# jhljx/CTGCN

Measured on AMD Instinct MI355X. Metric: aggregated edges/s over T-snapshot window (CTGCN-C embedding forward), higher is better.
Workload: dtype f32 (fp16x2-split MFMA operands); 1 GPU; BASELINE config 5: synthetic 1M nodes x 16 cumulative snapshots, avg-deg 16; CTGCN-C hid=128 embed=128, 1 transform + 2 diffusion layers, max_core=8, one-hot features; nodes=1000000, snapshots=16, max_core=8, parallelism=single GPU

## Files before the change

ctgcn_amd/_lib.py:

```python
import ctypes
import os

_HERE = os.path.dirname(os.path.abspath(__file__))
LIB_PATH = os.environ.get("CTGCN_HIP_LIB") or os.path.join(_HERE, "csrc", "libctgcn_hip.so")

F_SELF_LOOP, F_RELU, F_NESTED = 1, 2, 4
ACT_NONE, ACT_SELU = 0, 1
CLS_NODE, CLS_HADAMARD, CLS_DOT = 0, 1, 2
OP_KCORE = 1
OP_INGEST = 2
MAX_SLOTS = 255
ABI_VERSION = 31

_c = ctypes
_vp, _i64, _i32, _u32, _int, _sz = _c.c_void_p, _c.c_int64, _c.c_int32, _c.c_uint32, _c.c_int, _c.c_size_t

class AggSplitGroup(_c.Structure):
    _fields_ = [("row_ptr", _vp), ("col_idx", _vp), ("val", _vp), ("slot", _vp), ("X", _vp), ("ldx", _i64), ("K", _i32), ("flags", _u32),
                ("row_order", _vp), ("tile_mask", _vp), ("workspace", _vp), ("workspace_bytes", _sz),
                ("planes1", _vp), ("planes2", _vp), ("scales", _vp), ("tile_base", _vp)]


class GruLayerGroup(_c.Structure):
    _fields_ = [("planes", _vp), ("w_ih", _vp), ("w_hh", _vp), ("bias_gi", _vp), ("b_hn", _vp), ("ln_weight", _vp), ("ln_bias", _vp),
                ("ln_eps", _c.c_float), ("steps", _i32), ("out", _vp), ("ld_out", _i64), ("row_order", _vp), ("tile_mask", _vp), ("work", _i64)]


class GruSeqGroup(_c.Structure):
    _fields_ = [("gi", _vp), ("w_hh", _vp), ("b_hn", _vp), ("ln_weight", _vp), ("ln_bias", _vp), ("ln_eps", _c.c_float), ("steps", _i32),
                ("out", _vp), ("ld_out", _i64), ("row_order", _vp), ("tile_mask", _vp), ("tile_base", _vp), ("work", _i64)]


SIGNATURES = {
    "ctgcn_abi_version": (_int, []),
    "ctgcn_last_error": (_c.c_char_p, []),
    "ctgcn_device_info": (_int, [_c.c_char_p, _sz, _c.POINTER(_int)]),
    "ctgcn_transpose_bias_f32": (_int, [_i64, _i32, _vp, _i64, _vp, _vp, _i64, _vp]),
    "ctgcn_spmm_csr_f32": (_int, [_i64, _i32, _vp, _vp, _vp, _vp, _i64, _vp, _i64, _int, _vp]),
    "ctgcn_hub_workspace_bytes": (_sz, [_i32, _i32, _i32, _i32]),
    "ctgcn_hub_split_entries": (_i32, []),
    "ctgcn_core_aggregate_f32": (_int, [_i64, _i32, _i32, _vp, _vp, _vp, _vp, _vp, _i64, _vp, _u32, _vp, _i32, _i32, _i32, _vp, _sz, _vp]),
    "ctgcn_core_aggregate_bwd_prep_f32": (_int, [_i64, _i32, _i32, _vp, _vp, _vp, _vp, _u32, _vp]),
    "ctgcn_core_aggregate_bwd_f32": (_int, [_i64, _i32, _i32, _vp, _vp, _vp, _vp, _vp, _vp, _vp, _i64, _u32, _vp, _i32, _i32, _i32, _vp, _sz, _vp]),
    "ctgcn_edges_to_csr": (_int, [_i64, _i64, _vp, _vp, _vp, _vp, _vp, _vp, _c.POINTER(_i64), _vp, _sz, _vp]),
    "ctgcn_kcore_i32": (_int, [_i64, _vp, _vp, _vp, _vp, _sz, _i32, _c.POINTER(_i32), _vp]),
    "ctgcn_edge_levels_i32": (_int, [_i64, _vp, _vp, _vp, _vp, _vp, _vp, _vp, _i32, _vp]),
    "ctgcn_slot_reorder": (_int, [_i64, _i32, _vp, _vp, _vp, _vp, _vp, _i32, _vp, _vp, _vp, _vp]),
    "ctgcn_gru_seq_f32": (_int, [_i64, _i32, _i32, _vp, _vp, _vp, _vp, _vp, _c.c_float, _int, _vp, _i64, _vp, _int, _int, _vp, _vp, _vp, _vp]),
    "ctgcn_layernorm_bwd_f32": (_int, [_i64, _i32, _i32, _vp, _vp, _i64, _vp, _c.c_float, _vp, _vp, _i32, _vp, _vp]),
    "ctgcn_group_table_bytes": (_sz, [_i32]),
    "ctgcn_table_uploads": (ctypes.c_uint64, [_int]),
    "ctgcn_core_aggregate_split_group_f32": (_int, [_i32, _i64, _i32, _vp, _vp, _sz, _vp, _vp]),
    "ctgcn_gru_layer_presplit_group_f32": (_int, [_i32, _i64, _i32, _vp, _vp, _sz, _vp, _vp]),
    "ctgcn_transpose_bias_group_f32": (_int, [_i32, _i64, _i32, _vp, _i64, _vp, _vp, _i64, _vp, _sz, _vp, _vp]),
    "ctgcn_gru_seq_group_f32": (_int, [_i32, _i64, _i32, _vp, _vp, _sz, _vp, _vp]),
    "ctgcn_linear_packed_chain_f32": (_int, [_i64, _i32, _i32, _vp, _vp, _vp, _i32, _vp, _sz, _vp]),
    "ctgcn_linear_packed_group_f32": (_int, [_i32, _i64, _i32, _i32, _vp, _vp, _vp, _vp, _vp, _vp, _i32, _vp, _i64, _vp, _sz, _vp, _vp]),
    "ctgcn_gru_bwd_blocks": (_i32, [_i64]),
    "ctgcn_gru_layer_presplit_save_f32": (_int, [_i64, _i32, _i32, _vp, _i64, _i64, _vp, _vp, _vp, _vp, _vp, _vp, _vp, _vp, _vp]),
    "ctgcn_gru_bwd_rec_f32": (_int, [_i64, _i32, _i32, _vp, _i32, _vp, _vp, _vp, _vp, _vp, _vp, _vp, _vp, _i32, _i32, _vp]),
    "ctgcn_gru_bwd_in_f32": (_int, [_i64, _i32, _i32, _vp, _vp, _vp, _vp, _i64, _i64, _vp, _i64, _vp, _vp, _vp, _vp, _i32, _vp, _vp, _i32, _i32, _vp]),
    "ctgcn_lstm_seq_f32": (_int, [_i64, _i32, _i32, _vp, _vp, _vp, _vp, _c.c_float, _int, _vp, _vp, _vp]),
    "ctgcn_lstm_seq_bwd_f32": (_int, [_i64, _i32, _i32, _vp, _vp, _vp, _vp, _vp, _vp, _i32, _vp]),
    "ctgcn_gru_layer_f32": (_int, [_i64, _i32, _i32, _i32, _vp, _i64, _vp, _vp, _vp, _vp, _vp, _vp, _c.c_float, _int, _vp, _i64, _vp, _vp, _i64, _vp]),
    "ctgcn_linear_workspace_bytes": (_sz, [_i64, _i32, _i32]),
    "ctgcn_split_planes_bytes": (_sz, [_i64, _i32]),
    "ctgcn_split_rows_f32": (_int, [_i64, _i32, _vp, _i64, _vp, _sz, _vp]),
    "ctgcn_pack_weight_bytes": (_sz, [_i32, _i32]),
    "ctgcn_pack_weight_f32": (_int, [_i32, _i32, _vp, _i64, _vp, _sz, _vp]),
    "ctgcn_linear_packed_f32": (_int, [_i64, _i32, _i32, _vp, _vp, _vp, _i32, _vp, _i64, _vp]),
    "ctgcn_linear_f32": (_int, [_i64, _i32, _i32, _vp, _i64, _vp, _i64, _vp, _i32, _vp, _i64, _vp, _sz, _vp]),
    "ctgcn_core_aggregate_split_workspace_bytes": (_sz, [_i64, _i32, _i32, _i32, _i32]),
    "ctgcn_core_aggregate_split_f32": (_int, [_i64, _i32, _i32, _vp, _vp, _vp, _vp, _vp, _i64, _u32, _vp, _i32, _i32, _i32, _vp, _vp, _vp, _i64, _vp, _i32, _vp, _sz, _vp, _sz, _vp]),
    "ctgcn_gru_layer_presplit_f32": (_int, [_i64, _i32, _i32, _vp, _vp, _vp, _vp, _vp, _vp, _vp, _c.c_float, _vp, _i64, _vp, _vp, _vp]),
    "ctgcn_linear_presplit_f32": (_int, [_i64, _i32, _i32, _vp, _i64, _vp, _vp, _i64, _vp, _sz, _vp]),
    "ctgcn_gru_seq_bwd_f32": (_int, [_i64, _i32, _i32, _vp, _vp, _vp, _vp, _vp, _vp, _vp, _vp, _i32, _int, _vp]),
    "ctgcn_gru_input_proj_f32": (_int, [_i64, _i32, _i32, _vp, _i64, _vp, _vp, _vp, _int, _i32, _vp]),
    "ctgcn_gru_input_grad_f32": (_int, [_i64, _i32, _i32, _vp, _vp, _vp, _i64, _vp]),
    "ctgcn_gru_weight_grad_f32": (_int, [_i64, _i32, _i32, _vp, _i64, _vp, _i64, _vp, _i64, _int, _vp, _i32, _int, _vp]),
    "ctgcn_gru_row_granule": (_i64, []),
    "ctgcn_compute_units": (_i32, []),
    "ctgcn_row_cumsum_f32": (_int, [_i64, _vp, _vp, _vp, _vp]),
    "ctgcn_random_walk_pairs": (_int, [_i64, _vp, _vp, _vp, _i32, _i32, _i32, _c.c_uint64, _int, _vp, _vp, _vp, _vp]),
    "ctgcn_neg_sampling_indices": (_int, [_i64, _vp, _vp, _vp, _i32, _i64, _vp, _c.c_uint64, _vp, _vp, _vp, _vp, _vp, _vp]),
    "ctgcn_epoch_scan_workspace_bytes": (_sz, [_i64]),
    "ctgcn_neg_sampling_offsets_batched": (_int, [_i64, _vp, _vp, _i32, _i64, _vp, _vp, _vp, _sz, _vp]),
    "ctgcn_neg_sampling_indices_batched": (_int, [_i64, _vp, _i64, _vp, _vp, _vp, _i32, _i64, _vp, _vp, _vp, _vp, _vp, _vp, _vp]),
    "ctgcn_negsampling_loss_workspace_bytes": (_sz, [_i64, _i64, _i64, _i32]),
    "ctgcn_negsampling_loss_fwd_bwd_f32": (_int, [_i64, _i64, _i64, _i32, _i32, _c.c_float, _vp, _i64, _vp, _vp, _vp, _vp, _vp, _vp, _vp,
                                                  _vp, _vp, _vp, _i64, _vp, _sz, _vp]),
    "ctgcn_reconstruction_loss_workspace_bytes": (_sz, [_i64]),
    "ctgcn_reconstruction_loss_fwd_bwd_f32": (_int, [_i64, _i64, _i32, _vp, _vp, _i64, _vp, _i64, _vp, _vp, _i64, _vp, _i64, _vp, _sz, _vp]),
    "ctgcn_write_embedding_tsv": (_int, [_c.c_char_p, _i64, _i32, _vp, _i64, _c.c_char_p, _vp, _c.c_char, _i32]),
    "ctgcn_lp_neg_sample": (_int, [_i64, _i64, _vp, _i64, _c.c_uint64, _i64, _vp, _vp, _vp, _vp]),
    "ctgcn_lp_grad_workspace_bytes": (_sz, [_i64, _i32, _i32]),
    "ctgcn_lp_grad_f32": (_int, [_i64, _i32, _i32, _u32, _i64, _vp, _i64, _vp, _vp, _vp, _c.c_double, _c.c_double, _vp, _vp, _vp, _vp, _sz, _vp]),
    "ctgcn_lp_hess_workspace_bytes": (_sz, [_i64, _i32, _i32]),
    "ctgcn_lp_hess_f32": (_int, [_i64, _i32, _i32, _u32, _i64, _vp, _i64, _vp, _vp, _vp, _c.c_double, _c.c_double, _vp, _vp, _vp, _sz, _vp]),
    "ctgcn_lp_scores_f32": (_int, [_i64, _i32, _i32, _u32, _i64, _vp, _i64, _vp, _vp, _vp, _vp, _vp]),
    "ctgcn_cent_brandes_workspace_bytes": (_sz, [_i64, _i64, _i64]),
    "ctgcn_cent_brandes": (_int, [_i64, _vp, _vp, _i64, _i64, _vp, _vp, _vp, _vp, _sz, _vp]),
    "ctgcn_cent_eigenvector_workspace_bytes": (_sz, [_i64]),
    "ctgcn_cent_eigenvector": (_int, [_i64, _vp, _vp, _i32, _c.c_double, _vp, _c.POINTER(_i32), _vp, _sz, _vp]),
    "ctgcn_ridge_gram_workspace_bytes": (_sz, [_i32, _i32, _i32]),
    "ctgcn_ridge_gram_f32": (_int, [_i64, _i32, _i32, _i32, _vp, _i64, _vp, _vp, _vp, _sz, _vp]),
    "ctgcn_ridge_gram_f64": (_int, [_i64, _i32, _i32, _i32, _vp, _i64, _vp, _vp, _vp, _sz, _vp]),
    "ctgcn_ridge_sse_workspace_bytes": (_sz, [_i32, _i32]),
    "ctgcn_ridge_sse_f32": (_int, [_i64, _i32, _i32, _i32, _i32, _vp, _i64, _vp, _vp, _vp, _vp, _vp, _sz, _vp]),
    "ctgcn_ridge_sse_f64": (_int, [_i64, _i32, _i32, _i32, _i32, _vp, _i64, _vp, _vp, _vp, _vp, _vp, _sz, _vp]),
    "ctgcn_nc_chunks": (_i64, [_i64]),
    "ctgcn_nc_hess_parts": (_i64, [_i64, _i64]),
    "ctgcn_nc_grad_workspace_bytes": (_sz, [_i64, _i32, _i32]),
    "ctgcn_nc_grad_f32": (_int, [_i32, _i32, _i32, _vp, _vp, _i64, _vp, _vp, _vp, _vp, _vp, _vp, _i64, _vp, _i64, _vp, _i64, _vp, _vp, _vp,
                                 _sz, _vp]),
    "ctgcn_nc_hess_workspace_bytes": (_sz, [_i64, _i32, _i32]),
    "ctgcn_nc_hess_f32": (_int, [_i32, _i32, _i32, _vp, _vp, _i64, _i64, _vp, _vp, _vp, _vp, _vp, _vp, _i64, _vp, _i64, _vp, _i64, _vp, _vp,
                                 _sz, _vp]),
    "ctgcn_nc_predict_f32": (_int, [_i32, _i32, _i32, _i32, _vp, _vp, _i64, _vp, _vp, _vp, _vp, _vp, _i64, _vp, _i64, _vp, _i64, _vp, _vp,
                                    _vp]),
    "ctgcn_ec_grad_f32": (_int, [_i32, _i32, _i32, _vp, _vp, _i64, _vp, _vp, _vp, _vp, _vp, _vp, _vp, _i64, _vp, _i64, _vp, _i64, _vp, _vp,
                                 _vp, _sz, _vp]),
    "ctgcn_ec_hess_f32": (_int, [_i32, _i32, _i32, _vp, _vp, _i64, _i64, _vp, _vp, _vp, _vp, _vp, _vp, _vp, _i64, _vp, _i64, _vp, _i64, _vp,
                                 _vp, _sz, _vp]),
    "ctgcn_ec_predict_f32": (_int, [_i32, _i32, _i32, _i32, _vp, _vp, _i64, _vp, _vp, _vp, _vp, _vp, _vp, _i64, _vp, _i64, _vp, _i64, _vp,
                                    _vp, _vp]),
    "ctgcn_sim_panel_cols": (_i64, [_i64, _i64]),
    "ctgcn_sim_series_workspace_bytes": (_sz, [_i64, _i64]),
    "ctgcn_sim_series": (_int, [_i64, _vp, _vp, _vp, _c.c_double, _i32, _i64, _i64, _i64, _vp, _vp, _sz, _vp]),
    "ctgcn_sim_finish_workspace_bytes": (_sz, [_i64]),
    "ctgcn_sim_finish": (_int, [_i64, _i32, _c.c_double, _vp, _vp, _vp, _vp, _sz, _vp]),
    "ctgcn_sim_coo": (_int, [_i64, _vp, _vp, _vp, _vp, _vp, _vp, _vp]),
    "ctgcn_sim_gram_f32": (_int, [_i64, _i32, _vp, _i64, _vp, _vp, _vp]),
    "ctgcn_sim_gram_f64": (_int, [_i64, _i32, _vp, _i64, _vp, _vp, _vp]),
    "ctgcn_sim_normalize_workspace_bytes": (_sz, [_i64]),
    "ctgcn_sim_normalize": (_int, [_i64, _vp, _vp, _vp, _sz, _vp]),
    "ctgcn_sim_spearman_workspace_bytes": (_sz, [_i64]),
    "ctgcn_sim_spearman": (_int, [_i64, _vp, _vp, _vp, _vp, _vp, _vp, _sz, _vp]),
    "ctgcn_cls_pull_piece": (_i64, []),
    "ctgcn_cls_check_items": (_int, [_i32, _i64, _vp, _vp, _i64, _vp]),
    "ctgcn_cls_head_fwd_f32": (_int, [_i32, _i32, _i64, _i32, _i32, _vp, _vp, _i64, _vp, _i64, _vp, _vp, _vp, _vp]),
    "ctgcn_cls_loss_workspace_bytes": (_sz, [_i64]),
    "ctgcn_cls_loss_f32": (_int, [_i32, _i32, _i64, _i32, _vp, _vp, _vp, _vp, _vp, _vp, _vp, _sz, _vp]),
    "ctgcn_cls_head_bwd_workspace_bytes": (_sz, [_i64, _i32, _i32, _i64]),
    "ctgcn_cls_head_bwd_f32": (_int, [_i32, _i64, _i32, _i32, _vp, _vp, _i64, _vp, _i64, _vp, _vp, _i64, _vp, _vp, _vp, _vp, _vp, _i64, _vp,
                                      _vp, _i64, _vp, _i64, _vp, _vp, _vp, _sz, _vp]),
    "ctgcn_gcn_normalize_workspace_bytes": (_sz, [_i64]),
    "ctgcn_gcn_normalize_f32": (_int, [_i64, _vp, _vp, _vp, _i32, _vp, _vp, _vp, _sz, _vp]),
    "ctgcn_gcn_layer_fwd_f32": (_int, [_i64, _i32, _vp, _vp, _vp, _vp, _i64, _vp, _i64, _i32, _vp, _vp, _vp, _i32, _i32, _vp, _sz, _vp]),
    "ctgcn_gcn_layer_bwd_f32": (_int, [_i64, _i32, _vp, _vp, _vp, _vp, _i64, _vp, _i64, _i32, _vp, _i64, _vp, _i32, _i32, _vp, _sz, _vp]),
    "ctgcn_gcn_conv_fwd_f32": (_int, [_i64, _i32, _vp, _vp, _vp, _vp, _i64, _vp, _vp, _i64, _i32, _c.c_double, _c.c_uint64, _vp, _vp, _i32, _i32,
                                      _vp, _sz, _vp]),
    "ctgcn_gcn_conv_prep_rows": (_i32, []),
    "ctgcn_gcn_conv_prep_workspace_bytes": (_sz, [_i64, _i32]),
    "ctgcn_gcn_conv_prep_f32": (_int, [_i64, _i32, _vp, _i64, _vp, _i64, _vp, _i32, _c.c_double, _vp, _i64, _vp, _vp, _sz, _vp]),
    "ctgcn_gat_piece_floats": (_i32, [_i32, _i32]),
    "ctgcn_gat_da_workspace_bytes": (_sz, [_i64, _i32]),
# ... 110 lines not shown
```

ctgcn_amd/csrc/ctgcn_hip.hip:

```cpp
#include <hip/hip_runtime.h>

#include <atomic>
#include <cstdarg>
#include <cstdio>
#include <cstring>
#include <type_traits>
#include <vector>

#include "../../include/ctgcn_hip.h"
#include "ctgcn_jitter.h"
#include "ctgcn_table.h"
#include "ctgcn_try.h"

namespace {

thread_local char g_err[512] = "";

int fail(int code, const char *fmt, ...)
{
    va_list ap;
    va_start(ap, fmt);
    vsnprintf(g_err, sizeof(g_err), fmt, ap);
    va_end(ap);
    return code;
}

#define HIP_TRY(expr) CTGCN_TRY(expr)

typedef float f4 __attribute__((ext_vector_type(4)));


template <int VEC> struct vec_of;
template <> struct vec_of<4> { using type = f4; };
template <> struct vec_of<1> { using type = float; };

template <int VEC> __device__ __forceinline__ typename vec_of<VEC>::type vzero();
template <> __device__ __forceinline__ f4 vzero<4>() { return f4{0.f, 0.f, 0.f, 0.f}; }
template <> __device__ __forceinline__ float vzero<1>() { return 0.f; }

__device__ __forceinline__ f4 vmax0(f4 v) { return f4{fmaxf(v.x, 0.f), fmaxf(v.y, 0.f), fmaxf(v.z, 0.f), fmaxf(v.w, 0.f)}; }
__device__ __forceinline__ float vmax0(float v) { return fmaxf(v, 0.f); }
__device__ __forceinline__ f4 vfma(float a, f4 x, f4 acc)
{
    return f4{fmaf(a, x.x, acc.x), fmaf(a, x.y, acc.y), fmaf(a, x.z, acc.z), fmaf(a, x.w, acc.w)};
}
__device__ __forceinline__ float vfma(float a, float x, float acc) { return fmaf(a, x, acc); }

struct AggArgs {
    int64_t n;
    int32_t d, K;
    const int32_t *row_ptr;
    const int32_t *col;
    const float *val;
    const uint8_t *slot;
    const float *src;
    int64_t ldsrc;
    const float *self;
    float *out;
    int64_t out_ld;
    uint32_t flags;
    int32_t accumulate;
    int32_t chunks;
    int32_t passes;
    const int32_t *long_rows;
    int32_t n_long;
    int32_t long_thresh;
    int32_t hub_groups;
    int32_t hub_compact;
    int32_t hub_split;
    int32_t hub_ld;
    float *hub_part;
    const int32_t *order;
    const uint32_t *tmask;
    int32_t tile_shift;
    const int32_t *tbase;
};

template <int VEC, int LPR, int U>
__global__ __launch_bounds__(256) void agg_fwd_kernel(const AggArgs a)
{
    using V = typename vec_of<VEC>::type;
    const int lig = threadIdx.x & (LPR - 1);
    const int64_t row = (int64_t)blockIdx.x * (256 / LPR) + (threadIdx.x / LPR);
    if (row >= a.n) return;
    const int start = a.row_ptr[row], end = a.row_ptr[row + 1];
    if (end - start > a.long_thresh) return;
    const bool self = (a.flags & CTGCN_F_SELF_LOOP) != 0;
    const bool relu = (a.flags & CTGCN_F_RELU) != 0;
    const bool nested = (a.flags & CTGCN_F_NESTED) != 0;
    const uint8_t *__restrict__ slot = a.slot;
    const float *__restrict__ X = a.src;
    float *__restrict__ outrow = a.out + row * a.out_ld;

    for (int pass = 0; pass < a.passes; ++pass) {
        const int ch = pass * LPR + lig;
        const bool live = ch < a.chunks;
        const int64_t foff = live ? (int64_t)ch * VEC : 0;
        V R = vzero<VEC>(), P = vzero<VEC>();
        if (self) R = *(const V *)(X + row * a.ldsrc + foff);
        int cur = 0;

        auto close_slot = [&]() {
            R += P;
            if (!nested) P = vzero<VEC>();
            V v = relu ? vmax0(R) : R;
            if (live) {
                V *o = (V *)(outrow + (int64_t)cur * a.d + foff);
                if (a.accumulate) v += *o;
                __builtin_nontemporal_store(v, o);
            }
            ++cur;
        };

        for (int base = start; base < end; base += LPR) {
            const int my = base + lig;
            int c = 0, s = 0;
            float w = 0.f;
            if (my < end) {
                c = a.col[my];
                w = a.val[my];
                s = slot ? (int)slot[my] : 0;
            }
            const int cnt = min(LPR, end - base);
            int j = 0;
            for (; j + U <= cnt; j += U) {
                V xv[U];
                float wj[U];
                int sj[U];
#pragma unroll
                for (int u = 0; u < U; ++u) {
                    const int cj = __shfl(c, j + u, LPR);
                    wj[u] = __shfl(w, j + u, LPR);
                    sj[u] = __shfl(s, j + u, LPR);
                    xv[u] = *(const V *)(X + (int64_t)cj * a.ldsrc + foff);
                }
#pragma unroll
                for (int u = 0; u < U; ++u) {
                    while (cur < sj[u]) close_slot();
                    P = vfma(wj[u], xv[u], P);
                }
            }
            for (; j < cnt; ++j) {
                const int cj = __shfl(c, j, LPR);
                const float w1 = __shfl(w, j, LPR);
                const int s1 = __shfl(s, j, LPR);
                const V x1 = *(const V *)(X + (int64_t)cj * a.ldsrc + foff);
                while (cur < s1) close_slot();
                P = vfma(w1, x1, P);
            }
        }
        while (cur < a.K) close_slot();
    }
}

template <int VEC, int LPR, int U>
__global__ __launch_bounds__(256) void agg_bwd_kernel(const AggArgs a)
{
    using V = typename vec_of<VEC>::type;
    const int lig = threadIdx.x & (LPR - 1);
    const int64_t row = (int64_t)blockIdx.x * (256 / LPR) + (threadIdx.x / LPR);
    if (row >= a.n) return;
    const int start = a.row_ptr[row], end = a.row_ptr[row + 1];
    if (end - start > a.long_thresh) return;
    const uint8_t *__restrict__ slot = a.slot;
    const float *__restrict__ Z = a.src;
    const int64_t zrow = (int64_t)a.K * a.d;

    for (int pass = 0; pass < a.passes; ++pass) {
        const int ch = pass * LPR + lig;
        const bool live = ch < a.chunks;
        const int64_t foff = live ? (int64_t)ch * VEC : 0;
        V P = vzero<VEC>();
        if (a.self) P = *(const V *)(a.self + row * (int64_t)a.d + foff);
        for (int base = start; base < end; base += LPR) {
            const int my = base + lig;
            int64_t off = 0;
            float w = 0.f;
            if (my < end) {
                off = (int64_t)a.col[my] * zrow + (slot ? (int64_t)slot[my] * a.d : 0);
                w = a.val[my];
            }
            const int cnt = min(LPR, end - base);
            int j = 0;
            for (; j + U <= cnt; j += U) {
                V xv[U];
                float wj[U];
#pragma unroll
                for (int u = 0; u < U; ++u) {
                    const int64_t oj = __shfl(off, j + u, LPR);
                    wj[u] = __shfl(w, j + u, LPR);
                    xv[u] = *(const V *)(Z + oj + foff);
                }
#pragma unroll
                for (int u = 0; u < U; ++u) P = vfma(wj[u], xv[u], P);
            }
            for (; j < cnt; ++j) {
                const int64_t oj = __shfl(off, j, LPR);
                const float w1 = __shfl(w, j, LPR);
                P = vfma(w1, *(const V *)(Z + oj + foff), P);
            }
        }
        if (live) {
            V *o = (V *)(a.out + row * a.out_ld + foff);
            if (a.accumulate) P += *o;
            *o = P;
        }
    }
}


constexpr int HUB_THREADS = 1024;
constexpr int HUB_SPLIT_ENTRIES = 8192;
__host__ __device__ __forceinline__ int hub_pieces(int len, int max_pieces)
{
    const int np = (len + HUB_SPLIT_ENTRIES - 1) / HUB_SPLIT_ENTRIES;
    return np < 1 ? 1 : (np > max_pieces ? max_pieces : np);
}

template <int VEC, int LPR, int U>
__global__ __launch_bounds__(HUB_THREADS) void agg_fwd_hub_kernel(const AggArgs a)
{
    using V = typename vec_of<VEC>::type;
    extern __shared__ __align__(16) unsigned char hub_smem[];
    V *part = reinterpret_cast<V *>(hub_smem);
    const int lig = threadIdx.x & (LPR - 1), grp = threadIdx.x / LPR, G = a.hub_groups;
    const bool pieces = a.hub_part != nullptr;
    const int hub = pieces ? (int)(blockIdx.x / a.hub_split) : (int)blockIdx.x, piece = pieces ? (int)(blockIdx.x % a.hub_split) : 0;
    const int64_t row = a.long_rows[hub];
    int start = a.row_ptr[row], end = a.row_ptr[row + 1];
    if (pieces) {
        const int np = hub_pieces(end - start, a.hub_split);
        if (piece >= np) return;
        const int plen = ((end - start + np - 1) / np + LPR - 1) / LPR * LPR;
        start = min(end, start + piece * plen);
        end = min(end, start + plen);
    }
    const int seg = ((end - start + G - 1) / G + LPR - 1) / LPR * LPR;
    const int my_s = min(end, start + grp * seg), my_e = min(end, my_s + seg);
    const bool self = (a.flags & CTGCN_F_SELF_LOOP) != 0, relu = (a.flags & CTGCN_F_RELU) != 0;
    const bool nested = (a.flags & CTGCN_F_NESTED) != 0;
    const uint8_t *__restrict__ slot = a.slot;
    const float *__restrict__ X = a.src;
    float *__restrict__ outrow = a.out + (a.hub_compact ? (int64_t)hub : row) * a.out_ld;

    for (int pass = 0; pass < a.passes; ++pass) {
        const int ch = pass * LPR + lig;
        const bool live = ch < a.chunks;
        const int64_t foff = live ? (int64_t)ch * VEC : 0;
        if (grp < G) {
            for (int k = 0; k < a.K; ++k) part[((int64_t)grp * a.K + k) * LPR + lig] = vzero<VEC>();
            V P = vzero<VEC>();
            int cur = -1;
            for (int base = my_s; base < my_e; base += LPR) {
                const int my = base + lig;
                int c = 0, s = 0;
                float w = 0.f;
                if (my < my_e) { c = a.col[my]; w = a.val[my]; s = slot ? (int)slot[my] : 0; }
                const int cnt = min(LPR, my_e - base);
                int j = 0;
                for (; j + U <= cnt; j += U) {
                    V xv[U];
                    float wj[U];
                    int sj[U];
#pragma unroll
                    for (int u = 0; u < U; ++u) {
                        const int cj = __shfl(c, j + u, LPR);
                        wj[u] = __shfl(w, j + u, LPR);
                        sj[u] = __shfl(s, j + u, LPR);
                        xv[u] = *(const V *)(X + (int64_t)cj * a.ldsrc + foff);
                    }
#pragma unroll
                    for (int u = 0; u < U; ++u) {
                        if (sj[u] != cur) {
                            if (cur >= 0) part[((int64_t)grp * a.K + cur) * LPR + lig] = P;
                            P = vzero<VEC>();
                            cur = sj[u];
                        }
                        P = vfma(wj[u], xv[u], P);
                    }
                }
                for (; j < cnt; ++j) {
                    const int cj = __shfl(c, j, LPR);
                    const float w1 = __shfl(w, j, LPR);
                    const int s1 = __shfl(s, j, LPR);
                    const V x1 = *(const V *)(X + (int64_t)cj * a.ldsrc + foff);
                    if (s1 != cur) {
                        if (cur >= 0) part[((int64_t)grp * a.K + cur) * LPR + lig] = P;
                        P = vzero<VEC>();
                        cur = s1;
                    }
                    P = vfma(w1, x1, P);
                }
            }
            if (cur >= 0) part[((int64_t)grp * a.K + cur) * LPR + lig] = P;
        }
        __syncthreads();
        if (pieces) {
            if (grp == 0 && live) {
                for (int k = 0; k < a.K; ++k) {
                    V sk = vzero<VEC>();
                    for (int g = 0; g < G; ++g) sk += part[((int64_t)g * a.K + k) * LPR + lig];
                    *(V *)(a.hub_part + (((int64_t)hub * a.hub_split + piece) * a.K + k) * a.hub_ld + foff) = sk;
                }
            }
            __syncthreads();
            continue;
        }
        if (grp == 0) {
            V R = vzero<VEC>(), Pc = vzero<VEC>();
            if (self) R = *(const V *)(X + row * a.ldsrc + foff);
            for (int k = 0; k < a.K; ++k) {
                V sk = vzero<VEC>();
                for (int g = 0; g < G; ++g) sk += part[((int64_t)g * a.K + k) * LPR + lig];
                Pc = nested ? Pc + sk : sk;
                R += Pc;
                V v = relu ? vmax0(R) : R;
                if (live) {
                    V *o = (V *)(outrow + (int64_t)k * a.d + foff);
                    if (a.accumulate) v += *o;
                    *o = v;
                }
            }
        }
        __syncthreads();
    }
}

template <int VEC, int LPR, int U>
__global__ __launch_bounds__(HUB_THREADS) void agg_bwd_hub_kernel(const AggArgs a)
{
    using V = typename vec_of<VEC>::type;
    extern __shared__ __align__(16) unsigned char hub_smem[];
    V *part = reinterpret_cast<V *>(hub_smem);
    const int lig = threadIdx.x & (LPR - 1), grp = threadIdx.x / LPR, G = a.hub_groups;
    const bool pieces = a.hub_part != nullptr;
    const int hub = pieces ? (int)(blockIdx.x / a.hub_split) : (int)blockIdx.x, piece = pieces ? (int)(blockIdx.x % a.hub_split) : 0;
    const int64_t row = a.long_rows[hub];
    int start = a.row_ptr[row], end = a.row_ptr[row + 1];
    if (pieces) {
        const int np = hub_pieces(end - start, a.hub_split);
        if (piece >= np) return;
        const int plen = ((end - start + np - 1) / np + LPR - 1) / LPR * LPR;
        start = min(end, start + piece * plen);
        end = min(end, start + plen);
    }
    const int seg = ((end - start + G - 1) / G + LPR - 1) / LPR * LPR;
    const int my_s = min(end, start + grp * seg), my_e = min(end, my_s + seg);
    const uint8_t *__restrict__ slot = a.slot;
    const float *__restrict__ Z = a.src;
    const int64_t zrow = (int64_t)a.K * a.d;

    for (int pass = 0; pass < a.passes; ++pass) {
        const int ch = pass * LPR + lig;
        const bool live = ch < a.chunks;
        const int64_t foff = live ? (int64_t)ch * VEC : 0;
        if (grp < G) {
            V P = vzero<VEC>();
            for (int base = my_s; base < my_e; base += LPR) {
                const int my = base + lig;
                int64_t off = 0;
                float w = 0.f;
                if (my < my_e) {
                    off = (int64_t)a.col[my] * zrow + (slot ? (int64_t)slot[my] * a.d : 0);
                    w = a.val[my];
                }
                const int cnt = min(LPR, my_e - base);
                int j = 0;
                for (; j + U <= cnt; j += U) {
                    V xv[U];
                    float wj[U];
#pragma unroll
                    for (int u = 0; u < U; ++u) {
                        const int64_t oj = __shfl(off, j + u, LPR);
                        wj[u] = __shfl(w, j + u, LPR);
                        xv[u] = *(const V *)(Z + oj + foff);
                    }
#pragma unroll
                    for (int u = 0; u < U; ++u) P = vfma(wj[u], xv[u], P);
                }
                for (; j < cnt; ++j) {
                    const int64_t oj = __shfl(off, j, LPR);
                    const float w1 = __shfl(w, j, LPR);
                    P = vfma(w1, *(const V *)(Z + oj + foff), P);
                }
            }
            part[(int64_t)grp * LPR + lig] = P;
        }
        __syncthreads();
        if (pieces) {
            if (grp == 0 && live) {
                V P = vzero<VEC>();
                for (int g = 0; g < G; ++g) P += part[(int64_t)g * LPR + lig];
                *(V *)(a.hub_part + ((int64_t)hub * a.hub_split + piece) * a.hub_ld + foff) = P;
            }
            __syncthreads();
            continue;
        }
        if (grp == 0) {
            V P = vzero<VEC>();
            if (a.self) P = *(const V *)(a.self + row * (int64_t)a.d + foff);
            for (int g = 0; g < G; ++g) P += part[(int64_t)g * LPR + lig];
            if (live) {
                V *o = (V *)(a.out + row * a.out_ld + foff);
                if (a.accumulate) P += *o;
                *o = P;
            }
        }
        __syncthreads();
    }
}

template <int VEC, bool FWD>
__global__ __launch_bounds__(256) void agg_hub_final_kernel(const AggArgs a)
{
    using V = typename vec_of<VEC>::type;
    const int hub = blockIdx.x;
    const int64_t row = a.long_rows[hub];
    const int np = hub_pieces(a.row_ptr[row + 1] - a.row_ptr[row], a.hub_split);
    const bool self = (a.flags & CTGCN_F_SELF_LOOP) != 0, relu = (a.flags & CTGCN_F_RELU) != 0, nested = (a.flags & CTGCN_F_NESTED) != 0;
    const int KK = FWD ? a.K : 1;
    const float *__restrict__ mine = a.hub_part + (int64_t)hub * a.hub_split * KK * a.hub_ld;
    for (int ch = threadIdx.x; ch < a.chunks; ch += 256) {
        const int64_t foff = (int64_t)ch * VEC;
        if (FWD) {
            float *__restrict__ outrow = a.out + (a.hub_compact ? (int64_t)hub : row) * a.out_ld;
            V R = vzero<VEC>(), Pc = vzero<VEC>();
            if (self) R = *(const V *)(a.src + row * a.ldsrc + foff);
            for (int k = 0; k < a.K; ++k) {
                V sk = vzero<VEC>();
                for (int p = 0; p < np; ++p) sk += *(const V *)(mine + ((int64_t)p * a.K + k) * a.hub_ld + foff);
                Pc = nested ? Pc + sk : sk;
                R += Pc;
                V v = relu ? vmax0(R) : R;
                V *o = (V *)(outrow + (int64_t)k * a.d + foff);
                if (a.accumulate) v += *o;
                *o = v;
            }
        } else {
            V P = vzero<VEC>();
            if (a.self) P = *(const V *)(a.self + row * (int64_t)a.d + foff);
            for (int p = 0; p < np; ++p) P += *(const V *)(mine + (int64_t)p * a.hub_ld + foff);
            V *o = (V *)(a.out + row * a.out_ld + foff);
            if (a.accumulate) P += *o;
            *o = P;
        }
    }
}

template <int VEC>
__global__ __launch_bounds__(256) void agg_bwd_prep_kernel(int64_t n, int32_t d, int32_t K, int32_t chunks,
                                                           const float *__restrict__ dH, const float *__restrict__ H,
                                                           float *__restrict__ Z, float *__restrict__ S0, uint32_t flags)
{
    using V = typename vec_of<VEC>::type;
    const int64_t idx = (int64_t)blockIdx.x * 256 + threadIdx.x;
    if (idx >= n * chunks) return;
    const int64_t row = idx / chunks;
    const int64_t foff = (idx - row * chunks) * VEC;
    const bool relu = (flags & CTGCN_F_RELU) != 0, nested = (flags & CTGCN_F_NESTED) != 0;
    V s = vzero<VEC>(), t = vzero<VEC>();
    for (int j = K - 1; j >= 0; --j) {
        const int64_t o = (row * K + j) * d + foff;
        V g = *(const V *)(dH + o);
        if (relu) {
            const V h = *(const V *)(H + o);
            if constexpr (VEC == 4) {
                g.x = h.x > 0.f ? g.x : 0.f; g.y = h.y > 0.f ? g.y : 0.f;
                g.z = h.z > 0.f ? g.z : 0.f; g.w = h.w > 0.f ? g.w : 0.f;
            } else {
                g = h > 0.f ? g : 0.f;
            }
        }
        s += g;
        t += s;
        *(V *)(Z + o) = nested ? t : s;
    }
    if (S0) *(V *)(S0 + row * d + foff) = s;
}

struct AggPlan { int vec, lpr, chunks, passes; };

AggPlan plan_for(int d, bool vec4_ok)
{
    AggPlan p;
    p.vec = vec4_ok ? 4 : 1;
    p.chunks = (d + p.vec - 1) / p.vec;
    int lpr = 8;
    while (lpr < 64 && lpr < p.chunks) lpr <<= 1;
    p.lpr = lpr;
    p.passes = (p.chunks + lpr - 1) / lpr;
    return p;
}

#ifdef CTGCN_LAYER_TIMELINE
struct LayerArgs;
const char *timeline_begin(LayerArgs &a, unsigned nb8, void *stream);
void timeline_end(LayerArgs &a, unsigned nb8, const char *tl_file, void *stream);
#endif
int g_persistent_cus = 0;
int persistent_cus(int device_cus) { return g_persistent_cus > 0 && g_persistent_cus < device_cus ? g_persistent_cus : device_cus; }


constexpr size_t HUB_LDS_BUDGET = 144 * 1024;

template <bool FWD, int VEC, int LPR>
void launch_agg_t(AggArgs a, hipStream_t st)
{
    constexpr int U = 4;
    const int rows_per_block = 256 / LPR;
    const int64_t blocks = (a.n + rows_per_block - 1) / rows_per_block;
    if (FWD)
        hipLaunchKernelGGL((agg_fwd_kernel<VEC, LPR, U>), dim3((unsigned)blocks), dim3(256), 0, st, a);
    else
        hipLaunchKernelGGL((agg_bwd_kernel<VEC, LPR, U>), dim3((unsigned)blocks), dim3(256), 0, st, a);
    if (a.n_long > 0) {
        const size_t per_group = (size_t)(FWD ? a.K : 1) * LPR * sizeof(typename vec_of<VEC>::type);
        int G = HUB_THREADS / LPR;
        while (G > 1 && per_group * G > HUB_LDS_BUDGET) --G;
        a.hub_groups = G;
        const size_t lds = per_group * G;
        const unsigned hub_grid = (unsigned)a.n_long * (unsigned)(a.hub_part ? a.hub_split : 1);
        if (FWD) {
            auto k = agg_fwd_hub_kernel<VEC, LPR, U>;
            if (lds > 64 * 1024) (void)hipFuncSetAttribute(reinterpret_cast<const void *>(k), hipFuncAttributeMaxDynamicSharedMemorySize, (int)lds);
            hipLaunchKernelGGL(k, dim3(hub_grid), dim3(HUB_THREADS), lds, st, a);
        } else {
            auto k = agg_bwd_hub_kernel<VEC, LPR, U>;
            hipLaunchKernelGGL(k, dim3(hub_grid), dim3(HUB_THREADS), lds, st, a);
        }
        if (a.hub_part) hipLaunchKernelGGL((agg_hub_final_kernel<VEC, FWD>), dim3((unsigned)a.n_long), dim3(256), 0, st, a);
    }
}

size_t hub_workspace_bytes_(int64_t n_long, int32_t hub_split, int32_t slots, int32_t d)
{
    if (n_long <= 0 || hub_split <= 1) return 0;
    return (size_t)n_long * hub_split * slots * ((d + 3) / 4 * 4) * sizeof(float);
}
int set_hub_pieces(AggArgs &a, int32_t slots, int32_t hub_split, void *ws, size_t ws_bytes, const char *who)
{
    a.hub_split = 1; a.hub_part = nullptr; a.hub_ld = (a.d + 3) / 4 * 4;
    if (a.n_long <= 0 || hub_split <= 1 || !ws) return CTGCN_OK;
    if (hub_split > 64) return fail(CTGCN_E_INVALID, "%s: hub_split=%d outside [1,64]", who, hub_split);
    if ((reinterpret_cast<uintptr_t>(ws) & 15u) || ws_bytes < hub_workspace_bytes_(a.n_long, hub_split, slots, a.d))
        return fail(CTGCN_E_WORKSPACE, "%s: hub workspace must be 16-byte aligned and hold ctgcn_hub_workspace_bytes() bytes", who);
    a.hub_split = hub_split; a.hub_part = (float *)ws;
    return CTGCN_OK;
}

template <bool FWD>
int launch_agg(AggArgs a, bool vec4_ok, hipStream_t st)
{
    const AggPlan p = plan_for(a.d, vec4_ok);
    a.chunks = p.chunks;
    a.passes = p.passes;
    if (a.n == 0) return CTGCN_OK;
    if (a.n_long <= 0 || !a.long_rows) { a.n_long = 0; a.long_thresh = 0x7fffffff; }
    if (a.n_long > 0 && (size_t)a.K * p.lpr * (p.vec * 4) > HUB_LDS_BUDGET) { a.n_long = 0; a.long_thresh = 0x7fffffff; }
    const int64_t rows_per_block = 256 / p.lpr;
    if ((a.n + rows_per_block - 1) / rows_per_block > 0x7fffffffLL) return fail(CTGCN_E_UNSUPPORTED, "grid too large");
#define CASE(V, L) if (p.vec == V && p.lpr == L) { launch_agg_t<FWD, V, L>(a, st); }
    CASE(4, 8) else CASE(4, 16) else CASE(4, 32) else CASE(4, 64)
    else CASE(1, 8) else CASE(1, 16) else CASE(1, 32) else CASE(1, 64)
#undef CASE
    HIP_TRY(hipGetLastError());
    return CTGCN_OK;
}

struct KcoreCtl {
    int visited;
    int pool_tail;
    int max_core;
    int pad[13];
};

constexpr int KC_QCAP = 8192;
constexpr int KC_GROUP = 16;
constexpr int KC_LONG = 48;

__global__ __launch_bounds__(256) void kcore_init_kernel(int n, const int32_t *__restrict__ row_ptr,
                                                         const int32_t *__restrict__ col, int32_t *__restrict__ deg)
{
    const int lig = threadIdx.x & 7;
    const int64_t v = ((int64_t)blockIdx.x * 256 + threadIdx.x) >> 3;
    if (v >= n) return;
    int cnt = 0;
    for (int e = row_ptr[v] + lig, end = row_ptr[v + 1]; e < end; e += 8) cnt += (col[e] != (int)v);
    cnt += __shfl_xor(cnt, 1, 8);
    cnt += __shfl_xor(cnt, 2, 8);
    cnt += __shfl_xor(cnt, 4, 8);
    if (lig == 0) deg[v] = cnt;
}

__device__ __forceinline__ bool kc_claim(unsigned *claimed, int v)
{
    const unsigned bit = 1u << (v & 31);
    return (atomicOr(&claimed[v >> 5], bit) & bit) == 0;
}

__global__ __launch_bounds__(256) void kcore_level_kernel(int n, int k, int chunk, const int32_t *__restrict__ row_ptr,
                                                          const int32_t *__restrict__ col, int32_t *deg,
                                                          unsigned *claimed, int32_t *pool_v, int32_t *pool_prev,
                                                          KcoreCtl *ctl)
{
    __shared__ int q[KC_QCAP];
    __shared__ int s_tail, s_top;
    const int tid = threadIdx.x;
    if (tid == 0) { s_tail = 0; s_top = -1; }
    __syncthreads();

    auto push = [&](int u) {
        const int pos = atomicAdd(&s_tail, 1);
        if (pos < KC_QCAP) {
            q[pos] = u;
        } else {
            const int p = atomicAdd(&ctl->pool_tail, 1);
            pool_v[p] = u;
            pool_prev[p] = atomicExch(&s_top, p);
        }
    };

    const int lo = blockIdx.x * chunk, hi = min(n, lo + chunk);
    for (int v = lo + tid; v < hi; v += 256)
        if (__hip_atomic_load(&deg[v], __ATOMIC_RELAXED, __HIP_MEMORY_SCOPE_AGENT) == k && kc_claim(claimed, v)) push(v);

    const int grp = tid / KC_GROUP, lig = tid % KC_GROUP, ngrp = 256 / KC_GROUP;
    const int wv = tid >> 6, wl = tid & 63;
    auto relax = [&](int v, int u) {
        if (u == v) return;
        if (__hip_atomic_load(&deg[u], __ATOMIC_RELAXED, __HIP_MEMORY_SCOPE_AGENT) > k) {
            const int old = atomicSub(&deg[u], 1);
            if (old == k + 1) {
                if (kc_claim(claimed, u)) push(u);
            } else if (old <= k) {
                atomicAdd(&deg[u], 1);
            }
        }
    };
    int begin = 0, processed = 0;
    for (;;) {
        __syncthreads();
        int tail = min(s_tail, KC_QCAP);
        __syncthreads();
        if (begin == tail) {
// ... 808 lines not shown
        __syncthreads();
        auto emit_step = [&](int t) {
            for (int r = wave; r <= last; r += 8)
                gru_layernorm_row(sbuf[r], a.out + ((row0 + r) * steps + t) * GRU_H, lane, a.gamma, a.beta, a.eps);
            __syncthreads();
        };
        if (!REDUCE) emit_step(0);

        for (int t = 1; t < steps; ++t) {
            const int pb = (t - 1) & 1, cb = t & 1;
            const float *gi_t = gi_tile + t * 3 * GRU_H;
            f4v acc[2][3], gq[2][3];
#pragma unroll
            for (int rt = 0; rt <= GRU_RT; ++rt) {
                const int cur = rt & 1, prv = cur ^ 1;
                if (rt < GRU_RT) {
                    const float *p = gi_t + goff(rt);
                    gq[cur][0] = *(const f4v *)p; gq[cur][1] = *(const f4v *)(p + GRU_H); gq[cur][2] = *(const f4v *)(p + 2 * GRU_H);
#pragma unroll
                    for (int g = 0; g < 3; ++g) acc[cur][g] = zero4;
#pragma unroll
                    for (int c = 0; c < 4; ++c) {
                        bf8v af[3];
#pragma unroll
                        for (int sp = 0; sp < 3; ++sp) af[sp] = *(const bf8v *)(&Hs[pb][sp][rt * 16 + col][c * 32 + 8 * grp]);
#define CTGCN_X3_MFMA(I, J)                                                                                              \
                        _Pragma("unroll") for (int g = 0; g < 3; ++g)                                                    \
                            acc[cur][g] = __builtin_amdgcn_mfma_f32_16x16x32_bf16(Wf[J][c][g], af[I], acc[cur][g], 0, 0, 0);
                        CTGCN_X3_PAIRS(CTGCN_X3_MFMA)
#undef CTGCN_X3_MFMA
                    }
                }
                if (rt > 0) {
                    const int rp = rt - 1;
                    const f4v h = gates(gq[prv][0], gq[prv][1], gq[prv][2], acc[prv][0], acc[prv][1], acc[prv][2], hreg[rp], t, rp * 16 + col);
                    hreg[rp] = h;
                    publish(cb, rp * 16 + col, h);
                    if (REDUCE) {
                        f4v *sp_ = (f4v *)(&sbuf[rp * 16 + col][oc]);
                        *sp_ = *sp_ + h;
                    }
                }
            }
            __syncthreads();
            if (!REDUCE) emit_step(t);
        }
        if (REDUCE)
            for (int r = wave; r <= last; r += 8)
                gru_layernorm_row(sbuf[r], a.out + (row0 + r) * a.ldo, lane, a.gamma, a.beta, a.eps);
        __syncthreads();
    }
}

typedef _Float16 h8v __attribute__((ext_vector_type(8)));
typedef _Float16 h4v __attribute__((ext_vector_type(4)));

__device__ __forceinline__ void h2_scale(float m, float &s, float &inv_s)
{
    int e = (int)(__float_as_uint(m) >> 23);
    e = e < 15 ? 15 : (e > 253 ? 253 : e);
    s = __uint_as_float((uint32_t)(e - 14) << 23);
    inv_s = __uint_as_float((uint32_t)(268 - e) << 23);
}
template <int RS>
__device__ __forceinline__ void h2_split(float xs, _Float16 &a, _Float16 &b)
{
    a = (_Float16)xs;
    b = (_Float16)((xs - (float)a) * (float)RS);
}
template <int LPR>
__device__ __forceinline__ float group_max(float m)
{
    uint32_t u = __float_as_uint(m);
    auto dpp = [](uint32_t v, auto ctrl) { return (uint32_t)__builtin_amdgcn_update_dpp(0, (int)v, decltype(ctrl)::value, 0xf, 0xf, true); };
    u = max(u, dpp(u, std::integral_constant<int, 0xB1>{}));
    u = max(u, dpp(u, std::integral_constant<int, 0x4E>{}));
    u = max(u, dpp(u, std::integral_constant<int, 0x141>{}));
    u = max(u, dpp(u, std::integral_constant<int, 0x140>{}));
    u = max(u, (uint32_t)__shfl_xor((int)u, 16, 64));
    if (LPR == 64) u = max(u, (uint32_t)__shfl_xor((int)u, 32, 64));
    return __uint_as_float(u);
}

template <int LPR, int CH, int U, bool WIDE = false>
__device__ __forceinline__ void agg_fwd_split_body(const AggArgs &a, _Float16 *__restrict__ p1, _Float16 *__restrict__ p2,
                                                   float *__restrict__ scale, int32_t kp, float residual_scale, const int64_t bid)
{
    const int lig = threadIdx.x & (LPR - 1);
    const int64_t pos = bid * (256 / LPR) + (threadIdx.x / LPR);
    if (pos >= a.n) return;
    const int64_t row = a.order ? (int64_t)a.order[pos] : pos;
    const int64_t tile = (bid * (256 / LPR)) >> a.tile_shift;
    typedef typename std::conditional<WIDE, uint64_t, uint32_t>::type mask_t;
    constexpr int MB = WIDE ? 63 : 31;
    mask_t need;
    int nneed;
    if constexpr (WIDE) {
        need = a.tmask ? ((mask_t)a.tmask[2 * tile] | ((mask_t)a.tmask[2 * tile + 1] << (WIDE ? 32 : 0))) : ~(mask_t)0;
        nneed = __popcll(need);
    } else {
        need = a.tmask ? a.tmask[tile] : 0xffffffffu;
        nneed = __popc(need);
    }
    const int64_t obase = a.tbase ? (int64_t)a.tbase[tile] + (pos & ((1 << a.tile_shift) - 1)) * nneed : pos * a.K;
    const int start = a.row_ptr[row], end = a.row_ptr[row + 1];
    if (end - start > a.long_thresh) return;
    const bool self = (a.flags & CTGCN_F_SELF_LOOP) != 0;
    const bool relu = (a.flags & CTGCN_F_RELU) != 0;
    const bool nested = (a.flags & CTGCN_F_NESTED) != 0;
    const uint8_t *__restrict__ slot = a.slot;
    const float *__restrict__ X = a.src;
    bool live[CH];
    int64_t foff[CH];
    f4 R[CH], P[CH];
#pragma unroll
    for (int c = 0; c < CH; ++c) {
        const int ch = c * LPR + lig;
        live[c] = ch < a.chunks;
        foff[c] = live[c] ? (int64_t)ch * 4 : 0;
        R[c] = P[c] = vzero<4>();
        if (self && live[c]) R[c] = *(const f4 *)(X + row * a.ldsrc + foff[c]);
    }
    int cur = 0;

    auto close_slot = [&]() {
        f4 v[CH];
        float m = 0.f;
#pragma unroll
        for (int c = 0; c < CH; ++c) {
            R[c] += P[c];
            if (!nested) P[c] = vzero<4>();
        }
        if (!((need >> (cur & MB)) & 1)) { ++cur; return; }
#pragma unroll
        for (int c = 0; c < CH; ++c) {
            v[c] = relu ? vmax0(R[c]) : R[c];
            if (!live[c]) v[c] = vzero<4>();
            m = fmaxf(m, fmaxf(fmaxf(fabsf(v[c].x), fabsf(v[c].y)), fmaxf(fabsf(v[c].z), fabsf(v[c].w))));
        }
        m = group_max<LPR>(m);
        float s, inv;
        h2_scale(m, s, inv);
        int64_t orow;
        if constexpr (WIDE) orow = obase + (a.tbase ? __popcll(need & (((mask_t)1 << (cur & 63)) - (mask_t)1)) : cur);
        else orow = obase + (a.tbase ? __popc(need & ((1u << cur) - 1u)) : cur);
        if (lig == 0) scale[orow] = s;
#pragma unroll
        for (int c = 0; c < CH; ++c) {
            const int k = (c * LPR + lig) * 4;
            if (k < kp) {
                const float xs[4] = {v[c].x * inv, v[c].y * inv, v[c].z * inv, v[c].w * inv};
                h4v h1, h2;
#pragma unroll
                for (int j = 0; j < 4; ++j) {
                    h1[j] = (_Float16)xs[j];
                    h2[j] = (_Float16)((xs[j] - (float)h1[j]) * residual_scale);
                }
                __builtin_nontemporal_store(h1, (h4v *)(p1 + orow * kp + k));
                __builtin_nontemporal_store(h2, (h4v *)(p2 + orow * kp + k));
            }
        }
        ++cur;
    };

    for (int base = start; base < end; base += LPR) {
        const int my = base + lig;
        int c = 0, s = 0;
        float w = 0.f;
        if (my < end) {
            c = a.col[my];
            w = a.val[my];
            s = slot ? (int)slot[my] : 0;
        }
        const int cnt = min(LPR, end - base);
        int j = 0;
        for (; j + U <= cnt; j += U) {
            f4 xv[U][CH];
            float wj[U];
            int sj[U];
#pragma unroll
            for (int u = 0; u < U; ++u) {
                const int cj = __shfl(c, j + u, LPR);
                wj[u] = __shfl(w, j + u, LPR);
                sj[u] = __shfl(s, j + u, LPR);
#pragma unroll
                for (int q = 0; q < CH; ++q) xv[u][q] = *(const f4 *)(X + (int64_t)cj * a.ldsrc + foff[q]);
            }
#pragma unroll
            for (int u = 0; u < U; ++u) {
                while (cur < sj[u]) close_slot();
#pragma unroll
                for (int q = 0; q < CH; ++q) P[q] = vfma(wj[u], xv[u][q], P[q]);
            }
        }
        for (; j < cnt; ++j) {
            const int cj = __shfl(c, j, LPR);
            const float w1 = __shfl(w, j, LPR);
            const int s1 = __shfl(s, j, LPR);
            f4 x1[CH];
#pragma unroll
            for (int q = 0; q < CH; ++q) x1[q] = *(const f4 *)(X + (int64_t)cj * a.ldsrc + foff[q]);
            while (cur < s1) close_slot();
#pragma unroll
            for (int q = 0; q < CH; ++q) P[q] = vfma(w1, x1[q], P[q]);
        }
    }
    while (cur < a.K) close_slot();
}

template <int LPR, int CH, int U, bool WIDE = false>
__global__ __launch_bounds__(256) void agg_fwd_split_kernel(const AggArgs a, _Float16 *__restrict__ p1, _Float16 *__restrict__ p2,
                                                            float *__restrict__ scale, int32_t kp, float residual_scale)
{
    agg_fwd_split_body<LPR, CH, U, WIDE>(a, p1, p2, scale, kp, residual_scale, blockIdx.x);
}
__global__ __launch_bounds__(256) __attribute__((amdgpu_waves_per_eu(7, 8))) void agg_fwd_split32_kernel(
    const AggArgs a, _Float16 *__restrict__ p1, _Float16 *__restrict__ p2, float *__restrict__ scale, int32_t kp, float residual_scale)
{
    agg_fwd_split_body<32, 1, 4>(a, p1, p2, scale, kp, residual_scale, blockIdx.x);
}
__global__ __launch_bounds__(256) void agg_fwd_split32_u8_kernel(
    const AggArgs a, _Float16 *__restrict__ p1, _Float16 *__restrict__ p2, float *__restrict__ scale, int32_t kp, float residual_scale)
{
    agg_fwd_split_body<32, 1, 8>(a, p1, p2, scale, kp, residual_scale, blockIdx.x);
}
struct AggSplitGroup {
    AggArgs a;
    _Float16 *p1, *p2;
    float *scale;
};
__global__ __launch_bounds__(256) void agg_fwd_split32_group_kernel(const AggSplitGroup *__restrict__ table, int32_t blocks_per_group, int32_t kp,
                                                                    float residual_scale)
{
    const int g = __builtin_amdgcn_readfirstlane((int)(blockIdx.x / (unsigned)blocks_per_group));
    const AggSplitGroup G = table[g];
    agg_fwd_split_body<32, 1, 8>(G.a, G.p1, G.p2, G.scale, kp, residual_scale, (int64_t)(blockIdx.x % (unsigned)blocks_per_group));
}
template <int CH>
__global__ __launch_bounds__(256) void agg_fwd_split_group_kernel(const AggSplitGroup *__restrict__ table, int32_t blocks_per_group, int32_t kp,
                                                                  float residual_scale)
{
    const int g = __builtin_amdgcn_readfirstlane((int)(blockIdx.x / (unsigned)blocks_per_group));
    const AggSplitGroup G = table[g];
    agg_fwd_split_body<64, CH, 8>(G.a, G.p1, G.p2, G.scale, kp, residual_scale, (int64_t)(blockIdx.x % (unsigned)blocks_per_group));
}

template <int RS>
__device__ __forceinline__ void h2_split_x8(const float *src, float inv_s, h8v &s0, h8v &s1)
{
    const f4v lo = *(const f4v *)src, hi = *(const f4v *)(src + 4);
#pragma unroll
    for (int j = 0; j < 4; ++j) {
        _Float16 a, b;
        h2_split<RS>(lo[j] * inv_s, a, b); s0[j] = a; s1[j] = b;
        h2_split<RS>(hi[j] * inv_s, a, b); s0[4 + j] = a; s1[4 + j] = b;
    }
}
template <int RS>
__device__ __forceinline__ void h2_load_weights(const float *w, int wave, int col, int grp, h8v (&Wf)[2][4][3], float (*wscale)[GRU_H])
{
#pragma unroll
    for (int g = 0; g < 3; ++g) {
        const float *row = w + (int64_t)(g * GRU_H + wave * 16 + col) * GRU_H;
        float m = 0.f;
#pragma unroll
        for (int c = 0; c < 4; ++c) {
            const f4v lo = *(const f4v *)(row + c * 32 + 8 * grp), hi = *(const f4v *)(row + c * 32 + 8 * grp + 4);
#pragma unroll
            for (int j = 0; j < 4; ++j) m = fmaxf(m, fmaxf(fabsf(lo[j]), fabsf(hi[j])));
        }
        m = fmaxf(m, __shfl_xor(m, 16));
        m = fmaxf(m, __shfl_xor(m, 32));
        float sc, inv;
        h2_scale(m, sc, inv);
        if (grp == 0) wscale[g][wave * 16 + col] = sc;
#pragma unroll
        for (int c = 0; c < 4; ++c) h2_split_x8<RS>(row + c * 32 + 8 * grp, inv, Wf[0][c][g], Wf[1][c][g]);
    }
}
#define CTGCN_H2_MFMA1(WF, C, X1, X2, A)                                                                                 \
    _Pragma("unroll") for (int g = 0; g < 3; ++g) A[g] = __builtin_amdgcn_mfma_f32_16x16x32_f16(WF[0][C][g], X2, A[g], 0, 0, 0); \
    _Pragma("unroll") for (int g = 0; g < 3; ++g) A[g] = __builtin_amdgcn_mfma_f32_16x16x32_f16(WF[1][C][g], X1, A[g], 0, 0, 0); \
    _Pragma("unroll") for (int g = 0; g < 3; ++g) A[g] = __builtin_amdgcn_mfma_f32_16x16x32_f16(WF[0][C][g], X1, A[g], 0, 0, 0);

__global__ __launch_bounds__(512, 2) void gru_proj_h2_kernel(const ProjArgs a)
{
    __shared__ _Float16 As[2][2][PJ_BM][PJ_PITCH];
    __shared__ float rscale[2][PJ_BM];
    __shared__ float wscale[3][GRU_H];
    const int tid = threadIdx.x, wave = tid >> 6, lane = tid & 63;
    const int col = lane & 15, grp = lane >> 4;

    h8v Wf[2][4][3];
    h2_load_weights<1>(a.w, wave, col, grp, Wf, wscale);
    __syncthreads();
    const int oc = wave * 16 + 4 * grp;
    f4v bias[3], wsc[3];
#pragma unroll
    for (int g = 0; g < 3; ++g) {
        bias[g] = a.bias ? *(const f4v *)(a.bias + g * GRU_H + oc) : f4v{0.f, 0.f, 0.f, 0.f};
        wsc[g] = *(const f4v *)(&wscale[g][oc]);
    }
// ... 1964 lines not shown
template <bool VEC>
__global__ __launch_bounds__(256) void transpose_bias_kernel(int64_t n, int d, const float *__restrict__ w, int64_t ldw,
                                                             const float *__restrict__ bias, float *__restrict__ out, int64_t ldo)
{
    transpose_bias_body<VEC>(n, d, w, ldw, bias, out, ldo);
}
template <bool VEC>
__global__ __launch_bounds__(256) void transpose_bias_group_kernel(int64_t n, int d, const TransposeGroup *__restrict__ table, int64_t ldw, int64_t ldo)
{
    const TransposeGroup G = table[blockIdx.z];
    transpose_bias_body<VEC>(n, d, G.w, ldw, G.bias, G.out, ldo);
}

__global__ void kcore_copy_kernel(int n, int cap, const int32_t *__restrict__ deg, int32_t *__restrict__ core)
{
    const int64_t v = (int64_t)blockIdx.x * 256 + threadIdx.x;
    if (v < n) core[v] = min(deg[v], cap);
}

size_t align_up(size_t x, size_t a) { return (x + a - 1) / a * a; }

}

extern "C" size_t ctgcn_ingest_workspace_bytes_(int64_t n, int64_t m);

extern "C" int ctgcn_set_error_(int code, const char *msg) { return fail(code, "%s", msg); }
extern "C" void ctgcn_set_persistent_cus(int cus) { g_persistent_cus = cus; }
extern "C" int ctgcn_persistent_cus_(int device_cus) { return persistent_cus(device_cus); }
extern "C" int ctgcn_split_rows_mapped_(int64_t rows, int32_t k, int32_t kp, const float *x, int64_t ldx, void *p1, void *p2, float *scale,
                                        const int32_t *group_map, int32_t group, float residual_scale, void *stream);

extern "C" {

int ctgcn_abi_version(void) { return CTGCN_ABI_VERSION; }

static std::atomic<uint64_t> g_table_written{0}, g_table_current{0};
void ctgcn_table_count_(int written) { (written ? g_table_written : g_table_current).fetch_add(1, std::memory_order_relaxed); }
uint64_t ctgcn_table_uploads(int current) { return (current ? g_table_current : g_table_written).load(std::memory_order_relaxed); }

const char *ctgcn_last_error(void) { return g_err; }

int ctgcn_device_info(char *name_host, size_t name_len, int *cu_count_host)
{
    int dev = 0;
    HIP_TRY(hipGetDevice(&dev));
    hipDeviceProp_t prop;
    HIP_TRY(hipGetDeviceProperties(&prop, dev));
    if (name_host && name_len) snprintf(name_host, name_len, "%s (%s)", prop.name, prop.gcnArchName);
    if (cu_count_host) *cu_count_host = prop.multiProcessorCount;
    return CTGCN_OK;
}

int ctgcn_transpose_bias_f32(int64_t n, int32_t d, const float *w, int64_t ldw, const float *bias, float *out, int64_t ldo,
                             void *stream)
{
    if (n < 0 || d < 1 || ldw < n || ldo < d) return fail(CTGCN_E_INVALID, "transpose_bias: bad sizes n=%lld d=%d", (long long)n, d);
    if (n == 0) return CTGCN_OK;
    if (!w || !out) return fail(CTGCN_E_INVALID, "transpose_bias: null pointer");
    const dim3 grid((unsigned)((n + 63) / 64), (unsigned)((d + 63) / 64));
    if (!(ldw & 3) && !(ldo & 3) && ctgcn_aligned16(w) && ctgcn_aligned16(out))
        hipLaunchKernelGGL(transpose_bias_kernel<true>, grid, dim3(256), 0, (hipStream_t)stream, n, d, w, ldw, bias, out, ldo);
    else
        hipLaunchKernelGGL(transpose_bias_kernel<false>, grid, dim3(256), 0, (hipStream_t)stream, n, d, w, ldw, bias, out, ldo);
    HIP_TRY(hipGetLastError());
    return CTGCN_OK;
}

int ctgcn_spmm_csr_f32(int64_t n_rows, int32_t d, const int32_t *row_ptr, const int32_t *col_idx,
                       const float *val, const float *X, int64_t ldx, float *Y, int64_t ldy,
                       int accumulate, void *stream)
{
    if (n_rows < 0 || d <= 0 || ldx < d || ldy < d) return fail(CTGCN_E_INVALID, "spmm_csr: bad sizes n=%lld d=%d ldx=%lld ldy=%lld", (long long)n_rows, d, (long long)ldx, (long long)ldy);
    if (n_rows == 0) return CTGCN_OK;
    if (!row_ptr || !X || !Y) return fail(CTGCN_E_INVALID, "spmm_csr: null pointer");
    AggArgs a{};
    a.n = n_rows; a.d = d; a.K = 1;
    a.row_ptr = row_ptr; a.col = col_idx; a.val = val; a.slot = nullptr;
    a.src = X; a.ldsrc = ldx; a.self = nullptr; a.out = Y; a.out_ld = ldy;
    a.flags = CTGCN_F_NESTED; a.accumulate = accumulate ? 1 : 0;
    const bool v4 = (d % 4 == 0) && (ldx % 4 == 0) && (ldy % 4 == 0) && ctgcn_aligned16(X) && ctgcn_aligned16(Y);
    return launch_agg<true>(a, v4, (hipStream_t)stream);
}

int ctgcn_core_aggregate_f32(int64_t n_rows, int32_t d, int32_t K, const int32_t *row_ptr,
                             const int32_t *col_idx, const float *val, const uint8_t *slot,
                             const float *X, int64_t ldx, float *H, uint32_t flags,
                             const int32_t *long_rows, int32_t n_long, int32_t long_threshold,
                             int32_t hub_split, void *hub_workspace, size_t hub_workspace_bytes, void *stream)
{
    if (n_rows < 0 || d <= 0 || ldx < d) return fail(CTGCN_E_INVALID, "core_aggregate: bad sizes n=%lld d=%d ldx=%lld", (long long)n_rows, d, (long long)ldx);
    if (K < 1 || K > CTGCN_MAX_SLOTS) return fail(CTGCN_E_INVALID, "core_aggregate: K=%d outside [1,%d]", K, CTGCN_MAX_SLOTS);
    if (n_rows == 0) return CTGCN_OK;
    if (!row_ptr || !X || !H) return fail(CTGCN_E_INVALID, "core_aggregate: null pointer");
    if (!slot && K != 1) return fail(CTGCN_E_INVALID, "core_aggregate: slot tags required when K > 1");
    AggArgs a{};
    a.n = n_rows; a.d = d; a.K = K;
    a.row_ptr = row_ptr; a.col = col_idx; a.val = val; a.slot = slot;
    a.src = X; a.ldsrc = ldx; a.self = nullptr; a.out = H; a.out_ld = (int64_t)K * d;
    a.flags = flags; a.accumulate = 0;
    a.long_rows = long_rows; a.n_long = n_long; a.long_thresh = long_threshold;
    if (n_long > 0 && long_threshold < 1) return fail(CTGCN_E_INVALID, "core_aggregate: long_threshold must be >= 1");
    if (int rc = set_hub_pieces(a, K, hub_split, hub_workspace, hub_workspace_bytes, "core_aggregate")) return rc;
    const bool v4 = (d % 4 == 0) && (ldx % 4 == 0) && ctgcn_aligned16(X) && ctgcn_aligned16(H);
    return launch_agg<true>(a, v4, (hipStream_t)stream);
}

size_t ctgcn_core_aggregate_split_workspace_bytes(int64_t n_rows, int32_t d, int32_t K, int32_t n_out, int32_t n_long)
{
    if (n_rows < 0 || d < 1 || K < 1 || n_out < 1 || n_long < 0) return 0;
    return ctgcn_linear_workspace_bytes((n_rows + 63) / 64 * 64 * K, n_out, d) + ((size_t)n_long * K * d * 4 + 255) / 256 * 256;
}

int ctgcn_core_aggregate_split_f32(int64_t n_rows, int32_t d, int32_t K, const int32_t *row_ptr, const int32_t *col_idx,
                                   const float *val, const uint8_t *slot, const float *X, int64_t ldx, uint32_t flags,
                                   const int32_t *long_rows, int32_t n_long, int32_t long_threshold, int32_t n_out,
                                   const int32_t *row_order, const uint32_t *tile_mask, const int32_t *tile_base, int64_t operand_rows,
                                   const int32_t *hub_row_dest,
                                   int32_t hub_split, void *hub_workspace, size_t hub_workspace_bytes,
                                   void *workspace, size_t workspace_bytes, void *stream)
{
    if (n_rows < 0 || d <= 0 || ldx < d || n_out < 1) return fail(CTGCN_E_INVALID, "core_aggregate_split: bad sizes n=%lld d=%d ldx=%lld", (long long)n_rows, d, (long long)ldx);
    if (K < 1 || K > CTGCN_MAX_SLOTS) return fail(CTGCN_E_INVALID, "core_aggregate_split: K=%d outside [1,%d]", K, CTGCN_MAX_SLOTS);
    if (n_rows == 0) return CTGCN_OK;
    if (!row_ptr || !X || !workspace) return fail(CTGCN_E_INVALID, "core_aggregate_split: null pointer");
    if (!slot && K != 1) return fail(CTGCN_E_INVALID, "core_aggregate_split: slot tags required when K > 1");
    if ((d & 3) || d > 512 || (ldx & 3) || !ctgcn_aligned16(X) || (reinterpret_cast<uintptr_t>(workspace) & 255u))
        return fail(CTGCN_E_UNSUPPORTED, "core_aggregate_split: needs d %% 4 == 0, d <= 512, 16-byte aligned rows, 256-byte aligned workspace");
    if (n_long < 0 || (n_long > 0 && (!long_rows || long_threshold < 1))) return fail(CTGCN_E_INVALID, "core_aggregate_split: bad hub row list");
    if ((row_order == nullptr) != (tile_mask == nullptr)) return fail(CTGCN_E_INVALID, "core_aggregate_split: row_order and tile_mask come together");
    if (row_order && K > 64) return fail(CTGCN_E_UNSUPPORTED, "core_aggregate_split: a row plan needs K <= 64");
    if (row_order && ((d == 128 && n_out == 1) != (tile_base == nullptr)))
        return fail(CTGCN_E_INVALID, "core_aggregate_split: tile_base (compact operand rows, tiles of 64) goes with the GEMM consumer, tiles of 16 without it with the GRU layer kernel");
    if (!row_order && tile_base) return fail(CTGCN_E_INVALID, "core_aggregate_split: tile_base without a row plan");
    if (tile_base && (operand_rows < 1 || operand_rows > (n_rows + 63) / 64 * 64 * K))
        return fail(CTGCN_E_INVALID, "core_aggregate_split: operand_rows=%lld outside [1, ceil64(n_rows) K]", (long long)operand_rows);
    if (row_order && n_long > 0 && !hub_row_dest) return fail(CTGCN_E_INVALID, "core_aggregate_split: hub rows under a row plan need their destination rows");
    if (workspace_bytes < ctgcn_core_aggregate_split_workspace_bytes(n_rows, d, K, n_out, n_long))
        return fail(CTGCN_E_WORKSPACE, "core_aggregate_split: workspace too small (ctgcn_core_aggregate_split_workspace_bytes)");
    hipStream_t st = (hipStream_t)stream;
    const int64_t rows = tile_base ? operand_rows : n_rows * K;
    const int32_t kp = (d + 63) / 64 * 64;
    _Float16 *p1 = (_Float16 *)workspace, *p2 = p1 + (size_t)rows * kp;
    float *scale = (float *)(p2 + (size_t)rows * kp);
    float *hub = (float *)((char *)workspace + ctgcn_linear_workspace_bytes((n_rows + 63) / 64 * 64 * K, n_out, d));
    AggArgs a{};
    a.n = n_rows; a.d = d; a.K = K;
    a.row_ptr = row_ptr; a.col = col_idx; a.val = val; a.slot = slot;
    a.src = X; a.ldsrc = ldx; a.self = nullptr; a.out = hub; a.out_ld = (int64_t)K * d;
    a.flags = flags; a.accumulate = 0;
    a.long_rows = long_rows; a.n_long = n_long; a.long_thresh = long_threshold;
    a.order = row_order; a.tmask = tile_mask; a.tbase = tile_base; a.tile_shift = tile_base ? 6 : 4;
    const AggPlan p = plan_for(d, true);
    a.chunks = p.chunks;
    a.passes = p.passes;
    if (a.n_long > 0 && (size_t)K * p.lpr * 16 > HUB_LDS_BUDGET) a.n_long = 0;
    if (a.n_long <= 0) { a.n_long = 0; a.long_thresh = 0x7fffffff; }
    if (int rc = set_hub_pieces(a, K, hub_split, hub_workspace, hub_workspace_bytes, "core_aggregate_split")) return rc;
    const int rows_per_block = p.chunks <= 32 ? 8 : 4;
    const int64_t blocks = (n_rows + rows_per_block - 1) / rows_per_block;
    if (blocks > 0x7fffffffLL) return fail(CTGCN_E_UNSUPPORTED, "core_aggregate_split: grid too large");
    const float rsc = 1.f;
    static const int force_u8 = [] { const char *e = getenv("CTGCN_AGG_U8"); return e ? atoi(e) : -1; }();
    const bool u8 = force_u8 >= 0 ? force_u8 != 0 : n_rows <= 200000;
    if (row_order && K > 32) {
        if (p.chunks <= 32) hipLaunchKernelGGL((agg_fwd_split_kernel<32, 1, 8, true>), dim3((unsigned)blocks), dim3(256), 0, st, a, p1, p2, scale, kp, rsc);
        else if (p.chunks <= 64) hipLaunchKernelGGL((agg_fwd_split_kernel<64, 1, 8, true>), dim3((unsigned)blocks), dim3(256), 0, st, a, p1, p2, scale, kp, rsc);
        else hipLaunchKernelGGL((agg_fwd_split_kernel<64, 2, 8, true>), dim3((unsigned)blocks), dim3(256), 0, st, a, p1, p2, scale, kp, rsc);
    } else
    if (p.chunks <= 32 && u8) hipLaunchKernelGGL(agg_fwd_split32_u8_kernel, dim3((unsigned)blocks), dim3(256), 0, st, a, p1, p2, scale, kp, rsc);
    else if (p.chunks <= 32) hipLaunchKernelGGL(agg_fwd_split32_kernel, dim3((unsigned)blocks), dim3(256), 0, st, a, p1, p2, scale, kp, rsc);
    else if (p.chunks <= 64) hipLaunchKernelGGL((agg_fwd_split_kernel<64, 1, 4>), dim3((unsigned)blocks), dim3(256), 0, st, a, p1, p2, scale, kp, rsc);
    else if (n_rows <= 200000) hipLaunchKernelGGL((agg_fwd_split_kernel<64, 2, 8>), dim3((unsigned)blocks), dim3(256), 0, st, a, p1, p2, scale, kp, rsc);
    else hipLaunchKernelGGL((agg_fwd_split_kernel<64, 2, 4>), dim3((unsigned)blocks), dim3(256), 0, st, a, p1, p2, scale, kp, rsc);
    HIP_TRY(hipGetLastError());
    if (a.n_long > 0) {
        a.hub_compact = 1;
        const size_t per_group = (size_t)K * p.lpr * 16;
        int G = HUB_THREADS / p.lpr;
        while (G > 1 && per_group * G > HUB_LDS_BUDGET) --G;
        a.hub_groups = G;
        const size_t lds = per_group * G;
#define HUBCASE(L)                                                                                                                        \
        if (p.lpr == L) {                                                                                                                 \
            auto k = agg_fwd_hub_kernel<4, L, 4>;                                                                                        \
            if (lds > 64 * 1024) (void)hipFuncSetAttribute(reinterpret_cast<const void *>(k), hipFuncAttributeMaxDynamicSharedMemorySize, (int)lds); \
            hipLaunchKernelGGL(k, dim3((unsigned)a.n_long * (unsigned)(a.hub_part ? a.hub_split : 1)), dim3(HUB_THREADS), lds, st, a);    \
        }
        HUBCASE(8) else HUBCASE(16) else HUBCASE(32) else HUBCASE(64)
#undef HUBCASE
        if (a.hub_part) hipLaunchKernelGGL((agg_hub_final_kernel<4, true>), dim3((unsigned)a.n_long), dim3(256), 0, st, a);
        HIP_TRY(hipGetLastError());
        const int rc = row_order ? ctgcn_split_rows_mapped_((int64_t)a.n_long * K, d, kp, hub, d, p1, p2, scale, hub_row_dest, -1, rsc, stream)
                                 : ctgcn_split_rows_mapped_((int64_t)a.n_long * K, d, kp, hub, d, p1, p2, scale, long_rows, K, rsc, stream);
        if (rc != CTGCN_OK) return rc;
    }
    return CTGCN_OK;
}

int ctgcn_core_aggregate_bwd_prep_f32(int64_t n_rows, int32_t d, int32_t K, const float *dH,
                                      const float *H, float *Z, float *S0, uint32_t flags, void *stream)
{
    if (n_rows < 0 || d <= 0 || K < 1 || K > CTGCN_MAX_SLOTS) return fail(CTGCN_E_INVALID, "bwd_prep: bad sizes");
    if (n_rows == 0) return CTGCN_OK;
    if (!dH || !Z || ((flags & CTGCN_F_RELU) && !H)) return fail(CTGCN_E_INVALID, "bwd_prep: null pointer");
    const bool v4 = (d % 4 == 0) && ctgcn_aligned16(dH) && ctgcn_aligned16(Z) && (!H || ctgcn_aligned16(H)) && (!S0 || ctgcn_aligned16(S0));
    const int vec = v4 ? 4 : 1;
    const int chunks = (d + vec - 1) / vec;
    const int64_t total = n_rows * chunks;
    const int64_t blocks = (total + 255) / 256;
    if (blocks > 0x7fffffffLL) return fail(CTGCN_E_UNSUPPORTED, "bwd_prep: grid too large");
    if (v4)
        hipLaunchKernelGGL(agg_bwd_prep_kernel<4>, dim3((unsigned)blocks), dim3(256), 0, (hipStream_t)stream, n_rows, d, K, chunks, dH, H, Z, S0, flags);
    else
        hipLaunchKernelGGL(agg_bwd_prep_kernel<1>, dim3((unsigned)blocks), dim3(256), 0, (hipStream_t)stream, n_rows, d, K, chunks, dH, H, Z, S0, flags);
    HIP_TRY(hipGetLastError());
    return CTGCN_OK;
}

int ctgcn_core_aggregate_bwd_f32(int64_t n_rows, int32_t d, int32_t K, const int32_t *row_ptr,
                                 const int32_t *col_idx, const float *val, const uint8_t *slot,
                                 const float *Z, const float *S0, float *dX, int64_t lddx,
                                 uint32_t flags, const int32_t *long_rows, int32_t n_long,
                                 int32_t long_threshold, int32_t hub_split, void *hub_workspace, size_t hub_workspace_bytes, void *stream)
{
    if (n_rows < 0 || d <= 0 || lddx < d || K < 1 || K > CTGCN_MAX_SLOTS) return fail(CTGCN_E_INVALID, "core_aggregate_bwd: bad sizes");
    if (n_rows == 0) return CTGCN_OK;
    if (!row_ptr || !Z || !dX) return fail(CTGCN_E_INVALID, "core_aggregate_bwd: null pointer");
    if (!slot && K != 1) return fail(CTGCN_E_INVALID, "core_aggregate_bwd: slot tags required when K > 1");
    if ((flags & CTGCN_F_SELF_LOOP) && !S0) return fail(CTGCN_E_INVALID, "core_aggregate_bwd: S0 required with SELF_LOOP");
    AggArgs a{};
    a.n = n_rows; a.d = d; a.K = K;
    a.row_ptr = row_ptr; a.col = col_idx; a.val = val; a.slot = slot;
    a.src = Z; a.ldsrc = 0; a.self = (flags & CTGCN_F_SELF_LOOP) ? S0 : nullptr;
    a.out = dX; a.out_ld = lddx; a.flags = flags; a.accumulate = 0;
    a.long_rows = long_rows; a.n_long = n_long; a.long_thresh = long_threshold;
    if (n_long > 0 && long_threshold < 1) return fail(CTGCN_E_INVALID, "core_aggregate_bwd: long_threshold must be >= 1");
    if (int rc = set_hub_pieces(a, 1, hub_split, hub_workspace, hub_workspace_bytes, "core_aggregate_bwd")) return rc;
    const bool v4 = (d % 4 == 0) && (lddx % 4 == 0) && ctgcn_aligned16(Z) && ctgcn_aligned16(dX) && (!a.self || ctgcn_aligned16(a.self));
    return launch_agg<false>(a, v4, (hipStream_t)stream);
}

size_t ctgcn_hub_workspace_bytes(int32_t n_long, int32_t hub_split, int32_t slots, int32_t d)
{
    return hub_workspace_bytes_(n_long, hub_split, slots, d);
}

int32_t ctgcn_hub_split_entries(void) { return HUB_SPLIT_ENTRIES; }

size_t ctgcn_workspace_bytes(int op, int64_t n, int64_t nnz, int32_t d, int32_t K)
{
    (void)nnz; (void)d; (void)K;
    if (op == CTGCN_OP_KCORE) {
        const size_t nn = (size_t)(n > 0 ? n : 0);
        return align_up(sizeof(KcoreCtl), 256) + align_up(nn * 4, 256)  + align_up((nn + 31) / 32 * 4, 256)
               + 2 * align_up(nn * 4, 256) ;
    }
    if (op == CTGCN_OP_INGEST) return ctgcn_ingest_workspace_bytes_(n, nnz);
    return 0;
}

int ctgcn_kcore_i32(int64_t n, const int32_t *row_ptr, const int32_t *col_idx, int32_t *core,
                    void *workspace, size_t workspace_bytes, int32_t level_cap, int32_t *max_core_host, void *stream)
{
    if (n < 0 || n > 0x7fffffffLL) return fail(CTGCN_E_INVALID, "kcore: n=%lld out of range", (long long)n);
    if (max_core_host) *max_core_host = 0;
    if (n == 0) return CTGCN_OK;
    if (!row_ptr || !core || !workspace) return fail(CTGCN_E_INVALID, "kcore: null pointer");
    const size_t need = ctgcn_workspace_bytes(CTGCN_OP_KCORE, n, 0, 0, 0);
    if (workspace_bytes < need) return fail(CTGCN_E_WORKSPACE, "kcore: workspace %zu < %zu bytes", workspace_bytes, need);
    hipStream_t st = (hipStream_t)stream;
    char *ws = (char *)workspace;
    KcoreCtl *ctl = (KcoreCtl *)ws; ws += align_up(sizeof(KcoreCtl), 256);
    int32_t *deg = (int32_t *)ws; ws += align_up((size_t)n * 4, 256);
    unsigned *claimed = (unsigned *)ws; const size_t claimed_bytes = align_up(((size_t)n + 31) / 32 * 4, 256); ws += claimed_bytes;
    int32_t *pool_v = (int32_t *)ws; ws += align_up((size_t)n * 4, 256);
    int32_t *pool_prev = (int32_t *)ws;

    const int nn = (int)n;
    static const int forced = [] { const char *e = getenv("CTGCN_KCORE"); return !e ? 0 : (!strcmp(e, "peel") ? 1 : (!strcmp(e, "hindex") ? 2 : 0)); }();
// ... 697 lines not shown
```

ctgcn_amd/layers.py:

```python
import torch
from torch import nn
from torch.nn import functional as F

from . import ops
from .core_adj import CoreAdj

_RNN = {"GRU": nn.GRU, "LSTM": nn.LSTM}
_RNN_MAX_ELEMS = 1 << 29


def rnn_reduce_norm(rnn, norm, seq, reduce_sum, out=None, resident_backward=True):
    if out is not None and torch.is_grad_enabled() and (seq.requires_grad or any(p.requires_grad for p in rnn.parameters())):
        out = None
    if ops.gru_fused_ok(rnn, seq):
        if out is not None and reduce_sum:
            return ops.gru_sequence(rnn, seq, norm, reduce_sum, out=out)
        res = ops.gru_sequence(rnn, seq, norm, reduce_sum, resident_backward=resident_backward)
    elif ops.lstm_fused_ok(rnn, seq):
        res = ops.lstm_sequence(rnn, seq, norm, reduce_sum)
    elif ops.rnn_cell_ok(rnn, seq):
        res = norm(rnn_cells_over_rows(rnn, seq, reduce_sum))
    else:
        res = norm(rnn_over_rows(rnn, seq, reduce_sum))
    if out is not None:
# ... 47 lines not shown


def as_gcn_adj(adj, device, symmetric=True):
    if isinstance(adj, ops.GcnAdj):
        if adj.device != torch.device(device):
            raise ValueError("GcnAdj on %s but features on %s" % (adj.device, device))
        return adj
    if not (isinstance(adj, torch.Tensor) and adj.is_sparse):
        raise TypeError("a GcnAdj or a torch sparse matrix expected, got %s" % type(adj).__name__)
    key = (id(adj), adj._values().data_ptr(), str(device), bool(symmetric))
    hit = _gcn_adj_cache.get(key)
    if hit is None:
        if len(_gcn_adj_cache) > 256:
            _gcn_adj_cache.clear()
        hit = _gcn_adj_cache[key] = (ops.GcnAdj.from_sparse_tensor(adj, device, check_symmetric=bool(symmetric)), adj)
    return hit[0]


def as_pool_adj(adj, kind, self_loop=False):
    cache = adj.__dict__.setdefault("_pool", {})
    hit = cache.get((kind, bool(self_loop)))
    if hit is not None:
        return hit
    n, dev = adj.n, adj.device
    rows, cols = adj._rows(), adj.col.to(torch.int64)
    eye = torch.arange(n, device=dev)
    if kind in ("sum", "average"):
        vals = adj.val
        if self_loop:
            rows, cols, vals = torch.cat((rows, eye)), torch.cat((cols, eye)), torch.cat((vals, torch.ones(n, device=dev)))
        t = torch.sparse_coo_tensor(torch.stack((rows, cols)), vals, torch.Size((n, n)))
        out = ops.GcnAdj.from_sparse_tensor(t, dev, long_threshold=adj.long_threshold, check_symmetric=False)
        if kind == "average":
            out.val = ops.gcn_normalize(out.row_ptr, out.col, out.val, row_norm=True)
    elif kind in ("pattern-sum", "pattern-average"):
        keys = rows * n + cols
        if self_loop:
            keys = torch.unique(torch.cat((keys, eye * (n + 1))))
        else:
            keys = torch.unique(keys)
        rows, cols = torch.div(keys, n, rounding_mode="floor"), keys % n
        counts = torch.bincount(rows, minlength=n)
        row_ptr = torch.zeros(n + 1, dtype=torch.int64, device=dev)
        row_ptr[1:] = counts.cumsum(0)
        vals = torch.ones(keys.numel(), dtype=torch.float32, device=dev)
        if kind == "pattern-average":
            vals = (1.0 / counts.to(torch.float64))[rows].to(torch.float32)
        out = ops.GcnAdj(row_ptr.to(torch.int32), cols.to(torch.int32), vals, adj.long_threshold)
    else:
        raise ValueError("unknown pooling matrix %r" % (kind,))
    cache[kind, bool(self_loop)] = out
    return out


_identity_cache = {}


def _is_identity(sp_tensor):
    key = (id(sp_tensor), sp_tensor._values().data_ptr())
    entry = _identity_cache.get(key)
    if entry is None:
        n, m = sp_tensor.shape
        idx, val = sp_tensor._indices(), sp_tensor._values()
        flag = bool(n == m and val.numel() == n and idx.shape[0] == 2
                    and bool(((idx[0] == idx[1]) & (val == 1)).all())
                    and bool((idx[0].sort().values == torch.arange(n, device=idx.device)).all()))
        if len(_identity_cache) > 256:
            _identity_cache.clear()
        entry = _identity_cache[key] = (flag, sp_tensor)
    return entry[0]


class CoreDiffusion(nn.Module):

    def __init__(self, input_dim, output_dim, core_num=1, bias=True, rnn_type='GRU'):
        super().__init__()
        assert rnn_type in _RNN
        self.input_dim, self.output_dim = input_dim, output_dim
        self.core_num, self.bias, self.rnn_type = core_num, bias, rnn_type
        self.linear = nn.Linear(input_dim, output_dim)
        self.rnn = _RNN[rnn_type](input_size=input_dim, hidden_size=output_dim, num_layers=1, bias=bias, batch_first=True)
        self.norm = nn.LayerNorm(output_dim)

    def aggregate(self, x, adj_list):
        return ops.core_aggregate(x, as_core_adj(adj_list, x.device), relu=True)

    def forward(self, x, adj_list, out=None):
        if torch.is_tensor(x) and not x.is_sparse and x.is_cuda:
            adj = as_core_adj(adj_list, x.device)
            if ops.aggregate_split_ok(self.rnn, x, adj):
                return ops.core_diffusion_split(x, adj, self.rnn, self.norm, out=out)
            if torch.is_grad_enabled() and ops.core_diffusion_fused_ok(self.rnn, self.norm, x, adj):
                return ops.core_diffusion_fused(x, adj, self.rnn, self.norm)
        seq = self.aggregate(x, adj_list)
        return rnn_reduce_norm(self.rnn, self.norm, seq, reduce_sum=True, out=out)


class MLP(nn.Module):

    def __init__(self, input_dim, hidden_dim, output_dim, layer_num, bias=True, activate_type='N'):
        super().__init__()
        assert activate_type in ['L', 'N']
        assert layer_num > 0
        self.input_dim, self.hidden_dim, self.output_dim = input_dim, hidden_dim, output_dim
        self.layer_num, self.bias, self.activate_type = layer_num, bias, activate_type
        if layer_num == 1:
            self.linear = nn.Linear(input_dim, output_dim, bias=bias)
        else:
            widths = [input_dim] + [hidden_dim] * (layer_num - 1) + [output_dim]
            self.linears = nn.ModuleList(nn.Linear(a, b, bias=bias) for a, b in zip(widths[:-1], widths[1:]))

    @staticmethod
    def _apply_linear(layer, h, selu=False, static_x=False):
        out, fused = MLP._linear(layer, h, selu, static_x)
        return F.selu(out) if (selu and not fused) else out

    @staticmethod
    def _linear(layer, h, selu, static_x=False):
        if h.is_sparse:
            if _is_identity(h):
                if h.is_cuda and layer.weight.dtype == torch.float32:
                    return ops.linear_of_identity(layer.weight, layer.bias), False
                return (layer.weight.t() + layer.bias if layer.bias is not None else layer.weight.t().contiguous()), False
            out = torch.sparse.mm(h, layer.weight.t())
            return (out if layer.bias is None else out + layer.bias), False
        needs_grad = torch.is_grad_enabled() and (h.requires_grad or any(p.requires_grad for p in layer.parameters()))
        if not needs_grad and h.dim() == 2 and ops.linear_split_ok(h, layer.weight):
            return ops.linear_split(h, layer.weight, layer.bias, selu=selu, static_x=static_x), bool(selu)
        if needs_grad and h.dim() == 2 and ops.linear_train_enabled() and ops.linear_split_ok(h, layer.weight) and ops.plane_cache_enabled() \
                and h.shape[0] >= 4096:
            return ops.linear_split_train(h, layer.weight, layer.bias, static_x=static_x), False
        return layer(h), False

    def forward(self, x):
        stack = [self.linear] if self.layer_num == 1 else list(self.linears)
        selu = self.activate_type == 'N'
        if len(stack) > 1 and not (torch.is_grad_enabled() and (any(p.requires_grad for p in self.parameters()) or
                                                              (torch.is_tensor(x) and x.requires_grad))):
            i = 0
            while i + 1 < len(stack) and ops.linear_chain_ok(x, stack[i].weight, stack[i + 1].weight):
                x = ops.linear_split(x, stack[i].weight, stack[i].bias, selu=selu, static_x=(i == 0 and ops.is_static(x)), planes_out=True)
                i += 1
            if i:
                x = ops.linear_split(x, stack[i].weight, stack[i].bias, selu=selu)
                stack = stack[i + 1:]
        for i, layer in enumerate(stack):
            x = self._apply_linear(layer, x, selu=self.activate_type == 'N', static_x=(i == 0 and ops.is_static(x)))
        return x
```

ctgcn_amd/models.py:

```python
import os

import torch
from torch import nn
from torch.nn import functional as F

from . import ops
from ._lib import ACT_NONE, ACT_SELU, CtgcnHipError
from .layers import CoreDiffusion, MLP, rnn_reduce_norm
from . import snapshot_parallel as sp_par


class CDN(nn.Module):

    def __init__(self, input_dim, hidden_dim, output_dim, diffusion_num, bias=True, rnn_type='GRU'):
        super().__init__()
        if diffusion_num < 1:
            raise ValueError("number of layers should be positive!")
        self.input_dim, self.hidden_dim, self.output_dim = input_dim, hidden_dim, output_dim
        self.diffusion_num, self.bias, self.rnn_type = diffusion_num, bias, rnn_type
        dims = [input_dim] + [hidden_dim] * (diffusion_num - 1) + [output_dim]
        self.diffusion_list = nn.ModuleList(
            CoreDiffusion(a, b, bias=bias, rnn_type=rnn_type) for a, b in zip(dims[:-1], dims[1:]))

    def forward(self, x, adj_list, out=None):
        last = len(self.diffusion_list) - 1
        for i, layer in enumerate(self.diffusion_list):
            x = layer(x, adj_list, out=out if i == last else None)
        return x


def _check_types(model_type, trans_activate_type):
    assert model_type in ['C', 'S']
    assert trans_activate_type in ['L', 'N']


def _branch_dims(model_type, hidden_dim, output_dim):
    return (hidden_dim, hidden_dim) if model_type == 'C' else (output_dim, output_dim)


class CGCN(nn.Module):

    def __init__(self, input_dim, hidden_dim, output_dim, trans_num, diffusion_num, bias=True, rnn_type='GRU',
                 model_type='C', trans_activate_type='L'):
        super().__init__()
        _check_types(model_type, trans_activate_type)
        self.input_dim, self.hidden_dim, self.output_dim = input_dim, hidden_dim, output_dim
        self.trans_num, self.diffusion_num, self.bias = trans_num, diffusion_num, bias
        self.rnn_type, self.model_type, self.trans_activate_type = rnn_type, model_type, trans_activate_type
        self.method_name = 'CGCN-' + model_type
        mlp_out, cdn_in = _branch_dims(model_type, hidden_dim, output_dim)
        self.mlp = MLP(input_dim, hidden_dim, mlp_out, trans_num, bias=bias, activate_type=trans_activate_type)
        self.duffision = CDN(cdn_in, output_dim, output_dim, diffusion_num, rnn_type=rnn_type)
        self.process_group = None

    def cgcn(self, x, adj):
        trans = self.mlp(x)
        emb = self.duffision(trans, adj)
        return (emb, trans) if self.model_type == 'S' else emb

    def forward(self, x, adj):
        if not isinstance(x, list):
            return self.cgcn(x, adj)
        if self.process_group is not None:
            return sp_par.cgcn_forward_sharded(self, x, adj)
        results = [self.cgcn(x_t, adj_t) for x_t, adj_t in zip(x, adj)]
        if self.model_type == 'C':
            return results
        return [r[0] for r in results], [r[1] for r in results]


class _StackSteps(torch.autograd.Function):

    @staticmethod
    def forward(ctx, *hx):
        n, d = hx[0].shape
        out = torch.empty(n, len(hx), d, dtype=hx[0].dtype, device=hx[0].device)
        for t, h in enumerate(hx):
            out[:, t].copy_(h)
        return out

    @staticmethod
    def backward(ctx, grad):
        return tuple(grad[:, t] for t in range(grad.shape[1]))


def _stack_steps(hx):
    same = all(h.shape == hx[0].shape and h.dtype == hx[0].dtype and h.device == hx[0].device for h in hx)
    return _StackSteps.apply(*hx) if same and hx[0].dim() == 2 else torch.stack(hx).transpose(0, 1)


class CTGCN(nn.Module):

    def __init__(self, input_dim, hidden_dim, output_dim, trans_num, diffusion_num, duration, bias=True, rnn_type='GRU',
                 model_type='C', trans_activate_type='L'):
        super().__init__()
        _check_types(model_type, trans_activate_type)
        assert rnn_type in ['LSTM', 'GRU']
        self.input_dim, self.hidden_dim, self.output_dim = input_dim, hidden_dim, output_dim
        self.rnn_type, self.model_type, self.trans_activate_type = rnn_type, model_type, trans_activate_type
        self.method_name = 'CTGCN-' + model_type
        self.duration, self.trans_num, self.diffusion_num, self.bias = duration, trans_num, diffusion_num, bias
        mlp_out, cdn_in = _branch_dims(model_type, hidden_dim, output_dim)
        self.mlp_list = nn.ModuleList(
            MLP(input_dim, hidden_dim, mlp_out, trans_num, bias=bias, activate_type=trans_activate_type)
            for _ in range(duration))
        self.duffision_list = nn.ModuleList(
            CDN(cdn_in, output_dim, output_dim, diffusion_num, rnn_type=rnn_type) for _ in range(duration))
        rnn_cls = nn.LSTM if rnn_type == 'LSTM' else nn.GRU
        self.rnn = rnn_cls(output_dim, output_dim, num_layers=1, bias=bias, batch_first=True)
        self.norm = nn.LayerNorm(output_dim)
        self.process_group = None

    def snapshot_branch(self, t, x, adj, out=None):
        trans = self.mlp_list[t](x)
        return self.duffision_list[t](trans, adj, out=out), trans

    def temporal_head(self, hx):
        return rnn_reduce_norm(self.rnn, self.norm, hx, reduce_sum=False).transpose(0, 1)

    def _needs_autograd(self, x_list):
        if not torch.is_grad_enabled():
            return False
        return any(p.requires_grad for p in self.parameters()) or any(
            isinstance(x, torch.Tensor) and x.requires_grad for x in x_list)

    def _snapshot_streams(self, seq, n, T, x_list):
        if seq is None or not seq.is_cuda or T < 2:
            return None
        env = os.environ.get("CTGCN_STREAMS")
        k = int(env) if env else (2 if n <= 200_000 else 1)
        k = min(k, T)
        if k <= 1 or not self._branches_use_own_kernels(x_list):
            return None
        cache = getattr(self, "_stream_cache", None)
        if cache is None or cache[0] != (seq.device, k):
            cache = self._stream_cache = ((seq.device, k), [torch.cuda.Stream(device=seq.device) for _ in range(k)])
        return cache[1]

    def _training_streams(self, x_list, adj_list, T):
        from . import ops
        from .layers import _is_identity
        k = min(int(os.environ.get("CTGCN_TRAIN_STREAMS", "3")), T)
        if k <= 1 or self.rnn_type != 'GRU' or self.output_dim != 128 or not ops.split_mfma_enabled() or not ops.linear_split_enabled() \
                or not ops.wide_weight_grad_enabled() or torch.cuda.is_current_stream_capturing():
            return None
        p0 = next(self.parameters())
        if not p0.is_cuda or not all(torch.is_tensor(x) and x.is_sparse and x.is_cuda and _is_identity(x) for x in x_list):
            return None
        n = adj_list[0].n if hasattr(adj_list[0], "n") else adj_list[0][0].shape[0]
        if n > 200_000 or any(m.layer_num != 1 for m in self.mlp_list):
            return None
        cache = getattr(self, "_train_stream_cache", None)
        if cache is None or cache[0] != (p0.device, k):
            cache = self._train_stream_cache = ((p0.device, k), [torch.cuda.Stream(device=p0.device) for _ in range(k)])
        return cache[1]

    def _branches_use_own_kernels(self, x_list):
        from . import ops
        from .layers import _is_identity

        def kind(x):
            if not torch.is_tensor(x):
                return None
            if x.is_sparse:
                return ("sparse", _is_identity(x), tuple(x.shape))
            return ("dense", tuple(x.shape), tuple(x.stride()), x.data_ptr() % 16, x.dtype, x.device)
        key = (ops.forward_split_mode(), ops.linear_split_enabled()) + tuple(kind(x) for x in x_list)
        cache = getattr(self, "_own_kernel_cache", None)
        if cache is None or cache[0] != key:
            cache = self._own_kernel_cache = (key, self._branches_use_own_kernels_uncached(x_list))
        return cache[1]

    def _branches_use_own_kernels_uncached(self, x_list):
        from . import ops
        from .layers import _is_identity
        if self.rnn_type != 'GRU' or self.output_dim != 128 or ops.forward_split_mode() != 2 or not ops.linear_split_enabled():
            return False
        for t, x in enumerate(x_list):
            if not torch.is_tensor(x) or not x.is_cuda:
                return False
            mlp = self.mlp_list[t]
            layers = [mlp.linear] if mlp.layer_num == 1 else list(mlp.linears)
            if x.is_sparse:
                if not _is_identity(x) or layers[0].weight.dtype != torch.float32:
                    return False
                layers = layers[1:]
                h = None
                width = mlp.output_dim if mlp.layer_num == 1 else mlp.hidden_dim
            else:
                h, width = x, x.shape[1]
            for lin in layers:
                probe = h if h is not None else torch.empty(1, width, dtype=torch.float32, device=x.device)
                if probe.dim() != 2 or not ops.linear_split_ok(probe, lin.weight):
                    return False
                h, width = None, lin.weight.shape[0]
            for cd in self.duffision_list[t].diffusion_list:
# ... 6 lines not shown
        if not ops.group_launch_enabled() or T < 2 or self.rnn_type != 'GRU' or self.output_dim != 128 or not hasattr(adj_list[0], "n"):
            return None
        if adj_list[0].n > ops._GROUP_MAX_NODES:
            return None
        L = self.diffusion_num
        g0 = L
        for l in reversed(range(L)):
            if all(cdn.diffusion_list[l].input_dim == 128 and cdn.diffusion_list[l].output_dim == 128 for cdn in self.duffision_list):
                g0 = l
            else:
                break
        return g0 if g0 < L else None

    _HEAD_GROUP_MAX = 120_000

    def _grouped_head(self, x_list, adj_list, seq):
        from . import ops
        from .layers import as_core_adj, _is_identity
        T = len(x_list)
        dev = seq.device
        mods = [self.duffision_list[t].diffusion_list[0] for t in range(T)]
        if any(m.input_dim == 128 or m.output_dim != 128 for m in mods) or not ops.group_launch_enabled():
            return None
        adjs = [as_core_adj(adj_list[t], dev) for t in range(T)]
        env = os.environ.get("CTGCN_GROUP_HEAD")
        if env == "0" or (env != "1" and adjs[0].n * T > self._HEAD_GROUP_MAX):
            return None
        mlps = [self.mlp_list[t] for t in range(T)]
        one_hot = all(m.layer_num == 1 and m.activate_type == 'L' and torch.is_tensor(x) and x.is_sparse and x.is_cuda and _is_identity(x)
                      for m, x in zip(mlps, x_list))
        ws, bs = [m.linear.weight for m in mlps] if one_hot else None, [m.linear.bias for m in mlps] if one_hot else None
        if one_hot and ops.linear_of_identity_group_ok(ws, bs):
            trans = ops.linear_of_identity_group(ws, bs)
        else:
            trans = [mlps[t](x_list[t]) for t in range(T)]
        rnns, norms = [m.rnn for m in mods], [m.norm for m in mods]
        if ops.core_diffusion_wide_group_ok(trans, adjs, rnns, norms):
            outs = [torch.empty(trans[t].shape[0], self.output_dim, dtype=trans[t].dtype, device=dev) for t in range(T)]
            ops.core_diffusion_wide_group(trans, adjs, rnns, norms, outs)
        else:
            outs = [mods[t](trans[t], adjs[t]) for t in range(T)]
        return outs, trans

    def _grouped_layers(self, g0, hs, adj_list, seq):
        from . import ops
        from .layers import as_core_adj
        T, L = len(hs), self.diffusion_num
        adjs = [as_core_adj(adj_list[t], hs[t].device) for t in range(T)]
        for l in range(g0, L):
            mods = [self.duffision_list[t].diffusion_list[l] for t in range(T)]
            last = l == L - 1
            outs = [seq[:, t] if last else torch.empty(hs[t].shape[0], self.output_dim, dtype=hs[t].dtype, device=hs[t].device) for t in range(T)]
            rnns, norms = [m.rnn for m in mods], [m.norm for m in mods]
            if ops.core_diffusion_group_ok(hs, adjs, rnns, norms):
                ops.core_diffusion_split_group(hs, adjs, rnns, norms, outs)
            else:
                for t in range(T):
                    r = mods[t](hs[t], adjs[t], out=outs[t] if last else None)
                    if last and r.data_ptr() != outs[t].data_ptr():
                        outs[t].copy_(r)
                    elif not last:
                        outs[t] = r
            hs = outs
        return hs

    def forward(self, x_list, adj_list):
        if self.process_group is not None:
            return sp_par.ctgcn_forward_sharded(self, x_list, adj_list)
        hx, trans = [], []
        T = len(x_list)
        seq = None
        if T > 0 and not self._needs_autograd(x_list):
            n = adj_list[0].n if hasattr(adj_list[0], "n") else adj_list[0][0].shape[0]
            p0 = next(self.parameters())
            seq = torch.empty(n, T, self.output_dim, dtype=p0.dtype, device=p0.device)
        lanes = self._snapshot_streams(seq, n if seq is not None else 0, T, x_list)
        g0 = self._group_start(adj_list, T) if (seq is not None and seq.is_cuda) else None
        grouped_head = self._grouped_head(x_list, adj_list, seq) if g0 == 1 else None
        if grouped_head is not None:
            hx, trans = grouped_head
            self._grouped_layers(g0, hx, adj_list, seq)
        elif g0 is not None:
            def head(t):
                tr = self.mlp_list[t](x_list[t])
                h = tr
                for l in range(g0):
                    h = self.duffision_list[t].diffusion_list[l](h, adj_list[t])
                return h, tr
            if lanes:
                main = torch.cuda.current_stream(seq.device)
                for s_ in lanes:
                    s_.wait_stream(main)
                for t in range(T):
                    with torch.cuda.stream(lanes[t % len(lanes)]):
                        h, tr = head(t)
                        h.record_stream(main)
                        tr.record_stream(main)
                    hx.append(h)
                    trans.append(tr)
                for s_ in lanes:
                    main.wait_stream(s_)
            else:
                for t in range(T):
                    h, tr = head(t)
                    hx.append(h)
                    trans.append(tr)
            self._grouped_layers(g0, hx, adj_list, seq)
        elif lanes:
            main = torch.cuda.current_stream(seq.device)
            for s_ in lanes:
                s_.wait_stream(main)
            for t in range(T):
                with torch.cuda.stream(lanes[t % len(lanes)]):
                    h, tr = self.snapshot_branch(t, x_list[t], adj_list[t], out=seq[:, t])
                    if h.data_ptr() != seq[:, t].data_ptr():
                        seq[:, t].copy_(h)
                    tr.record_stream(main)
                hx.append(h)
                trans.append(tr)
            for s_ in lanes:
                main.wait_stream(s_)
        elif seq is None and self._training_streams(x_list, adj_list, T):
            tl = self._training_streams(x_list, adj_list, T)
            main = torch.cuda.current_stream(tl[0].device)
            for s_ in tl:
                s_.wait_stream(main)
            for t in range(T):
                with torch.cuda.stream(tl[t % len(tl)]):
                    h, tr = self.snapshot_branch(t, x_list[t], adj_list[t])
                    h.record_stream(main)
                    tr.record_stream(main)
                hx.append(h)
                trans.append(tr)
            for s_ in tl:
                main.wait_stream(s_)
        else:
            for t in range(T):
                h, tr = self.snapshot_branch(t, x_list[t], adj_list[t], out=None if seq is None else seq[:, t])
                if seq is not None and h.data_ptr() != seq[:, t].data_ptr():
                    seq[:, t].copy_(h)
                hx.append(h)
                trans.append(tr)
        out = self.temporal_head(seq if seq is not None else _stack_steps(hx))
        return out if self.model_type == 'C' else (out, trans)


def _snapshots(x):
    return isinstance(x, (list, tuple)) or x.dim() == 3


def _check_head_input(x, what):
    if not x.is_cuda:
        raise CtgcnHipError("%s runs on MI355X only: got a %s tensor; there is no CPU fallback" % (what, x.device))
    if x.dtype != torch.float32 or x.dim() != 2:
        raise ValueError("%s reads float32 [N, d] embeddings, got %s %s" % (what, x.dtype, tuple(x.shape)))


def _single_linear(layer_num, what):
    if layer_num != 1:
        raise NotImplementedError("%s: the fused head covers a single Linear (layer_num == 1, every shipped config); got layer_num = %d"
                                  % (what, layer_num))


class MLPClassifier(nn.Module):

    def __init__(self, input_dim, hidden_dim, output_dim, layer_num, duration, bias=True, activate_type='N'):
        super().__init__()
        _single_linear(layer_num, "MLPClassifier")
        self.input_dim, self.hidden_dim, self.output_dim = input_dim, hidden_dim, output_dim
        self.layer_num, self.duration, self.bias, self.activate_type = layer_num, duration, bias, activate_type
        self.fused = True
        self.mlp_list = nn.ModuleList(MLP(input_dim, hidden_dim, output_dim, layer_num, bias=bias, activate_type=activate_type)
                                      for _ in range(duration))

    def forward(self, x, batch_indices=None):
        if _snapshots(x):
            return [self.mlp_classifier(x[i], None if batch_indices is None else batch_indices[i]) for i in range(len(x))]
        return self.mlp_classifier(x, batch_indices)

    def _head(self, x, idx, mode):
        _check_head_input(x, type(self).__name__)
        lin = self.mlp_list[0].linear
        selu = self.activate_type == 'N'
        if self.fused:
            return ops.cls_head(x, idx, lin.weight, lin.bias, mode, ACT_SELU if selu else ACT_NONE)
        feat = x[idx] if mode == ops.CLS_NODE else x[idx[0]] * x[idx[1]]
        out = F.linear(feat, lin.weight, lin.bias)
        return F.selu(out) if selu else out

    def mlp_classifier(self, x, batch_indices=None):
        if batch_indices is None:
            _check_head_input(x, "MLPClassifier")
            return self.mlp_list[0](x)
        return self._head(x, batch_indices, ops.CLS_NODE)


class InnerProduct(nn.Module):

    def __init__(self, reduce=True):
        super().__init__()
        self.reduce = reduce
        self.fused = True

    def forward(self, x, edge_index):
        if _snapshots(x):
            return [self.inner_product(x[i], edge_index[i]) for i in range(len(x))]
        return self.inner_product(x, edge_index)

    def inner_product(self, x, edge_index):
        assert edge_index.shape[0] == 2
        _check_head_input(x, "InnerProduct")
        if self.reduce and self.fused:
            return ops.cls_head(x, edge_index, None, None, ops.CLS_DOT)
        prod = x[edge_index[0]] * x[edge_index[1]]
# ... 28 lines not shown
```

ctgcn_amd/ops.py:

```python
import ctypes

import torch

from . import _lib
from ._lib import check, ptr


def _need_cuda(*tensors):
    for t in tensors:
        if t is not None and not t.is_cuda:
            raise _lib.CtgcnHipError(
                "ctgcn_amd runs on MI355X only: got a %s tensor. Move inputs (features and CoreAdj) to the GPU; "
                "there is no CPU fallback." % t.device)


def _stream():
    return ctypes.c_void_p(torch.cuda.current_stream().cuda_stream)


_launch_timer = None


def set_launch_timer(callback):
    global _launch_timer
# ... 23 lines not shown


def edges_to_csr(src, dst, w, n):
    _need_cuda(src, dst, w)
    lib = _lib.load()
    src, dst = _i32(src), _i32(dst)
    if w is not None:
        w = w if (w.dtype == torch.float32 and w.is_contiguous()) else w.to(torch.float32).contiguous()
    m = src.numel()
    dev = src.device
    row_ptr = torch.empty(n + 1, dtype=torch.int32, device=dev)
    col = torch.empty(2 * m, dtype=torch.int32, device=dev)
    val = torch.empty(2 * m, dtype=torch.float32, device=dev)
    nnz = ctypes.c_int64(0)
    with torch.cuda.device(dev):
        nbytes = lib.ctgcn_workspace_bytes(_lib.OP_INGEST, n, m, 0, 0)
        ws = torch.empty(max(nbytes, 1), dtype=torch.uint8, device=dev)
        check(lib.ctgcn_edges_to_csr(n, m, ptr(src), ptr(dst), ptr(w), ptr(row_ptr), ptr(col), ptr(val), ctypes.byref(nnz),
                                     ptr(ws), nbytes, _stream()), "ctgcn_edges_to_csr")
    k = int(nnz.value)
    return row_ptr, col[:k], val[:k]


def kcore(row_ptr, col, level_cap=-1):
    _need_cuda(row_ptr, col)
    lib = _lib.load()
    row_ptr, col = _i32(row_ptr), _i32(col)
    n = row_ptr.numel() - 1
    core = torch.empty(n, dtype=torch.int32, device=row_ptr.device)
    if n == 0:
        return core, 0
    with torch.cuda.device(row_ptr.device):
        nbytes = lib.ctgcn_workspace_bytes(_lib.OP_KCORE, n, col.numel(), 0, 0)
        ws = torch.empty(nbytes, dtype=torch.uint8, device=row_ptr.device)
        mx = ctypes.c_int32(0)
        check(lib.ctgcn_kcore_i32(n, ptr(row_ptr), ptr(col), ptr(core), ptr(ws), nbytes, int(level_cap), ctypes.byref(mx),
                                  _stream()), "ctgcn_kcore_i32")
    return core, int(mx.value)


def edge_levels(row_ptr, col, val, core, hist_len):
    _need_cuda(row_ptr, col, val, core)
    lib = _lib.load()
    n = row_ptr.numel() - 1
    dev = row_ptr.device
    level = torch.empty(col.numel(), dtype=torch.int32, device=dev)
    count = torch.zeros(hist_len, dtype=torch.int64, device=dev)
    wsum = torch.zeros(hist_len, dtype=torch.float64, device=dev)
    with torch.cuda.device(dev):
        check(lib.ctgcn_edge_levels_i32(n, ptr(row_ptr), ptr(col), ptr(val), ptr(core), ptr(level), ptr(count), ptr(wsum),
                                        hist_len, _stream()), "ctgcn_edge_levels_i32")
    return level, count, wsum


def slot_reorder(row_ptr, col, val, level, table, K):
    _need_cuda(row_ptr, col, val, level, table)
    lib = _lib.load()
    n = row_ptr.numel() - 1
    col2, val2 = torch.empty_like(col), torch.empty_like(val)
    slot2 = torch.empty(col.numel(), dtype=torch.uint8, device=col.device)
    with torch.cuda.device(col.device):
        check(lib.ctgcn_slot_reorder(n, K, ptr(row_ptr), ptr(col), ptr(val), ptr(level), ptr(table), table.numel(),
                                     ptr(col2), ptr(val2), ptr(slot2), _stream()), "ctgcn_slot_reorder")
    return col2, val2, slot2


def spmm_csr(row_ptr, col, val, x, out=None, accumulate=False):
    _need_cuda(row_ptr, col, val, x)
    lib = _lib.load()
    if x.dtype != torch.float32:
        raise TypeError("fp32 features expected")
    x = x if x.stride(-1) == 1 else x.contiguous()
    n = row_ptr.numel() - 1
    d = x.shape[1]
    if out is None:
        out = torch.empty(n, d, dtype=torch.float32, device=x.device)
        accumulate = False
    with torch.cuda.device(x.device):
        check(lib.ctgcn_spmm_csr_f32(n, d, ptr(row_ptr), ptr(col), ptr(val), ptr(x), x.stride(0), ptr(out), out.stride(0),
                                     1 if accumulate else 0, _stream()), "ctgcn_spmm_csr_f32")
    return out


def _transpose_bias(src, bias):
    lib = _lib.load()
    d, n = src.shape
    w = src if src.stride(1) == 1 else src.contiguous()
    out = torch.empty(n, d, dtype=torch.float32, device=src.device)
    with torch.cuda.device(src.device):
        check(lib.ctgcn_transpose_bias_f32(n, d, ptr(w), w.stride(0), ptr(bias.contiguous() if bias is not None else None),
                                           ptr(out), out.stride(0), _stream()), "ctgcn_transpose_bias_f32")
    return out


class _LinearOfIdentity(torch.autograd.Function):

    @staticmethod
    def forward(ctx, weight, bias):
        ctx.has_bias = bias is not None
        return _transpose_bias(weight.detach(), None if bias is None else bias.detach())

    @staticmethod
    def backward(ctx, dout):
        if dout.shape[0] > 64 * 65535:
            dw = dout.t().contiguous()
        else:
            dw = _transpose_bias(dout if dout.stride(1) == 1 else dout.contiguous(), None)
        return dw, (dout.sum(0) if ctx.has_bias else None)


def linear_of_identity(weight, bias):
    _need_cuda(weight)
    if torch.is_grad_enabled() and (weight.requires_grad or (bias is not None and bias.requires_grad)):
        return _LinearOfIdentity.apply(weight, bias)
    return _transpose_bias(weight.detach(), None if bias is None else bias.detach())


def _hub_pieces(lib, adj, long_rows, slots, d, device, transposed=False):
    split = adj.hub_split(transposed) if long_rows is not None else 1
    if split <= 1:
        return 1, None, 0
    nbytes = int(lib.ctgcn_hub_workspace_bytes(long_rows.numel(), split, slots, d))
    return split, torch.empty(nbytes, dtype=torch.uint8, device=device), nbytes


def _aggregate_fwd(adj, x, relu):
    lib = _lib.load()
    n, d = x.shape
    H = torch.empty(n, adj.K, d, dtype=torch.float32, device=x.device)
    flags = adj.flags | (_lib.F_RELU if relu else 0)
    with torch.cuda.device(x.device), _timed("agg_fwd", n=n, d=d, K=adj.K, nnz=adj.nnz):
        long_rows = adj.long_rows()
        split, hub_ws, hub_bytes = _hub_pieces(lib, adj, long_rows, adj.K, d, x.device)
        check(lib.ctgcn_core_aggregate_f32(n, d, adj.K, ptr(adj.row_ptr), ptr(adj.col), ptr(adj.val), ptr(adj.slot), ptr(x),
                                           x.stride(0), ptr(H), flags, ptr(long_rows), 0 if long_rows is None else long_rows.numel(),
                                           adj.LONG_ROW, split, ptr(hub_ws), hub_bytes, _stream()), "ctgcn_core_aggregate_f32")
    return H


def _aggregate_gather(adj, Z, S0, relu):
    lib = _lib.load()
    n, K, d = Z.shape
    flags = adj.flags | (_lib.F_RELU if relu else 0)
    dX = torch.empty(n, d, dtype=torch.float32, device=Z.device)
    t_ptr, t_col, t_val, t_slot = adj.transposed()
    long_rows = adj.long_rows(transposed=True)
    split, hub_ws, hub_bytes = _hub_pieces(lib, adj, long_rows, 1, d, Z.device, transposed=True)
    with torch.cuda.device(Z.device), _timed("agg_bwd", n=n, d=d, K=K, nnz=adj.nnz):
        check(lib.ctgcn_core_aggregate_bwd_f32(n, d, K, ptr(t_ptr), ptr(t_col), ptr(t_val), ptr(t_slot), ptr(Z), ptr(S0),
                                               ptr(dX), d, flags, ptr(long_rows), 0 if long_rows is None else long_rows.numel(),
                                               adj.LONG_ROW, split, ptr(hub_ws), hub_bytes, _stream()), "ctgcn_core_aggregate_bwd_f32")
    return dX


def _aggregate_bwd(adj, H, dH, relu):
    lib = _lib.load()
    n, K, d = dH.shape
    flags = adj.flags | (_lib.F_RELU if relu else 0)
    Z = torch.empty_like(dH)
    S0 = torch.empty(n, d, dtype=torch.float32, device=dH.device) if adj.self_loop else None
    with torch.cuda.device(dH.device), _timed("agg_bwd_prep", n=n, d=d, K=K, self_loop=adj.self_loop):
        check(lib.ctgcn_core_aggregate_bwd_prep_f32(n, d, K, ptr(dH), ptr(H), ptr(Z), ptr(S0), flags, _stream()),
              "ctgcn_core_aggregate_bwd_prep_f32")
    return _aggregate_gather(adj, Z, S0, relu)


class _CoreAggregate(torch.autograd.Function):
    @staticmethod
    def forward(ctx, x, adj, relu):
        H = _aggregate_fwd(adj, x, relu)
        ctx.adj, ctx.relu = adj, relu
        ctx.save_for_backward(H)
        return H

    @staticmethod
    def backward(ctx, dH):
        (H,) = ctx.saved_tensors
        dH = dH.contiguous()
        return _aggregate_bwd(ctx.adj, H, dH, ctx.relu), None, None


def core_aggregate(x, adj, relu=True):
    _need_cuda(x, adj.col)
    if adj.K < 1:
        raise ValueError("empty k-core adjacency list")
    if x.dim() != 2 or x.shape[0] != adj.n:
        raise ValueError("features must be [%d, d], got %s" % (adj.n, tuple(x.shape)))
    if x.dtype != torch.float32:
        raise TypeError("fp32 features expected")
    if x.device != adj.device:
        raise ValueError("features on %s but adjacency on %s" % (x.device, adj.device))
    x = x if x.stride(1) == 1 else x.contiguous()
    return _CoreAggregate.apply(x, adj, relu)


import os as _os
_GI_MAX_ELEMS = int(_os.environ.get("CTGCN_GI_MAX_ELEMS", 1 << 30))


def gru_fused_ok(rnn, seq):
    return (isinstance(rnn, torch.nn.GRU) and rnn.hidden_size == 128 and rnn.num_layers == 1 and not rnn.bidirectional
            and rnn.batch_first and seq.is_cuda and seq.dtype == torch.float32)


def _gru_bias(rnn, hid):
    if not rnn.bias:
        return None, None
    b_ih, b_hh = rnn.bias_ih_l0, rnn.bias_hh_l0

    def fold():
        both = torch.empty(4 * hid, dtype=b_ih.dtype, device=b_ih.device)
        both[: 3 * hid] = b_ih.detach()
        both[: 2 * hid] += b_hh.detach()[: 2 * hid]
        both[3 * hid:] = b_hh.detach()[2 * hid:]
        return both
    if plane_cache_enabled() and not b_ih.is_inference() and not b_hh.is_inference():
        tag = (b_hh.data_ptr(), b_hh._version)

        def make():
            both = fold()
            both._ctgcn_tag = tag
            return both, 16 * hid
        both = _plane_cache.get(b_ih, "gru_bias", make)
        if getattr(both, "_ctgcn_tag", None) != tag:
            _plane_cache.forget(b_ih, "gru_bias")
            both = _plane_cache.get(b_ih, "gru_bias", make)
    else:
        both = fold()
    return both[: 3 * hid], both[3 * hid:]


def _row_chunks(lib, rows, steps, hid):
    if rows <= 0:
        return [(0, 0)]
    granule = int(lib.ctgcn_gru_row_granule())
    max_rows = max(granule, (_GI_MAX_ELEMS // (steps * 4 * hid)) // granule * granule)
    n_chunks = -(-rows // max_rows)
    chunk = -(-(-(-rows // n_chunks)) // granule) * granule
    return [(lo, min(chunk, rows - lo)) for lo in range(0, rows, chunk)]


def split_mfma_enabled():
    import os
    return os.environ.get("CTGCN_FP32_MFMA_ONLY", "0") != "1"


def layer_kernel_enabled(reduce_sum=True):
    import os
    mode = os.environ.get("CTGCN_GRU_LAYER", "1")
    if mode == "0":
        return False
    return bool(reduce_sum) or mode != "sum"


def forward_split_mode():
    import os
    if not split_mfma_enabled():
        return 0
    return 1 if os.environ.get("CTGCN_GRU_SPLIT", "f16x2") == "bf16x3" else 2


_LINEAR_WS_MAX = 2 << 30


def linear_split_enabled():
    import os
    return forward_split_mode() == 2 and os.environ.get("CTGCN_LINEAR_SPLIT", "1") != "0"


def linear_split_ok(x2d, weight):
    return (linear_split_enabled() and x2d.is_cuda and x2d.dtype == torch.float32 and weight.dtype == torch.float32 and x2d.dim() == 2
            and x2d.stride(1) == 1 and weight.stride(1) == 1 and x2d.data_ptr() % 4 == 0 and weight.data_ptr() % 4 == 0
            and x2d.shape[0] > 0 and x2d.shape[1] >= 32 and x2d.stride(0) >= x2d.shape[1] and weight.stride(0) >= weight.shape[1])


class _PlaneCache(object):
# ... 297 lines not shown
    rows, steps, d_in = seq.shape
    hid = w_hh.shape[1]
    if out is None:
        out = torch.empty((rows, hid) if reduce_sum else (rows, steps, hid), dtype=torch.float32, device=seq.device)
    elif not (reduce_sum and out.shape == (rows, hid) and out.dtype == torch.float32 and out.stride(1) == 1
              and out.stride(0) % 2 == 0 and out.stride(0) >= hid and out.device == seq.device):
        raise ValueError("gru: out must be a [rows, %d] fp32 view with unit column stride (reduce_sum only)" % hid)
    ldo = out.stride(0) if reduce_sum else 0
    if rows == 0:
        return out
    split = forward_split_mode()
    if split == 2 and d_in == hid and layer_kernel_enabled(reduce_sum) and seq.stride(2) == 1 and seq.stride(1) % 4 == 0 \
            and seq.stride(0) == steps * seq.stride(1) and seq.data_ptr() % 16 == 0 and w_ih.is_contiguous():
        with torch.cuda.device(seq.device), _timed("gru_layer", rows=rows, steps=steps, reduce_sum=bool(reduce_sum)):
            check(lib.ctgcn_gru_layer_f32(rows, steps, d_in, hid, ptr(seq), seq.stride(1), ptr(w_ih), ptr(w_hh), ptr(bias), ptr(b_hn),
                                          ptr(ln_w), ptr(ln_b), eps, 1 if reduce_sum else 0, ptr(out), ldo, None, None, 0, _stream()), "ctgcn_gru_layer_f32")
        return out
    chunks = _row_chunks(lib, rows, steps, hid)
    gi_buf = _gi_buffer(chunks[0][1], steps, hid, seq.device)
    with torch.cuda.device(seq.device):
        for lo, n in chunks:
            blocked = _project(seq[lo:lo + n].reshape(n * steps, d_in), w_ih, bias, gi_buf, steps_blocked=steps)
            with _timed("gru_seq", rows=n, steps=steps):
                check(lib.ctgcn_gru_seq_f32(n, steps, hid, ptr(gi_buf), ptr(w_hh), ptr(b_hn), ptr(ln_w), ptr(ln_b), eps,
                                            1 if reduce_sum else 0, ptr(out[lo:lo + n]), ldo, None, split, 1 if blocked else 0,
                                            None, None, None, _stream()), "ctgcn_gru_seq_f32")
        if keep_gi is not None and len(chunks) == 1:
            keep_gi.append((gi_buf, blocked))
    return out


def gru_steps_scattered_ok(rnn, base, steps=None):
    import os
    return ((steps is None or 1 <= steps <= 32) and gru_fused_ok(rnn, base) and rnn.input_size == rnn.hidden_size and forward_split_mode() == 2 and layer_kernel_enabled(False)
            and os.environ.get("CTGCN_GRU_LAYER_WAVES", "8") != "4" and rnn.weight_ih_l0.is_contiguous()
            and not (torch.is_grad_enabled() and any(p.requires_grad for p in rnn.parameters())))


def gru_sequence_scattered(rnn, norm, base, step_offsets, ld_row, rows):
    lib = _lib.load()
    steps, hid = int(step_offsets.numel()), rnn.hidden_size
    bias, b_hn = _gru_bias(rnn, hid)
    ln_w = None if norm is None else norm.weight
    ln_b = None if norm is None else norm.bias
    eps = 0.0 if norm is None else float(norm.eps)
    out = torch.empty(rows, steps, hid, dtype=torch.float32, device=base.device)
    if rows == 0:
        return out
    with torch.cuda.device(base.device), _timed("gru_layer", rows=rows, steps=steps, reduce_sum=False):
        check(lib.ctgcn_gru_layer_f32(rows, steps, hid, hid, ptr(base), hid, ptr(rnn.weight_ih_l0.detach()), ptr(rnn.weight_hh_l0.detach().contiguous()),
                                      ptr(bias), ptr(b_hn), ptr(ln_w), ptr(ln_b), eps, 0, ptr(out), 0, None, ptr(step_offsets), int(ld_row), _stream()),
              "ctgcn_gru_layer_f32")
    return out


def aggregate_split_enabled():
    import os
    return linear_split_enabled() and os.environ.get("CTGCN_AGG_SPLIT", "1") != "0"


_AGG_SPLIT_MAX = 16 << 30


def aggregate_split_ok(rnn, x, adj):
    if not aggregate_split_enabled() or x.dim() != 2 or not gru_fused_ok(rnn, x) or x.shape[0] != adj.n or x.device != adj.device:
        return False
    if torch.is_grad_enabled() and (x.requires_grad or any(p.requires_grad for p in rnn.parameters())):
        return False
    d, hid = x.shape[1], rnn.hidden_size
    if d % 4 or d < 32 or d > 512 or x.stride(1) != 1 or x.stride(0) % 4 or x.data_ptr() % 16 or adj.K < 1 or adj.n < 1:
        return False
    if d == hid:
        return layer_kernel_enabled(True) and adj.n * adj.K * (d * 4 + 4) <= _AGG_SPLIT_MAX and rnn.weight_ih_l0.is_contiguous()
    if adj.n * adj.K * (-(-d // 64) * 64 * 4 + 4) > _LINEAR_WS_MAX:
        return False
    return len(_row_chunks(_lib.load(), adj.n, adj.K, hid)) == 1


def row_plan_enabled():
    import os
    return os.environ.get("CTGCN_DEDUP", "1") != "0"


def aggregate_split_planes(x, adj, n_out, plan=None, ws=None):
    lib = _lib.load()
    n, d = x.shape
    flags = adj.flags | _lib.F_RELU
    long_rows = adj.long_rows()
    n_long = 0 if long_rows is None else long_rows.numel()
    ws_bytes = int(lib.ctgcn_core_aggregate_split_workspace_bytes(n, d, adj.K, n_out, n_long))
    if ws is None:
        ws = torch.empty(ws_bytes, dtype=torch.uint8, device=x.device)
    compact = plan is not None and not (d == 128 and n_out == 1)
    if plan is not None and plan["tile"] != (adj.PLAN_TILE_GEMM if compact else adj.PLAN_TILE):
        raise ValueError("aggregate_split_planes: plan tile %d does not belong to this consumer" % plan["tile"])
    hub_dest = adj.plan_row_dest(plan, long_rows, compact) if (plan is not None and n_long) else None
    split, hub_ws, hub_bytes = _hub_pieces(lib, adj, long_rows, adj.K, d, x.device)
    with _timed("agg_fwd", n=n, d=d, K=adj.K, nnz=adj.nnz, split=True, rows_written=(plan["new_rows"] if plan is not None else n * adj.K)):
        check(lib.ctgcn_core_aggregate_split_f32(n, d, adj.K, ptr(adj.row_ptr), ptr(adj.col), ptr(adj.val), ptr(adj.slot), ptr(x), x.stride(0),
                                                 flags, ptr(long_rows), n_long, adj.LONG_ROW, n_out,
                                                 ptr(plan["order"]) if plan is not None else None, ptr(plan["tile_mask"]) if plan is not None else None,
                                                 ptr(plan["tile_base"]) if compact else None, plan["operand_rows"] if compact else 0,
                                                 ptr(hub_dest), split, ptr(hub_ws), hub_bytes, ptr(ws), ws_bytes, _stream()), "ctgcn_core_aggregate_split_f32")
    return ws, ws_bytes


def gru_layer_presplit(ws, n, K, rnn, norm, out, plan=None):
    lib = _lib.load()
    hid = rnn.hidden_size
    bias, b_hn = _gru_bias(rnn, hid)
    w_ih, w_hh = rnn.weight_ih_l0.detach(), rnn.weight_hh_l0.detach().contiguous()
    ln_w = None if norm is None else norm.weight
    ln_b = None if norm is None else norm.bias
    eps = 0.0 if norm is None else float(norm.eps)
    with _timed("gru_layer", rows=n, steps=K, reduce_sum=True, presplit=True, new_rows=(plan["new_rows"] if plan is not None else n * K)):
        check(lib.ctgcn_gru_layer_presplit_f32(n, K, hid, ptr(ws), ptr(w_ih), ptr(w_hh), ptr(bias), ptr(b_hn), ptr(ln_w), ptr(ln_b), eps,
                                               ptr(out), out.stride(0), ptr(plan["order"]) if plan is not None else None,
                                               ptr(plan["tile_mask"]) if plan is not None else None, _stream()), "ctgcn_gru_layer_presplit_f32")
    return out


def core_diffusion_split(x, adj, rnn, norm, out=None):
    lib = _lib.load()
    n, d = x.shape
    K, hid = adj.K, rnn.hidden_size
    n_out = 3 * hid
    if out is None:
        out = torch.empty(n, hid, dtype=torch.float32, device=x.device)
    elif not (out.shape == (n, hid) and out.dtype == torch.float32 and out.stride(1) == 1 and out.stride(0) % 2 == 0
              and out.stride(0) >= hid and out.device == x.device):
        raise ValueError("core_diffusion_split: out must be a [rows, %d] fp32 view with unit column stride" % hid)
    with torch.cuda.device(x.device):
        if d == hid:
            plan = adj.row_plan() if row_plan_enabled() else None
            ws, _ = aggregate_split_planes(x, adj, 1, plan)
            return gru_layer_presplit(ws, n, K, rnn, norm, out, plan)
        bias, b_hn = _gru_bias(rnn, hid)
        w_ih, w_hh = rnn.weight_ih_l0.detach(), rnn.weight_hh_l0.detach().contiguous()
        ln_w = None if norm is None else norm.weight
        ln_b = None if norm is None else norm.bias
        eps = 0.0 if norm is None else float(norm.eps)
        plan = adj.row_plan(adj.PLAN_TILE_GEMM) if (row_plan_enabled() and forward_split_mode() == 2) else None
        rows = plan["operand_rows"] if plan is not None else n * K
        ws, ws_bytes = aggregate_split_planes(x, adj, n_out, plan)
        gi_buf = torch.empty(rows * n_out, dtype=torch.float32, device=x.device) if plan is not None else _gi_buffer(n, K, hid, x.device)
        with _timed("linear_split", rows=rows, k=d, n_out=n_out, presplit=True):
            if plane_cache_enabled():
                wp = _plane_cache.packed(rnn.weight_ih_l0, lib)
                check(lib.ctgcn_linear_packed_f32(rows, n_out, d, ptr(ws), ptr(wp), ptr(bias), _lib.ACT_NONE, ptr(gi_buf), n_out, _stream()),
                      "ctgcn_linear_packed_f32")
            else:
                check(lib.ctgcn_linear_presplit_f32(rows, n_out, d, ptr(w_ih), w_ih.stride(0), ptr(bias), ptr(gi_buf), n_out, ptr(ws), ws_bytes,
                                                    _stream()), "ctgcn_linear_presplit_f32")
        with _timed("gru_seq", rows=n, steps=K):
            check(lib.ctgcn_gru_seq_f32(n, K, hid, ptr(gi_buf), ptr(w_hh), ptr(b_hn), ptr(ln_w), ptr(ln_b), eps, 1, ptr(out), out.stride(0),
                                        None, forward_split_mode(), 0, ptr(plan["order"]) if plan is not None else None,
                                        ptr(plan["tile_mask"]) if plan is not None else None, ptr(plan["tile_base"]) if plan is not None else None,
                                        _stream()), "ctgcn_gru_seq_f32")
    return out


def train_fused_enabled():
    import os
    return os.environ.get("CTGCN_TRAIN_FUSED", "1") != "0"


def core_diffusion_fused_ok(rnn, norm, x, adj):
    if not train_fused_enabled() or not aggregate_split_enabled() or not layer_kernel_enabled(True) or forward_split_mode() != 2:
        return False
    if x.dim() != 2 or not gru_fused_ok(rnn, x) or x.shape[0] != adj.n or x.device != adj.device or not isinstance(norm, torch.nn.LayerNorm):
        return False
    if not norm.elementwise_affine or norm.bias is None:
        return False
    d, hid = x.shape[1], rnn.hidden_size
    if d != hid or rnn.input_size != hid or x.stride(1) != 1 or x.stride(0) % 4 or x.data_ptr() % 16 or adj.K < 1 or adj.K > 64 or adj.n < 1:
        return False
    return bool(adj.symmetric) and adj.n * adj.K * (d * 4 + 4) <= _AGG_SPLIT_MAX and rnn.weight_ih_l0.is_contiguous()


def _u32ptr(t, offset=0):
    return None if t is None else t.data_ptr() + 4 * int(offset)


_kept_planes = {"bytes": 0, "budget": int(float(_os.environ.get("CTGCN_TRAIN_PLANES_GB", "32")) * (1 << 30))}


def _release_planes(nbytes):
    _kept_planes["bytes"] -= nbytes


class _CoreDiffusionFused(torch.autograd.Function):

    @staticmethod
    def forward(ctx, x, adj, w_ih, w_hh, b_ih, b_hh, ln_w, ln_b, eps):
        lib = _lib.load()
        n, K, hid = adj.n, adj.K, w_hh.shape[1]
        plan = adj.row_plan() if row_plan_enabled() else None
        x_d = x.detach()
        with torch.cuda.device(x.device):
            ws, _ = aggregate_split_planes(x_d, adj, 1, plan)
            bias, b_hn = _fold_gru_bias(b_ih, b_hh, hid)
            out = torch.empty(n, hid, dtype=torch.float32, device=x.device)
            with _timed("gru_layer", rows=n, steps=K, reduce_sum=True, presplit=True, new_rows=(plan["new_rows"] if plan is not None else n * K)):
                check(lib.ctgcn_gru_layer_presplit_f32(n, K, hid, ptr(ws), ptr(w_ih.detach()), ptr(w_hh.detach().contiguous()), ptr(bias), ptr(b_hn),
                                                       ptr(ln_w.detach()), ptr(ln_b.detach()), eps, ptr(out), out.stride(0),
                                                       ptr(plan["order"]) if plan is not None else None,
                                                       ptr(plan["tile_mask"]) if plan is not None else None, _stream()), "ctgcn_gru_layer_presplit_f32")
        ctx.adj, ctx.plan, ctx.eps = adj, plan, eps
        nbytes = ws.numel()
        keep = _kept_planes["bytes"] + nbytes <= _kept_planes["budget"]
        ctx.kept = keep
        if keep:
            import weakref
            _kept_planes["bytes"] += nbytes
            weakref.finalize(ws, _release_planes, nbytes)
        ctx.save_for_backward(ws if keep else x_d, w_ih, w_hh, b_ih, b_hh, ln_w, ln_b)
        return out

    @staticmethod
    def backward(ctx, dout):
        lib = _lib.load()
        ws, w_ih, w_hh, b_ih, b_hh, ln_w, ln_b = ctx.saved_tensors
        if not ctx.kept:
            with torch.cuda.device(ws.device):
                ws, _ = aggregate_split_planes(ws, ctx.adj, 1, ctx.plan)
        adj, plan, eps = ctx.adj, ctx.plan, ctx.eps
        n, K, hid = adj.n, adj.K, w_hh.shape[1]
        dev = ws.device
        w_ih_d, w_hh_d = w_ih.detach(), w_hh.detach().contiguous()
        bias, b_hn = _fold_gru_bias(b_ih, b_hh, hid)
        if not (dout.dim() == 2 and dout.stride(1) == 1 and dout.stride(0) >= hid and dout.stride(0) % 2 == 0 and dout.data_ptr() % 8 == 0):
            dout = dout.contiguous()
        order = plan["order"] if plan is not None else None
        tmask = plan["tile_mask"] if plan is not None else None
        chunks = _row_chunks(lib, n, K, hid)
        cmax = chunks[0][1]
        nb = int(lib.ctgcn_gru_bwd_blocks(cmax))
        with torch.cuda.device(dev):
            gates = torch.empty(cmax * K, 3 * hid, dtype=torch.float32, device=dev)
            hseq = torch.empty(cmax * K, hid, dtype=torch.float32, device=dev)
            presum = torch.empty(cmax, hid, dtype=torch.float32, device=dev)
            dpre = torch.empty(cmax, hid, dtype=torch.float32, device=dev)
            dgi = torch.empty(cmax * K, 3 * hid, dtype=torch.float32, device=dev)
            dw_hh_part = torch.zeros(nb, 3 * hid, hid, dtype=torch.float32, device=dev)
            dw_ih_part = torch.zeros(nb, 3 * hid, hid, dtype=torch.float32, device=dev)
            dbn_part = torch.zeros(nb, hid, dtype=torch.float32, device=dev)
            dbi_part = torch.zeros(nb, 3 * hid, dtype=torch.float32, device=dev)
            ln_part = torch.empty(2048, 2 * hid, dtype=torch.float32, device=dev)
            ln_sum = torch.zeros(2 * hid, dtype=torch.float32, device=dev)
            Z = torch.empty(n, K, hid, dtype=torch.float32, device=dev)
            S0 = torch.empty(n, hid, dtype=torch.float32, device=dev) if adj.self_loop else None
            for lo, cnt in chunks:
                tm = _u32ptr(tmask, (lo // 16) * (2 if K > 32 else 1))
                od = _u32ptr(order, lo)
                fresh = (plan["new_rows"] / float(n * K)) if plan is not None else 1.0
                with _timed("gru_layer", rows=cnt, steps=K, reduce_sum=True, presplit=True, save=True, new_rows=int(cnt * K * fresh)):
                    check(lib.ctgcn_gru_layer_presplit_save_f32(cnt, K, hid, ptr(ws), n * K, lo, ptr(w_ih_d), ptr(w_hh_d), ptr(bias), ptr(b_hn), tm,
                                                                ptr(gates), ptr(hseq), ptr(presum), _stream()), "ctgcn_gru_layer_presplit_save_f32")
                dy = dout if order is not None else dout[lo:lo + cnt]
                check(lib.ctgcn_layernorm_bwd_f32(cnt, 1, hid, ptr(presum), ptr(dy), dy.stride(0), ptr(ln_w.detach()), eps, ptr(dpre), ptr(ln_part),
                                                  ln_part.shape[0], od, _stream()), "ctgcn_layernorm_bwd_f32")
                ln_sum += ln_part.sum(0)
                with _timed("gru_bwd_rec", rows=cnt, steps=K, fresh=fresh, per_step=False):
                    check(lib.ctgcn_gru_bwd_rec_f32(cnt, K, hid, ptr(gates), 3, ptr(hseq), ptr(dpre), None, ptr(w_hh_d), tm, ptr(dgi), ptr(dw_hh_part),
                                                    ptr(dbn_part), nb, 1, _stream()), "ctgcn_gru_bwd_rec_f32")
                with _timed("gru_bwd_in", rows=cnt, steps=K, fresh=fresh, z_out=True):
                    check(lib.ctgcn_gru_bwd_in_f32(cnt, K, hid, ptr(dgi), ptr(w_ih_d), tm, ptr(ws), n * K, lo, None, 0, None,
                                                   ptr(Z) if order is not None else ptr(Z[lo:]),
                                                   ptr(S0) if (S0 is None or order is not None) else ptr(S0[lo:]), od, 1 if adj.nested else 0,
                                                   ptr(dw_ih_part), ptr(dbi_part), nb, 1, _stream()), "ctgcn_gru_bwd_in_f32")
            dX = _aggregate_gather(adj, Z, S0, True) if ctx.needs_input_grad[0] else None
        dw_ih = dw_ih_part.sum(0)
        dw_hh = dw_hh_part.sum(0)
        db_ih = db_hh = None
        if b_ih is not None:
            db_ih = dbi_part.sum(0)
            db_hh = torch.cat([db_ih[: 2 * hid], dbn_part.sum(0)])
        return dX, None, dw_ih, dw_hh, db_ih, db_hh, ln_sum[:hid].clone(), ln_sum[hid:].clone(), None


def _fold_gru_bias(b_ih, b_hh, hid):
    if b_ih is None:
        return None, None
    bias = b_ih.detach().clone()
    bias[: 2 * hid] += b_hh.detach()[: 2 * hid]
    return bias, b_hh.detach()[2 * hid:].contiguous()


def core_diffusion_fused(x, adj, rnn, norm):
    b_ih = rnn.bias_ih_l0 if rnn.bias else None
    b_hh = rnn.bias_hh_l0 if rnn.bias else None
    return _CoreDiffusionFused.apply(x, adj, rnn.weight_ih_l0, rnn.weight_hh_l0, b_ih, b_hh, norm.weight, norm.bias, float(norm.eps))


_GROUP_MAX_NODES = 200_000


def _compute_units(dev):
    with torch.cuda.device(dev):
        return int(_lib.load().ctgcn_compute_units())


class _GroupTables(object):

    SLAB_BYTES = 8 << 20

    def __init__(self, limit=1024):
        import collections
        self.limit, self.entries = limit, collections.OrderedDict()
        self.slabs = {}
        self.misses = {}

    def _carve(self, dev, nbytes):
        key = str(dev)
        need = -(-nbytes // 256) * 256
        slab = self.slabs.get(key)
        if slab is None or slab[1] + need > slab[0].numel():
            if slab is not None:
                for k in [k for k in self.entries if k[2] == key]:
                    del self.entries[k]
                self._retire(slab[0])
            slab = self.slabs[key] = [torch.empty(max(self.SLAB_BYTES, need), dtype=torch.uint8, device=dev), 0]
        view = slab[0][slab[1]: slab[1] + need]
        slab[1] += need
        return view

    def get(self, lib, site, groups, dev, desc=b""):
        nbytes = int(lib.ctgcn_group_table_bytes(groups))
        if torch.cuda.is_current_stream_capturing():
            return torch.empty(nbytes, dtype=torch.uint8, device=dev), None, nbytes
        key = (site, groups, str(dev), torch.cuda.current_stream(dev).cuda_stream, hash(desc))
        e = self.entries.get(key)
        if e is None:
            self.misses[site] = self.misses.get(site, 0) + 1
            if len(self.entries) >= self.limit:
                self.entries.clear()
                for old in self.slabs.values():
                    self._retire(old[0])
                self.slabs.clear()
            e = self.entries[key] = (self._carve(dev, nbytes), ctypes.create_string_buffer(nbytes))
        else:
            self.entries.move_to_end(key)
        return e[0], e[1], nbytes

    def _retire(self, slab):
        torch.cuda.synchronize(slab.device)

    def clear(self):
        for old in self.slabs.values():
            self._retire(old[0])
        self.entries.clear()
        self.slabs.clear()


_group_tables = _GroupTables()


def group_launch_enabled():
    import os
    return os.environ.get("CTGCN_GROUP", "1") != "0"


def core_diffusion_group_ok(xs, adjs, rnns, norms):
    if not group_launch_enabled() or len(xs) < 2 or not xs[0].is_cuda or len(xs) > _compute_units(xs[0].device):
        return False
    n = adjs[0].n
    if n > _GROUP_MAX_NODES:
        return False
    planned = None
    for x, adj, rnn, norm in zip(xs, adjs, rnns, norms):
        if adj.n != n or x.dim() != 2 or x.shape[1] != 128 or rnn.hidden_size != 128 or not aggregate_split_ok(rnn, x, adj):
            return False
        if adj.K > 32 or adj.long_rows() is not None or not isinstance(norm, torch.nn.LayerNorm) or norm.weight is None or norm.bias is None:
            return False
        p = (adj.row_plan() is not None) if row_plan_enabled() else False
# ... 2778 lines not shown
```

include/ctgcn_hip.h:

```cpp
#ifndef CTGCN_HIP_H
#define CTGCN_HIP_H

#include <stddef.h>
#include <stdint.h>

#ifdef __cplusplus
extern "C" {
#endif

#define CTGCN_ABI_VERSION 31

enum {
    CTGCN_OK = 0,
    CTGCN_E_INVALID = -1,
    CTGCN_E_HIP = -2,
    CTGCN_E_WORKSPACE = -3,
    CTGCN_E_UNSUPPORTED = -4,
    CTGCN_E_LIMIT = -5
};

enum {
    CTGCN_F_SELF_LOOP = 1,
    CTGCN_F_RELU = 2,
    CTGCN_F_NESTED = 4
};

enum {
    CTGCN_OP_KCORE = 1,
    CTGCN_OP_INGEST = 2
};

#define CTGCN_MAX_SLOTS 255

#define CTGCN_SPLIT_NONE 0
#define CTGCN_SPLIT_BF16X3 1
#define CTGCN_SPLIT_F16X2 2
#define CTGCN_ACT_NONE 0
#define CTGCN_ACT_SELU 1

int ctgcn_abi_version(void);
const char *ctgcn_last_error(void);

int ctgcn_device_info(char *name_host, size_t name_len, int *cu_count_host);

int ctgcn_transpose_bias_f32(int64_t n, int32_t d, const float *w, int64_t ldw, const float *bias, float *out, int64_t ldo,
                             void *stream);

int ctgcn_spmm_csr_f32(int64_t n_rows, int32_t d, const int32_t *row_ptr, const int32_t *col_idx,
                       const float *val, const float *X, int64_t ldx, float *Y, int64_t ldy,
                       int accumulate, void *stream);

size_t ctgcn_hub_workspace_bytes(int32_t n_long, int32_t hub_split, int32_t slots, int32_t d);
int32_t ctgcn_hub_split_entries(void);
int ctgcn_core_aggregate_f32(int64_t n_rows, int32_t d, int32_t K, const int32_t *row_ptr,
                             const int32_t *col_idx, const float *val, const uint8_t *slot,
                             const float *X, int64_t ldx, float *H, uint32_t flags,
                             const int32_t *long_rows, int32_t n_long, int32_t long_threshold,
                             int32_t hub_split, void *hub_workspace, size_t hub_workspace_bytes, void *stream);

int ctgcn_core_aggregate_bwd_prep_f32(int64_t n_rows, int32_t d, int32_t K, const float *dH,
                                      const float *H, float *Z, float *S0, uint32_t flags,
                                      void *stream);
int ctgcn_core_aggregate_bwd_f32(int64_t n_rows, int32_t d, int32_t K, const int32_t *row_ptr,
                                 const int32_t *col_idx, const float *val, const uint8_t *slot,
                                 const float *Z, const float *S0, float *dX, int64_t lddx,
                                 uint32_t flags, const int32_t *long_rows, int32_t n_long,
                                 int32_t long_threshold, int32_t hub_split, void *hub_workspace, size_t hub_workspace_bytes,
                                 void *stream);

int ctgcn_edges_to_csr(int64_t n, int64_t m, const int32_t *src, const int32_t *dst, const float *w,
                       int32_t *row_ptr, int32_t *col_idx, float *val, int64_t *nnz_host,
                       void *workspace, size_t workspace_bytes, void *stream);

int ctgcn_kcore_i32(int64_t n, const int32_t *row_ptr, const int32_t *col_idx, int32_t *core,
                    void *workspace, size_t workspace_bytes, int32_t level_cap, int32_t *max_core_host,
                    void *stream);

int ctgcn_edge_levels_i32(int64_t n, const int32_t *row_ptr, const int32_t *col_idx,
                          const float *val, const int32_t *core, int32_t *level,
                          int64_t *count, double *wsum, int32_t hist_len, void *stream);

int ctgcn_slot_reorder(int64_t n, int32_t K, const int32_t *row_ptr, const int32_t *col_idx,
                       const float *val, const int32_t *level, const uint8_t *slot_of_level,
                       int32_t table_len, int32_t *col_out, float *val_out, uint8_t *slot_out,
                       void *stream);

int ctgcn_gru_seq_f32(int64_t rows, int32_t steps, int32_t hidden, const float *gi, const float *w_hh,
                      const float *b_hn, const float *ln_weight, const float *ln_bias, float ln_eps,
                      int reduce_sum, float *out, int64_t ld_out, float *gates_out, int split_bf16, int gi_blocked,
                      const int32_t *row_order, const uint32_t *tile_mask, const int32_t *tile_base, void *stream);

int ctgcn_layernorm_bwd_f32(int64_t rows, int32_t steps, int32_t hidden, const float *h, const float *dy, int64_t ld_dy, const float *gamma, float eps,
                            float *dx, float *partial, int32_t n_partial, const int32_t *dy_rows, void *stream);

int ctgcn_lstm_seq_f32(int64_t rows, int32_t steps, int32_t hidden, const float *gi, const float *w_hh,
                       const float *ln_weight, const float *ln_bias, float ln_eps, int reduce_sum, float *out,
                       float *gates_out, void *stream);
int ctgcn_lstm_seq_bwd_f32(int64_t rows, int32_t steps, int32_t hidden, const float *gates, const float *dh_seq, const float *dh_sum,
                           const float *w_hh, float *d_gi, float *bias_partial, int32_t n_partial, void *stream);

int ctgcn_gru_layer_f32(int64_t rows, int32_t steps, int32_t d_in, int32_t hidden, const float *x, int64_t ldx, const float *w_ih,
                        const float *w_hh, const float *bias_gi, const float *b_hn, const float *ln_weight, const float *ln_bias,
                        float ln_eps, int reduce_sum, float *out, int64_t ld_out, float *gates_out,
                        const int64_t *step_offsets, int64_t ld_row, void *stream);

int ctgcn_gru_layer_presplit_f32(int64_t rows, int32_t steps, int32_t hidden, const void *planes, const float *w_ih, const float *w_hh,
                                 const float *bias_gi, const float *b_hn, const float *ln_weight, const float *ln_bias, float ln_eps,
                                 float *out, int64_t ld_out, const int32_t *row_order, const uint32_t *tile_mask, void *stream);

int32_t ctgcn_gru_bwd_blocks(int64_t rows);
int ctgcn_gru_layer_presplit_save_f32(int64_t rows, int32_t steps, int32_t hidden, const void *planes, int64_t plane_rows, int64_t first_row,
                                      const float *w_ih, const float *w_hh, const float *bias_gi, const float *b_hn, const uint32_t *tile_mask,
                                      float *gates_out, float *hseq_out, float *presum_out, void *stream);
int ctgcn_gru_bwd_rec_f32(int64_t rows, int32_t steps, int32_t hidden, const float *gates, int32_t gate_count, const float *h_seq, const float *dh_sum,
                          const float *dh_seq, const float *w_hh, const uint32_t *tile_mask, float *d_gi, float *dw_partial,
                          float *dbn_partial, int32_t n_partial, int32_t accumulate, void *stream);
int ctgcn_gru_bwd_in_f32(int64_t rows, int32_t steps, int32_t hidden, const float *d_gi, const float *w_ih, const uint32_t *tile_mask,
                         const void *x_planes, int64_t plane_rows, int64_t first_row, const float *x, int64_t ldx, float *dx, float *Z, float *S0,
                         const int32_t *row_order, int32_t nested, float *dw_partial, float *dbi_partial, int32_t n_partial,
                         int32_t accumulate, void *stream);

typedef struct {
    const int32_t *row_ptr, *col_idx;
    const float *val;
    const uint8_t *slot;
    const float *X;
    int64_t ldx;
    int32_t K;
    uint32_t flags;
    const int32_t *row_order;
    const uint32_t *tile_mask;
    void *workspace;
    size_t workspace_bytes;
    void *planes1, *planes2;
    float *scales;
    const int32_t *tile_base;
} ctgcn_agg_split_group_t;
typedef struct {
    const void *planes;
    const float *w_ih, *w_hh, *bias_gi, *b_hn, *ln_weight, *ln_bias;
    float ln_eps;
    int32_t steps;
    float *out;
    int64_t ld_out;
    const int32_t *row_order;
    const uint32_t *tile_mask;
    int64_t work;
} ctgcn_gru_layer_group_t;
typedef struct {
    const float *gi;
    const float *w_hh, *b_hn, *ln_weight, *ln_bias;
    float ln_eps;
    int32_t steps;
    float *out;
    int64_t ld_out;
    const int32_t *row_order;
    const uint32_t *tile_mask;
    const int32_t *tile_base;
    int64_t work;
} ctgcn_gru_seq_group_t;
size_t ctgcn_group_table_bytes(int32_t groups);
uint64_t ctgcn_table_uploads(int current);
int ctgcn_transpose_bias_group_f32(int32_t groups, int64_t n, int32_t d, const float *const *w, int64_t ldw, const float *const *bias, float *const *out,
                                   int64_t ldo, void *table, size_t table_bytes, void *shadow, void *stream);
int ctgcn_gru_seq_group_f32(int32_t groups, int64_t rows, int32_t hidden, const ctgcn_gru_seq_group_t *g, void *table, size_t table_bytes, void *shadow,
                            void *stream);
int ctgcn_core_aggregate_split_group_f32(int32_t groups, int64_t n_rows, int32_t d, const ctgcn_agg_split_group_t *g, void *table, size_t table_bytes,
                                         void *shadow, void *stream);
int ctgcn_gru_layer_presplit_group_f32(int32_t groups, int64_t rows, int32_t hidden, const ctgcn_gru_layer_group_t *g, void *table, size_t table_bytes,
                                       void *shadow, void *stream);

size_t ctgcn_linear_workspace_bytes(int64_t rows, int32_t n_out, int32_t k);
size_t ctgcn_split_planes_bytes(int64_t rows, int32_t k);
size_t ctgcn_pack_weight_bytes(int32_t n_out, int32_t k);
int ctgcn_split_rows_f32(int64_t rows, int32_t k, const float *x, int64_t ldx, void *planes, size_t planes_bytes, void *stream);
int ctgcn_pack_weight_f32(int32_t n_out, int32_t k, const float *w, int64_t ldw, void *packed, size_t packed_bytes, void *stream);
int ctgcn_linear_packed_f32(int64_t rows, int32_t n_out, int32_t k, const void *x_planes, const void *w_packed, const float *bias,
                            int32_t activation, float *y, int64_t ldy, void *stream);
int ctgcn_linear_packed_chain_f32(int64_t rows, int32_t n_out, int32_t k, const void *x_planes, const void *w_packed, const float *bias, int32_t activation,
                                  void *out_planes, size_t out_planes_bytes, void *stream);
int ctgcn_linear_packed_group_f32(int32_t groups, int64_t total_rows, int32_t n_out, int32_t k, const void *planes1, const void *planes2,
                                  const float *scales, const int32_t *panel_group, const void *const *w_packed, const float *const *bias,
                                  int32_t activation, float *y, int64_t ldy, void *table, size_t table_bytes, void *shadow, void *stream);
int ctgcn_linear_f32(int64_t rows, int32_t n_out, int32_t k, const float *x, int64_t ldx, const float *w, int64_t ldw, const float *bias,
                     int32_t activation, float *y, int64_t ldy, void *workspace, size_t workspace_bytes, void *stream);

size_t ctgcn_core_aggregate_split_workspace_bytes(int64_t n_rows, int32_t d, int32_t K, int32_t n_out, int32_t n_long);
int ctgcn_core_aggregate_split_f32(int64_t n_rows, int32_t d, int32_t K, const int32_t *row_ptr, const int32_t *col_idx,
                                   const float *val, const uint8_t *slot, const float *X, int64_t ldx, uint32_t flags,
                                   const int32_t *long_rows, int32_t n_long, int32_t long_threshold, int32_t n_out,
                                   const int32_t *row_order, const uint32_t *tile_mask, const int32_t *tile_base, int64_t operand_rows,
                                   const int32_t *hub_row_dest,
                                   int32_t hub_split, void *hub_workspace, size_t hub_workspace_bytes,
                                   void *workspace, size_t workspace_bytes, void *stream);
int ctgcn_linear_presplit_f32(int64_t rows, int32_t n_out, int32_t k, const float *w, int64_t ldw, const float *bias, float *y, int64_t ldy,
                              void *workspace, size_t workspace_bytes, void *stream);

int ctgcn_gru_seq_bwd_f32(int64_t rows, int32_t steps, int32_t hidden, const float *gates, const float *h_seq,
                          const float *dh_seq, const float *dh_sum, const float *w_hh, float *d_gi, float *d_ghn,
                          float *bias_partial, int32_t n_partial, int split_bf16, void *stream);

int ctgcn_gru_input_proj_f32(int64_t rows, int32_t d_in, int32_t hidden, const float *x, int64_t ldx,
                             const float *w_ih, const float *bias, float *gi, int split_mode, int32_t steps_blocked, void *stream);

int ctgcn_gru_input_grad_f32(int64_t rows, int32_t d_in, int32_t hidden, const float *d_gi, const float *w_ih, float *d_x,
                             int64_t ldx, void *stream);

int ctgcn_gru_weight_grad_f32(int64_t rows, int32_t steps, int32_t hidden, const float *g01, int64_t ldg01, const float *g2,
                              int64_t ldg2, const float *x, int64_t ldx, int shift_steps, float *partial, int32_t n_pairs,
                              int accumulate, void *stream);

int64_t ctgcn_gru_row_granule(void);
int32_t ctgcn_compute_units(void);

int ctgcn_row_cumsum_f32(int64_t n, const int32_t *row_ptr, const float *val, float *cumw, void *stream);
int ctgcn_random_walk_pairs(int64_t n, const int32_t *row_ptr, const int32_t *col_idx, const float *cumw,
                            int32_t walk_length, int32_t walk_time, int32_t first_walk, uint64_t seed, int weighted,
                            int32_t *pair_src, int32_t *pair_dst, int64_t *freq, void *stream);

int ctgcn_neg_sampling_indices(int64_t batch, const int64_t *batch_nodes, const int32_t *pair_row_ptr,
                               const int32_t *pair_col, int32_t num, int64_t table_len, const int32_t *neg_table,
                               uint64_t seed, const int64_t *offsets, int64_t *node_out, int64_t *pos_out,
                               int64_t *neg_out, int64_t *scratch, void *stream);

size_t ctgcn_epoch_scan_workspace_bytes(int64_t positions);
int ctgcn_neg_sampling_offsets_batched(int64_t positions, const int64_t *perm, const int32_t *pair_row_ptr, int32_t num,
                                       int64_t batch_size, int64_t *offsets, int64_t *batch_offsets, void *workspace,
                                       size_t workspace_bytes, void *stream);
int ctgcn_neg_sampling_indices_batched(int64_t positions, const int64_t *perm, int64_t batch_size, const uint64_t *seeds,
                                       const int32_t *pair_row_ptr, const int32_t *pair_col, int32_t num, int64_t table_len,
                                       const int32_t *neg_table, const int64_t *offsets, int64_t *node_out, int64_t *pos_out,
                                       int64_t *neg_out, int64_t *scratch, void *stream);

size_t ctgcn_negsampling_loss_workspace_bytes(int64_t positions, int64_t samples, int64_t batch_size, int32_t d);
int ctgcn_negsampling_loss_fwd_bwd_f32(int64_t positions, int64_t batch_size, int64_t samples, int32_t d, int32_t num, float Q,
                                       const float *E, int64_t lde, const int64_t *offsets, const int64_t *node_idx,
                                       const int64_t *pos_idx, const int64_t *neg_idx, const int64_t *pos_sorted,
                                       const int64_t *pos_order, const int64_t *neg_sorted, const int64_t *neg_order,
                                       double *loss_out, float *dE, int64_t ldg, void *workspace, size_t workspace_bytes,
                                       void *stream);

size_t ctgcn_reconstruction_loss_workspace_bytes(int64_t positions);
int ctgcn_reconstruction_loss_fwd_bwd_f32(int64_t positions, int64_t batch_size, int32_t d, const int64_t *rows, const float *S,
                                          int64_t lds, const float *E, int64_t lde, double *loss_out, float *dS, int64_t ldds,
                                          float *dE, int64_t ldde, void *workspace, size_t workspace_bytes, void *stream);

int ctgcn_write_embedding_tsv(const char *path_host, int64_t n, int32_t d, const float *data_host, int64_t ld,
                              const char *names_blob_host, const int64_t *name_offsets_host, char sep,
                              int32_t threads);

int ctgcn_lp_neg_sample(int64_t count, int64_t n_nodes, const int64_t *keys, int64_t n_keys, uint64_t seed, int64_t max_attempts,
                        int64_t *from_out, int64_t *to_out, int32_t *flag, void *stream);
size_t ctgcn_lp_grad_workspace_bytes(int64_t n, int32_t d, int32_t models);
int ctgcn_lp_grad_f32(int64_t n, int32_t d, int32_t models, uint32_t measures, int64_t n_nodes, const float *E, int64_t lde,
                      const int64_t *src, const int64_t *dst, const uint8_t *label, double w_neg, double w_pos, const float *W,
                      double *loss_out, double *grad_out, void *workspace, size_t workspace_bytes, void *stream);
size_t ctgcn_lp_hess_workspace_bytes(int64_t n, int32_t d, int32_t models);
int ctgcn_lp_hess_f32(int64_t n, int32_t d, int32_t models, uint32_t measures, int64_t n_nodes, const float *E, int64_t lde,
                      const int64_t *src, const int64_t *dst, const uint8_t *label, double w_neg, double w_pos, const float *W,
                      double *hess_out, void *workspace, size_t workspace_bytes, void *stream);
int ctgcn_lp_scores_f32(int64_t n, int32_t d, int32_t models, uint32_t measures, int64_t n_nodes, const float *E, int64_t lde,
                        const int64_t *src, const int64_t *dst, const float *W, float *score_out, void *stream);

size_t ctgcn_cent_brandes_workspace_bytes(int64_t n, int64_t s0, int64_t s1);
int ctgcn_cent_brandes(int64_t n, const int32_t *row_ptr, const int32_t *col, int64_t s0, int64_t s1, double *bc_out,
                       int64_t *r_out, int64_t *D_out, void *workspace, size_t workspace_bytes, void *stream);
size_t ctgcn_cent_eigenvector_workspace_bytes(int64_t n);
int ctgcn_cent_eigenvector(int64_t n, const int32_t *row_ptr, const int32_t *col, int32_t max_iter, double tol, double *x_out,
                           int32_t *stop_step, void *workspace, size_t workspace_bytes, void *stream);
size_t ctgcn_ridge_gram_workspace_bytes(int32_t d, int32_t targets, int32_t folds);
int ctgcn_ridge_gram_f32(int64_t n, int32_t d, int32_t targets, int32_t folds, const float *X, int64_t ldx, const double *Y,
                         double *gram_out, void *workspace, size_t workspace_bytes, void *stream);
int ctgcn_ridge_gram_f64(int64_t n, int32_t d, int32_t targets, int32_t folds, const double *X, int64_t ldx, const double *Y,
                         double *gram_out, void *workspace, size_t workspace_bytes, void *stream);
size_t ctgcn_ridge_sse_workspace_bytes(int32_t models, int32_t folds);
int ctgcn_ridge_sse_f32(int64_t n, int32_t d, int32_t targets, int32_t folds, int32_t models, const float *X, int64_t ldx,
                        const double *Y, const double *W, const int32_t *target_of, double *sse_out, void *workspace,
// ... 257 lines not shown
```

Before: 11.07 billion edges/s.

## Fuse one-hot transform bias into core aggregation gather using transposed weight

With one-hot features, the transform layer's output for node j is simply column j of the weight plus the bias. The change adds bias-aware aggregation kernels that gather rows of the transposed weight directly and add the bias on the fly in the forward, hub and final kernels. This is meant to skip materialising the n-by-hid transform output (a GEMM or gather plus a write) and read a small weight table in its place. The cost is an extra vector add per gathered edge, new template variants (including U=3 and U=8 split kernels), and gradient plumbing for the bias through dX.sum.

```diff
diff --git a/ctgcn_amd/_lib.py b/ctgcn_amd/_lib.py
--- a/ctgcn_amd/_lib.py
+++ b/ctgcn_amd/_lib.py
@@ -40,6 +40,7 @@
     "ctgcn_hub_workspace_bytes": (_sz, [_i32, _i32, _i32, _i32]),
     "ctgcn_hub_split_entries": (_i32, []),
     "ctgcn_core_aggregate_f32": (_int, [_i64, _i32, _i32, _vp, _vp, _vp, _vp, _vp, _i64, _vp, _u32, _vp, _i32, _i32, _i32, _vp, _sz, _vp]),
+    "ctgcn_core_aggregate_bias_f32": (_int, [_i64, _i32, _i32, _vp, _vp, _vp, _vp, _vp, _vp, _vp, _u32, _vp, _i32, _i32, _i32, _vp, _sz, _vp]),
     "ctgcn_core_aggregate_bwd_prep_f32": (_int, [_i64, _i32, _i32, _vp, _vp, _vp, _vp, _u32, _vp]),
     "ctgcn_core_aggregate_bwd_f32": (_int, [_i64, _i32, _i32, _vp, _vp, _vp, _vp, _vp, _vp, _vp, _i64, _u32, _vp, _i32, _i32, _i32, _vp, _sz, _vp]),
     "ctgcn_edges_to_csr": (_int, [_i64, _i64, _vp, _vp, _vp, _vp, _vp, _vp, _c.POINTER(_i64), _vp, _sz, _vp]),
@@ -72,6 +73,7 @@
     "ctgcn_linear_f32": (_int, [_i64, _i32, _i32, _vp, _i64, _vp, _i64, _vp, _i32, _vp, _i64, _vp, _sz, _vp]),
     "ctgcn_core_aggregate_split_workspace_bytes": (_sz, [_i64, _i32, _i32, _i32, _i32]),
     "ctgcn_core_aggregate_split_f32": (_int, [_i64, _i32, _i32, _vp, _vp, _vp, _vp, _vp, _i64, _u32, _vp, _i32, _i32, _i32, _vp, _vp, _vp, _i64, _vp, _i32, _vp, _sz, _vp, _sz, _vp]),
+    "ctgcn_core_aggregate_split_bias_f32": (_int, [_i64, _i32, _i32, _vp, _vp, _vp, _vp, _vp, _vp, _u32, _vp, _i32, _i32, _i32, _vp, _vp, _vp, _i64, _vp, _i32, _vp, _sz, _vp, _sz, _vp]),
     "ctgcn_gru_layer_presplit_f32": (_int, [_i64, _i32, _i32, _vp, _vp, _vp, _vp, _vp, _vp, _vp, _c.c_float, _vp, _i64, _vp, _vp, _vp]),
     "ctgcn_linear_presplit_f32": (_int, [_i64, _i32, _i32, _vp, _i64, _vp, _vp, _i64, _vp, _sz, _vp]),
     "ctgcn_gru_seq_bwd_f32": (_int, [_i64, _i32, _i32, _vp, _vp, _vp, _vp, _vp, _vp, _vp, _vp, _i32, _int, _vp]),
diff --git a/ctgcn_amd/csrc/ctgcn_hip.hip b/ctgcn_amd/csrc/ctgcn_hip.hip
--- a/ctgcn_amd/csrc/ctgcn_hip.hip
+++ b/ctgcn_amd/csrc/ctgcn_hip.hip
@@ -74,9 +74,10 @@
     const uint32_t *tmask;
     int32_t tile_shift;
     const int32_t *tbase;
+    const float *gather_bias;
 };
 
-template <int VEC, int LPR, int U>
+template <int VEC, int LPR, int U, bool BIAS = false>
 __global__ __launch_bounds__(256) void agg_fwd_kernel(const AggArgs a)
 {
     using V = typename vec_of<VEC>::type;
@@ -97,7 +98,12 @@
         const bool live = ch < a.chunks;
         const int64_t foff = live ? (int64_t)ch * VEC : 0;
         V R = vzero<VEC>(), P = vzero<VEC>();
-        if (self) R = *(const V *)(X + row * a.ldsrc + foff);
+        V bv = vzero<VEC>();
+        if constexpr (BIAS) bv = *(const V *)(a.gather_bias + foff);
+        if (self) {
+            R = *(const V *)(X + row * a.ldsrc + foff);
+            if constexpr (BIAS) R += bv;
+        }
         int cur = 0;
 
         auto close_slot = [&]() {
@@ -137,6 +143,7 @@
 #pragma unroll
                 for (int u = 0; u < U; ++u) {
                     while (cur < sj[u]) close_slot();
+                    if constexpr (BIAS) xv[u] += bv;
                     P = vfma(wj[u], xv[u], P);
                 }
             }
@@ -144,8 +151,9 @@
                 const int cj = __shfl(c, j, LPR);
                 const float w1 = __shfl(w, j, LPR);
                 const int s1 = __shfl(s, j, LPR);
-                const V x1 = *(const V *)(X + (int64_t)cj * a.ldsrc + foff);
+                V x1 = *(const V *)(X + (int64_t)cj * a.ldsrc + foff);
                 while (cur < s1) close_slot();
+                if constexpr (BIAS) x1 += bv;
                 P = vfma(w1, x1, P);
             }
         }
@@ -217,7 +225,7 @@
     return np < 1 ? 1 : (np > max_pieces ? max_pieces : np);
 }
 
-template <int VEC, int LPR, int U>
+template <int VEC, int LPR, int U, bool BIAS = false>
 __global__ __launch_bounds__(HUB_THREADS) void agg_fwd_hub_kernel(const AggArgs a)
 {
     using V = typename vec_of<VEC>::type;
@@ -247,6 +255,8 @@
         const int ch = pass * LPR + lig;
         const bool live = ch < a.chunks;
         const int64_t foff = live ? (int64_t)ch * VEC : 0;
+        V bv = vzero<VEC>();
+        if constexpr (BIAS) bv = *(const V *)(a.gather_bias + foff);
         if (grp < G) {
             for (int k = 0; k < a.K; ++k) part[((int64_t)grp * a.K + k) * LPR + lig] = vzero<VEC>();
             V P = vzero<VEC>();
@@ -276,6 +286,7 @@
                             P = vzero<VEC>();
                             cur = sj[u];
                         }
+                        if constexpr (BIAS) xv[u] += bv;
                         P = vfma(wj[u], xv[u], P);
                     }
                 }
@@ -283,12 +294,13 @@
                     const int cj = __shfl(c, j, LPR);
                     const float w1 = __shfl(w, j, LPR);
                     const int s1 = __shfl(s, j, LPR);
-                    const V x1 = *(const V *)(X + (int64_t)cj * a.ldsrc + foff);
+                    V x1 = *(const V *)(X + (int64_t)cj * a.ldsrc + foff);
                     if (s1 != cur) {
                         if (cur >= 0) part[((int64_t)grp * a.K + cur) * LPR + lig] = P;
                         P = vzero<VEC>();
                         cur = s1;
                     }
+                    if constexpr (BIAS) x1 += bv;
                     P = vfma(w1, x1, P);
                 }
             }
@@ -308,7 +320,10 @@
         }
         if (grp == 0) {
             V R = vzero<VEC>(), Pc = vzero<VEC>();
-            if (self) R = *(const V *)(X + row * a.ldsrc + foff);
+            if (self) {
+                R = *(const V *)(X + row * a.ldsrc + foff);
+                if constexpr (BIAS) R += bv;
+            }
             for (int k = 0; k < a.K; ++k) {
                 V sk = vzero<VEC>();
                 for (int g = 0; g < G; ++g) sk += part[((int64_t)g * a.K + k) * LPR + lig];
@@ -410,7 +425,7 @@
     }
 }
 
-template <int VEC, bool FWD>
+template <int VEC, bool FWD, bool BIAS = false>
 __global__ __launch_bounds__(256) void agg_hub_final_kernel(const AggArgs a)
 {
     using V = typename vec_of<VEC>::type;
@@ -425,7 +440,10 @@
         if (FWD) {
             float *__restrict__ outrow = a.out + (a.hub_compact ? (int64_t)hub : row) * a.out_ld;
             V R = vzero<VEC>(), Pc = vzero<VEC>();
-            if (self) R = *(const V *)(a.src + row * a.ldsrc + foff);
+            if (self) {
+                R = *(const V *)(a.src + row * a.ldsrc + foff);
+                if constexpr (BIAS) R += *(const V *)(a.gather_bias + foff);
+            }
             for (int k = 0; k < a.K; ++k) {
                 V sk = vzero<VEC>();
                 for (int p = 0; p < np; ++p) sk += *(const V *)(mine + ((int64_t)p * a.K + k) * a.hub_ld + foff);
@@ -503,14 +521,14 @@
 
 constexpr size_t HUB_LDS_BUDGET = 144 * 1024;
 
-template <bool FWD, int VEC, int LPR>
+template <bool FWD, int VEC, int LPR, bool BIAS = false>
 void launch_agg_t(AggArgs a, hipStream_t st)
 {
     constexpr int U = 4;
     const int rows_per_block = 256 / LPR;
     const int64_t blocks = (a.n + rows_per_block - 1) / rows_per_block;
     if (FWD)
-        hipLaunchKernelGGL((agg_fwd_kernel<VEC, LPR, U>), dim3((unsigned)blocks), dim3(256), 0, st, a);
+        hipLaunchKernelGGL((agg_fwd_kernel<VEC, LPR, U, BIAS>), dim3((unsigned)blocks), dim3(256), 0, st, a);
     else
         hipLaunchKernelGGL((agg_bwd_kernel<VEC, LPR, U>), dim3((unsigned)blocks), dim3(256), 0, st, a);
     if (a.n_long > 0) {
@@ -521,14 +539,14 @@
         const size_t lds = per_group * G;
         const unsigned hub_grid = (unsigned)a.n_long * (unsigned)(a.hub_part ? a.hub_split : 1);
         if (FWD) {
-            auto k = agg_fwd_hub_kernel<VEC, LPR, U>;
+            auto k = agg_fwd_hub_kernel<VEC, LPR, U, BIAS>;
             if (lds > 64 * 1024) (void)hipFuncSetAttribute(reinterpret_cast<const void *>(k), hipFuncAttributeMaxDynamicSharedMemorySize, (int)lds);
             hipLaunchKernelGGL(k, dim3(hub_grid), dim3(HUB_THREADS), lds, st, a);
         } else {
             auto k = agg_bwd_hub_kernel<VEC, LPR, U>;
             hipLaunchKernelGGL(k, dim3(hub_grid), dim3(HUB_THREADS), lds, st, a);
         }
-        if (a.hub_part) hipLaunchKernelGGL((agg_hub_final_kernel<VEC, FWD>), dim3((unsigned)a.n_long), dim3(256), 0, st, a);
+        if (a.hub_part) hipLaunchKernelGGL((agg_hub_final_kernel<VEC, FWD, BIAS>), dim3((unsigned)a.n_long), dim3(256), 0, st, a);
     }
 }
 
@@ -559,7 +577,7 @@
     if (a.n_long > 0 && (size_t)a.K * p.lpr * (p.vec * 4) > HUB_LDS_BUDGET) { a.n_long = 0; a.long_thresh = 0x7fffffff; }
     const int64_t rows_per_block = 256 / p.lpr;
     if ((a.n + rows_per_block - 1) / rows_per_block > 0x7fffffffLL) return fail(CTGCN_E_UNSUPPORTED, "grid too large");
-#define CASE(V, L) if (p.vec == V && p.lpr == L) { launch_agg_t<FWD, V, L>(a, st); }
+#define CASE(V, L) if (p.vec == V && p.lpr == L) { if (FWD && a.gather_bias) launch_agg_t<FWD, V, L, FWD>(a, st); else launch_agg_t<FWD, V, L>(a, st); }
     CASE(4, 8) else CASE(4, 16) else CASE(4, 32) else CASE(4, 64)
     else CASE(1, 8) else CASE(1, 16) else CASE(1, 32) else CASE(1, 64)
 #undef CASE
@@ -1534,7 +1552,7 @@
     return __uint_as_float(u);
 }
 
-template <int LPR, int CH, int U, bool WIDE = false>
+template <int LPR, int CH, int U, bool WIDE = false, bool BIAS = false>
 __device__ __forceinline__ void agg_fwd_split_body(const AggArgs &a, _Float16 *__restrict__ p1, _Float16 *__restrict__ p2,
                                                    float *__restrict__ scale, int32_t kp, float residual_scale, const int64_t bid)
 {
@@ -1565,13 +1583,19 @@
     bool live[CH];
     int64_t foff[CH];
     f4 R[CH], P[CH];
+    f4 bv[CH];
 #pragma unroll
     for (int c = 0; c < CH; ++c) {
         const int ch = c * LPR + lig;
         live[c] = ch < a.chunks;
         foff[c] = live[c] ? (int64_t)ch * 4 : 0;
         R[c] = P[c] = vzero<4>();
-        if (self && live[c]) R[c] = *(const f4 *)(X + row * a.ldsrc + foff[c]);
+        bv[c] = vzero<4>();
+        if constexpr (BIAS) bv[c] = *(const f4 *)(a.gather_bias + foff[c]);
+        if (self && live[c]) {
+            R[c] = *(const f4 *)(X + row * a.ldsrc + foff[c]);
+            if constexpr (BIAS) R[c] += bv[c];
+        }
     }
     int cur = 0;
 
@@ -1642,7 +1666,10 @@
             for (int u = 0; u < U; ++u) {
                 while (cur < sj[u]) close_slot();
 #pragma unroll
-                for (int q = 0; q < CH; ++q) P[q] = vfma(wj[u], xv[u][q], P[q]);
+                for (int q = 0; q < CH; ++q) {
+                    if constexpr (BIAS) xv[u][q] += bv[q];
+                    P[q] = vfma(wj[u], xv[u][q], P[q]);
+                }
             }
         }
         for (; j < cnt; ++j) {
@@ -1654,22 +1681,35 @@
             for (int q = 0; q < CH; ++q) x1[q] = *(const f4 *)(X + (int64_t)cj * a.ldsrc + foff[q]);
             while (cur < s1) close_slot();
 #pragma unroll
-            for (int q = 0; q < CH; ++q) P[q] = vfma(w1, x1[q], P[q]);
+            for (int q = 0; q < CH; ++q) {
+                if constexpr (BIAS) x1[q] += bv[q];
+                P[q] = vfma(w1, x1[q], P[q]);
+            }
         }
     }
     while (cur < a.K) close_slot();
 }
 
-template <int LPR, int CH, int U, bool WIDE = false>
+template <int LPR, int CH, int U, bool WIDE = false, bool BIAS = false>
 __global__ __launch_bounds__(256) void agg_fwd_split_kernel(const AggArgs a, _Float16 *__restrict__ p1, _Float16 *__restrict__ p2,
                                                             float *__restrict__ scale, int32_t kp, float residual_scale)
 {
-    agg_fwd_split_body<LPR, CH, U, WIDE>(a, p1, p2, scale, kp, residual_scale, blockIdx.x);
+    agg_fwd_split_body<LPR, CH, U, WIDE, BIAS>(a, p1, p2, scale, kp, residual_scale, blockIdx.x);
 }
 __global__ __launch_bounds__(256) __attribute__((amdgpu_waves_per_eu(7, 8))) void agg_fwd_split32_kernel(
     const AggArgs a, _Float16 *__restrict__ p1, _Float16 *__restrict__ p2, float *__restrict__ scale, int32_t kp, float residual_scale)
 {
     agg_fwd_split_body<32, 1, 4>(a, p1, p2, scale, kp, residual_scale, blockIdx.x);
+}
+__global__ __launch_bounds__(256) __attribute__((amdgpu_waves_per_eu(7, 8))) void agg_fwd_split32_bias_kernel(
+    const AggArgs a, _Float16 *__restrict__ p1, _Float16 *__restrict__ p2, float *__restrict__ scale, int32_t kp, float residual_scale)
+{
+    agg_fwd_split_body<32, 1, 3, false, true>(a, p1, p2, scale, kp, residual_scale, blockIdx.x);
+}
+__global__ __launch_bounds__(256) void agg_fwd_split32_u8_bias_kernel(
+    const AggArgs a, _Float16 *__restrict__ p1, _Float16 *__restrict__ p2, float *__restrict__ scale, int32_t kp, float residual_scale)
+{
+    agg_fwd_split_body<32, 1, 8, false, true>(a, p1, p2, scale, kp, residual_scale, blockIdx.x);
 }
 __global__ __launch_bounds__(256) void agg_fwd_split32_u8_kernel(
     const AggArgs a, _Float16 *__restrict__ p1, _Float16 *__restrict__ p2, float *__restrict__ scale, int32_t kp, float residual_scale)
@@ -3800,11 +3840,11 @@
     return launch_agg<true>(a, v4, (hipStream_t)stream);
 }
 
-int ctgcn_core_aggregate_f32(int64_t n_rows, int32_t d, int32_t K, const int32_t *row_ptr,
-                             const int32_t *col_idx, const float *val, const uint8_t *slot,
-                             const float *X, int64_t ldx, float *H, uint32_t flags,
-                             const int32_t *long_rows, int32_t n_long, int32_t long_threshold,
-                             int32_t hub_split, void *hub_workspace, size_t hub_workspace_bytes, void *stream)
+static int core_aggregate_(int64_t n_rows, int32_t d, int32_t K, const int32_t *row_ptr,
+                           const int32_t *col_idx, const float *val, const uint8_t *slot,
+                           const float *X, int64_t ldx, const float *gather_bias, float *H, uint32_t flags,
+                           const int32_t *long_rows, int32_t n_long, int32_t long_threshold,
+                           int32_t hub_split, void *hub_workspace, size_t hub_workspace_bytes, void *stream)
 {
     if (n_rows < 0 || d <= 0 || ldx < d) return fail(CTGCN_E_INVALID, "core_aggregate: bad sizes n=%lld d=%d ldx=%lld", (long long)n_rows, d, (long long)ldx);
     if (K < 1 || K > CTGCN_MAX_SLOTS) return fail(CTGCN_E_INVALID, "core_aggregate: K=%d outside [1,%d]", K, CTGCN_MAX_SLOTS);
@@ -3816,11 +3856,32 @@
     a.row_ptr = row_ptr; a.col = col_idx; a.val = val; a.slot = slot;
     a.src = X; a.ldsrc = ldx; a.self = nullptr; a.out = H; a.out_ld = (int64_t)K * d;
     a.flags = flags; a.accumulate = 0;
+    a.gather_bias = gather_bias;
     a.long_rows = long_rows; a.n_long = n_long; a.long_thresh = long_threshold;
     if (n_long > 0 && long_threshold < 1) return fail(CTGCN_E_INVALID, "core_aggregate: long_threshold must be >= 1");
     if (int rc = set_hub_pieces(a, K, hub_split, hub_workspace, hub_workspace_bytes, "core_aggregate")) return rc;
-    const bool v4 = (d % 4 == 0) && (ldx % 4 == 0) && ctgcn_aligned16(X) && ctgcn_aligned16(H);
+    const bool v4 = (d % 4 == 0) && (ldx % 4 == 0) && ctgcn_aligned16(X) && ctgcn_aligned16(H) && (!gather_bias || ctgcn_aligned16(gather_bias));
     return launch_agg<true>(a, v4, (hipStream_t)stream);
+}
+
+int ctgcn_core_aggregate_f32(int64_t n_rows, int32_t d, int32_t K, const int32_t *row_ptr,
+                             const int32_t *col_idx, const float *val, const uint8_t *slot,
+                             const float *X, int64_t ldx, float *H, uint32_t flags,
+                             const int32_t *long_rows, int32_t n_long, int32_t long_threshold,
+                             int32_t hub_split, void *hub_workspace, size_t hub_workspace_bytes, void *stream)
+{
+    return core_aggregate_(n_rows, d, K, row_ptr, col_idx, val, slot, X, ldx, nullptr, H, flags, long_rows, n_long, long_threshold,
+                           hub_split, hub_workspace, hub_workspace_bytes, stream);
+}
+
+int ctgcn_core_aggregate_bias_f32(int64_t n_rows, int32_t d, int32_t K, const int32_t *row_ptr,
+                                  const int32_t *col_idx, const float *val, const uint8_t *slot,
+                                  const float *Wt, const float *gather_bias, float *H, uint32_t flags,
+                                  const int32_t *long_rows, int32_t n_long, int32_t long_threshold,
+                                  int32_t hub_split, void *hub_workspace, size_t hub_workspace_bytes, void *stream)
+{
+    return core_aggregate_(n_rows, d, K, row_ptr, col_idx, val, slot, Wt, d, gather_bias, H, flags, long_rows, n_long, long_threshold,
+                           hub_split, hub_workspace, hub_workspace_bytes, stream);
 }
 
 size_t ctgcn_core_aggregate_split_workspace_bytes(int64_t n_rows, int32_t d, int32_t K, int32_t n_out, int32_t n_long)
@@ -3829,13 +3890,13 @@
     return ctgcn_linear_workspace_bytes((n_rows + 63) / 64 * 64 * K, n_out, d) + ((size_t)n_long * K * d * 4 + 255) / 256 * 256;
 }
 
-int ctgcn_core_aggregate_split_f32(int64_t n_rows, int32_t d, int32_t K, const int32_t *row_ptr, const int32_t *col_idx,
-                                   const float *val, const uint8_t *slot, const float *X, int64_t ldx, uint32_t flags,
-                                   const int32_t *long_rows, int32_t n_long, int32_t long_threshold, int32_t n_out,
-                                   const int32_t *row_order, const uint32_t *tile_mask, const int32_t *tile_base, int64_t operand_rows,
-                                   const int32_t *hub_row_dest,
-                                   int32_t hub_split, void *hub_workspace, size_t hub_workspace_bytes,
-                                   void *workspace, size_t workspace_bytes, void *stream)
+static int core_aggregate_split_(int64_t n_rows, int32_t d, int32_t K, const int32_t *row_ptr, const int32_t *col_idx,
+                                 const float *val, const uint8_t *slot, const float *X, int64_t ldx, const float *gather_bias,
+                                 uint32_t flags, const int32_t *long_rows, int32_t n_long, int32_t long_threshold, int32_t n_out,
+                                 const int32_t *row_order, const uint32_t *tile_mask, const int32_t *tile_base, int64_t operand_rows,
+                                 const int32_t *hub_row_dest,
+                                 int32_t hub_split, void *hub_workspace, size_t hub_workspace_bytes,
+                                 void *workspace, size_t workspace_bytes, void *stream)
 {
     if (n_rows < 0 || d <= 0 || ldx < d || n_out < 1) return fail(CTGCN_E_INVALID, "core_aggregate_split: bad sizes n=%lld d=%d ldx=%lld", (long long)n_rows, d, (long long)ldx);
     if (K < 1 || K > CTGCN_MAX_SLOTS) return fail(CTGCN_E_INVALID, "core_aggregate_split: K=%d outside [1,%d]", K, CTGCN_MAX_SLOTS);
@@ -3844,6 +3905,7 @@
     if (!slot && K != 1) return fail(CTGCN_E_INVALID, "core_aggregate_split: slot tags required when K > 1");
     if ((d & 3) || d > 512 || (ldx & 3) || !ctgcn_aligned16(X) || (reinterpret_cast<uintptr_t>(workspace) & 255u))
         return fail(CTGCN_E_UNSUPPORTED, "core_aggregate_split: needs d %% 4 == 0, d <= 512, 16-byte aligned rows, 256-byte aligned workspace");
+    if (gather_bias && !ctgcn_aligned16(gather_bias)) return fail(CTGCN_E_UNSUPPORTED, "core_aggregate_split: gather_bias must be 16-byte aligned");
     if (n_long < 0 || (n_long > 0 && (!long_rows || long_threshold < 1))) return fail(CTGCN_E_INVALID, "core_aggregate_split: bad hub row list");
     if ((row_order == nullptr) != (tile_mask == nullptr)) return fail(CTGCN_E_INVALID, "core_aggregate_split: row_order and tile_mask come together");
     if (row_order && K > 64) return fail(CTGCN_E_UNSUPPORTED, "core_aggregate_split: a row plan needs K <= 64");
@@ -3868,6 +3930,7 @@
     a.flags = flags; a.accumulate = 0;
     a.long_rows = long_rows; a.n_long = n_long; a.long_thresh = long_threshold;
     a.order = row_order; a.tmask = tile_mask; a.tbase = tile_base; a.tile_shift = tile_base ? 6 : 4;
+    a.gather_bias = gather_bias;
     const AggPlan p = plan_for(d, true);
     a.chunks = p.chunks;
     a.passes = p.passes;
@@ -3880,6 +3943,19 @@
     const float rsc = 1.f;
     static const int force_u8 = [] { const char *e = getenv("CTGCN_AGG_U8"); return e ? atoi(e) : -1; }();
     const bool u8 = force_u8 >= 0 ? force_u8 != 0 : n_rows <= 200000;
+#define SPLIT_LAUNCH(kernel) hipLaunchKernelGGL(kernel, dim3((unsigned)blocks), dim3(256), 0, st, a, p1, p2, scale, kp, rsc)
+    if (gather_bias) {
+        if (row_order && K > 32) {
+            if (p.chunks <= 32) SPLIT_LAUNCH((agg_fwd_split_kernel<32, 1, 8, true, true>));
+            else if (p.chunks <= 64) SPLIT_LAUNCH((agg_fwd_split_kernel<64, 1, 8, true, true>));
+            else SPLIT_LAUNCH((agg_fwd_split_kernel<64, 2, 8, true, true>));
+        } else if (p.chunks <= 32 && u8) SPLIT_LAUNCH(agg_fwd_split32_u8_bias_kernel);
+        else if (p.chunks <= 32) SPLIT_LAUNCH(agg_fwd_split32_bias_kernel);
+        else if (p.chunks <= 64) SPLIT_LAUNCH((agg_fwd_split_kernel<64, 1, 4, false, true>));
+        else if (n_rows <= 200000) SPLIT_LAUNCH((agg_fwd_split_kernel<64, 2, 8, false, true>));
+        else SPLIT_LAUNCH((agg_fwd_split_kernel<64, 2, 4, false, true>));
+    } else
+#undef SPLIT_LAUNCH
     if (row_order && K > 32) {
         if (p.chunks <= 32) hipLaunchKernelGGL((agg_fwd_split_kernel<32, 1, 8, true>), dim3((unsigned)blocks), dim3(256), 0, st, a, p1, p2, scale, kp, rsc);
         else if (p.chunks <= 64) hipLaunchKernelGGL((agg_fwd_split_kernel<64, 1, 8, true>), dim3((unsigned)blocks), dim3(256), 0, st, a, p1, p2, scale, kp, rsc);
@@ -3900,19 +3976,46 @@
         const size_t lds = per_group * G;
 #define HUBCASE(L)                                                                                                                        \
         if (p.lpr == L) {                                                                                                                 \
-            auto k = agg_fwd_hub_kernel<4, L, 4>;                                                                                        \
+            auto k = gather_bias ? agg_fwd_hub_kernel<4, L, 4, true> : agg_fwd_hub_kernel<4, L, 4>;                                       \
             if (lds > 64 * 1024) (void)hipFuncSetAttribute(reinterpret_cast<const void *>(k), hipFuncAttributeMaxDynamicSharedMemorySize, (int)lds); \
             hipLaunchKernelGGL(k, dim3((unsigned)a.n_long * (unsigned)(a.hub_part ? a.hub_split : 1)), dim3(HUB_THREADS), lds, st, a);    \
         }
         HUBCASE(8) else HUBCASE(16) else HUBCASE(32) else HUBCASE(64)
 #undef HUBCASE
-        if (a.hub_part) hipLaunchKernelGGL((agg_hub_final_kernel<4, true>), dim3((unsigned)a.n_long), dim3(256), 0, st, a);
+        if (a.hub_part && gather_bias) hipLaunchKernelGGL((agg_hub_final_kernel<4, true, true>), dim3((unsigned)a.n_long), dim3(256), 0, st, a);
+        else if (a.hub_part) hipLaunchKernelGGL((agg_hub_final_kernel<4, true>), dim3((unsigned)a.n_long), dim3(256), 0, st, a);
         HIP_TRY(hipGetLastError());
         const int rc = row_order ? ctgcn_split_rows_mapped_((int64_t)a.n_long * K, d, kp, hub, d, p1, p2, scale, hub_row_dest, -1, rsc, stream)
                                  : ctgcn_split_rows_mapped_((int64_t)a.n_long * K, d, kp, hub, d, p1, p2, scale, long_rows, K, rsc, stream);
         if (rc != CTGCN_OK) return rc;
     }
     return CTGCN_OK;
+}
+
+int ctgcn_core_aggregate_split_f32(int64_t n_rows, int32_t d, int32_t K, const int32_t *row_ptr, const int32_t *col_idx,
+                                   const float *val, const uint8_t *slot, const float *X, int64_t ldx, uint32_t flags,
+                                   const int32_t *long_rows, int32_t n_long, int32_t long_threshold, int32_t n_out,
+                                   const int32_t *row_order, const uint32_t *tile_mask, const int32_t *tile_base, int64_t operand_rows,
+                                   const int32_t *hub_row_dest,
+                                   int32_t hub_split, void *hub_workspace, size_t hub_workspace_bytes,
+                                   void *workspace, size_t workspace_bytes, void *stream)
+{
+    return core_aggregate_split_(n_rows, d, K, row_ptr, col_idx, val, slot, X, ldx, nullptr, flags, long_rows, n_long, long_threshold, n_out,
+                                 row_order, tile_mask, tile_base, operand_rows, hub_row_dest, hub_split, hub_workspace,
+                                 hub_workspace_bytes, workspace, workspace_bytes, stream);
+}
+
+int ctgcn_core_aggregate_split_bias_f32(int64_t n_rows, int32_t d, int32_t K, const int32_t *row_ptr, const int32_t *col_idx,
+                                        const float *val, const uint8_t *slot, const float *Wt, const float *gather_bias, uint32_t flags,
+                                        const int32_t *long_rows, int32_t n_long, int32_t long_threshold, int32_t n_out,
+                                        const int32_t *row_order, const uint32_t *tile_mask, const int32_t *tile_base, int64_t operand_rows,
+                                        const int32_t *hub_row_dest,
+                                        int32_t hub_split, void *hub_workspace, size_t hub_workspace_bytes,
+                                        void *workspace, size_t workspace_bytes, void *stream)
+{
+    return core_aggregate_split_(n_rows, d, K, row_ptr, col_idx, val, slot, Wt, d, gather_bias, flags, long_rows, n_long, long_threshold, n_out,
+                                 row_order, tile_mask, tile_base, operand_rows, hub_row_dest, hub_split, hub_workspace,
+                                 hub_workspace_bytes, workspace, workspace_bytes, stream);
 }
 
 int ctgcn_core_aggregate_bwd_prep_f32(int64_t n_rows, int32_t d, int32_t K, const float *dH,
diff --git a/ctgcn_amd/layers.py b/ctgcn_amd/layers.py
--- a/ctgcn_amd/layers.py
+++ b/ctgcn_amd/layers.py
@@ -153,17 +153,19 @@
         self.rnn = _RNN[rnn_type](input_size=input_dim, hidden_size=output_dim, num_layers=1, bias=bias, batch_first=True)
         self.norm = nn.LayerNorm(output_dim)
 
-    def aggregate(self, x, adj_list):
-        return ops.core_aggregate(x, as_core_adj(adj_list, x.device), relu=True)
-
-    def forward(self, x, adj_list, out=None):
+    def aggregate(self, x, adj_list, gather_bias=None):
+        if gather_bias is None:
+            return ops.core_aggregate(x, as_core_adj(adj_list, x.device), relu=True)
+        return ops.core_aggregate(x, as_core_adj(adj_list, x.device), relu=True, gather_bias=gather_bias)
+
+    def forward(self, x, adj_list, out=None, gather_bias=None):
         if torch.is_tensor(x) and not x.is_sparse and x.is_cuda:
             adj = as_core_adj(adj_list, x.device)
             if ops.aggregate_split_ok(self.rnn, x, adj):
-                return ops.core_diffusion_split(x, adj, self.rnn, self.norm, out=out)
+                return ops.core_diffusion_split(x, adj, self.rnn, self.norm, out=out, gather_bias=gather_bias)
             if torch.is_grad_enabled() and ops.core_diffusion_fused_ok(self.rnn, self.norm, x, adj):
-                return ops.core_diffusion_fused(x, adj, self.rnn, self.norm)
-        seq = self.aggregate(x, adj_list)
+                return ops.core_diffusion_fused(x, adj, self.rnn, self.norm, gather_bias=gather_bias)
+        seq = self.aggregate(x, adj_list, gather_bias)
         return rnn_reduce_norm(self.rnn, self.norm, seq, reduce_sum=True, out=out)
 
 
@@ -196,12 +198,13 @@
             out = torch.sparse.mm(h, layer.weight.t())
             return (out if layer.bias is None else out + layer.bias), False
         needs_grad = torch.is_grad_enabled() and (h.requires_grad or any(p.requires_grad for p in layer.parameters()))
-        if not needs_grad and h.dim() == 2 and ops.linear_split_ok(h, layer.weight):
-            return ops.linear_split(h, layer.weight, layer.bias, selu=selu, static_x=static_x), bool(selu)
-        if needs_grad and h.dim() == 2 and ops.linear_train_enabled() and ops.linear_split_ok(h, layer.weight) and ops.plane_cache_enabled() \
+        weight = layer.weight.contiguous() if ops.in_gather_layout(layer.weight) else layer.weight
+        if not needs_grad and h.dim() == 2 and ops.linear_split_ok(h, weight):
+            return ops.linear_split(h, weight, layer.bias, selu=selu, static_x=static_x), bool(selu)
+        if needs_grad and h.dim() == 2 and ops.linear_train_enabled() and ops.linear_split_ok(h, weight) and ops.plane_cache_enabled() \
                 and h.shape[0] >= 4096:
-            return ops.linear_split_train(h, layer.weight, layer.bias, static_x=static_x), False
-        return layer(h), False
+            return ops.linear_split_train(h, weight, layer.bias, static_x=static_x), False
+        return (layer(h) if weight is layer.weight else F.linear(h, weight, layer.bias)), False
 
     def forward(self, x):
         stack = [self.linear] if self.layer_num == 1 else list(self.linears)
diff --git a/ctgcn_amd/models.py b/ctgcn_amd/models.py
--- a/ctgcn_amd/models.py
+++ b/ctgcn_amd/models.py
@@ -22,10 +22,10 @@
         self.diffusion_list = nn.ModuleList(
             CoreDiffusion(a, b, bias=bias, rnn_type=rnn_type) for a, b in zip(dims[:-1], dims[1:]))
 
-    def forward(self, x, adj_list, out=None):
+    def forward(self, x, adj_list, out=None, gather_bias=None):
         last = len(self.diffusion_list) - 1
         for i, layer in enumerate(self.diffusion_list):
-            x = layer(x, adj_list, out=out if i == last else None)
+            x = layer(x, adj_list, out=out if i == last else None, gather_bias=gather_bias if i == 0 else None)
         return x
 
 
@@ -111,7 +111,27 @@
         self.norm = nn.LayerNorm(output_dim)
         self.process_group = None
 
+    def gather_operand(self, t, x):
+        from .layers import _is_identity
+        mlp = self.mlp_list[t]
+        if self.model_type != 'C' or mlp.layer_num != 1 or mlp.activate_type != 'L' or not ops.linear_gather_enabled():
+            return None
+        w, b = mlp.linear.weight, mlp.linear.bias
+        if not (torch.is_tensor(x) and x.is_sparse and x.is_cuda and w.device == x.device and w.dtype == torch.float32
+                and x.shape[1] == w.shape[1] and _is_identity(x)):
+            return None
+        if b is not None and (b.dtype != torch.float32 or not b.is_contiguous() or b.data_ptr() % 16):
+            return None
+        if not w.t().is_contiguous():
+            if torch.cuda.is_current_stream_capturing():
+                return None
+            ops.to_gather_layout(w)
+        return w.t(), b
+
     def snapshot_branch(self, t, x, adj, out=None):
+        g = self.gather_operand(t, x)
+        if g is not None:
+            return self.duffision_list[t](g[0], adj, out=out, gather_bias=g[1]), None
         trans = self.mlp_list[t](x)
         return self.duffision_list[t](trans, adj, out=out), trans
 
@@ -284,10 +304,11 @@
             self._grouped_layers(g0, hx, adj_list, seq)
         elif g0 is not None:
             def head(t):
-                tr = self.mlp_list[t](x_list[t])
-                h = tr
+                g = self.gather_operand(t, x_list[t]) if g0 >= 1 else None
+                tr = self.mlp_list[t](x_list[t]) if g is None else None
+                h = tr if g is None else g[0]
                 for l in range(g0):
-                    h = self.duffision_list[t].diffusion_list[l](h, adj_list[t])
+                    h = self.duffision_list[t].diffusion_list[l](h, adj_list[t], gather_bias=g[1] if (g is not None and l == 0) else None)
                 return h, tr
             if lanes:
                 main = torch.cuda.current_stream(seq.device)
@@ -297,7 +318,8 @@
                     with torch.cuda.stream(lanes[t % len(lanes)]):
                         h, tr = head(t)
                         h.record_stream(main)
-                        tr.record_stream(main)
+                        if tr is not None:
+                            tr.record_stream(main)
                     hx.append(h)
                     trans.append(tr)
                 for s_ in lanes:
@@ -317,7 +339,8 @@
                     h, tr = self.snapshot_branch(t, x_list[t], adj_list[t], out=seq[:, t])
                     if h.data_ptr() != seq[:, t].data_ptr():
                         seq[:, t].copy_(h)
-                    tr.record_stream(main)
+                    if tr is not None:
+                        tr.record_stream(main)
                 hx.append(h)
                 trans.append(tr)
             for s_ in lanes:
@@ -331,7 +354,8 @@
                 with torch.cuda.stream(tl[t % len(tl)]):
                     h, tr = self.snapshot_branch(t, x_list[t], adj_list[t])
                     h.record_stream(main)
-                    tr.record_stream(main)
+                    if tr is not None:
+                        tr.record_stream(main)
                 hx.append(h)
                 trans.append(tr)
             for s_ in tl:
diff --git a/ctgcn_amd/ops.py b/ctgcn_amd/ops.py
--- a/ctgcn_amd/ops.py
+++ b/ctgcn_amd/ops.py
@@ -129,9 +129,28 @@
     return out
 
 
+def linear_gather_enabled():
+    import os
+    return os.environ.get("CTGCN_LINEAR_GATHER", "1") != "0"
+
+
+def in_gather_layout(weight):
+    return weight.dim() == 2 and weight.stride(1) != 1 and weight.t().is_contiguous()
+
+
+def to_gather_layout(weight):
+    if weight.dim() != 2 or weight.t().is_contiguous():
+        return weight
+    with torch.no_grad():
+        weight.data = weight.detach().t().contiguous().t()
+    return weight
+
+
 def _transpose_bias(src, bias):
     lib = _lib.load()
     d, n = src.shape
+    if in_gather_layout(src):
+        return src.t() + bias if bias is not None else src.t().clone()
     w = src if src.stride(1) == 1 else src.contiguous()
     out = torch.empty(n, d, dtype=torch.float32, device=src.device)
     with torch.cuda.device(src.device):
@@ -171,7 +190,14 @@
     return split, torch.empty(nbytes, dtype=torch.uint8, device=device), nbytes
 
 
-def _aggregate_fwd(adj, x, relu):
+def _check_gather_bias(x, gather_bias):
+    if not x.is_contiguous():
+        raise ValueError("gather_bias goes with dense [n, d] rows (a weight in gather layout), got strides %s" % (tuple(x.stride()),))
+    if gather_bias.dtype != torch.float32 or gather_bias.shape != (x.shape[1],) or gather_bias.device != x.device or not gather_bias.is_contiguous():
+        raise ValueError("gather_bias must be a contiguous fp32 [%d] vector on %s" % (x.shape[1], x.device))
+
+
+def _aggregate_fwd(adj, x, relu, gather_bias=None):
     lib = _lib.load()
     n, d = x.shape
     H = torch.empty(n, adj.K, d, dtype=torch.float32, device=x.device)
@@ -179,6 +205,12 @@
     with torch.cuda.device(x.device), _timed("agg_fwd", n=n, d=d, K=adj.K, nnz=adj.nnz):
         long_rows = adj.long_rows()
         split, hub_ws, hub_bytes = _hub_pieces(lib, adj, long_rows, adj.K, d, x.device)
+        if gather_bias is not None:
+            _check_gather_bias(x, gather_bias)
+            check(lib.ctgcn_core_aggregate_bias_f32(n, d, adj.K, ptr(adj.row_ptr), ptr(adj.col), ptr(adj.val), ptr(adj.slot), ptr(x),
+                                                    ptr(gather_bias), ptr(H), flags, ptr(long_rows), 0 if long_rows is None else long_rows.numel(),
+                                                    adj.LONG_ROW, split, ptr(hub_ws), hub_bytes, _stream()), "ctgcn_core_aggregate_bias_f32")
+            return H
         check(lib.ctgcn_core_aggregate_f32(n, d, adj.K, ptr(adj.row_ptr), ptr(adj.col), ptr(adj.val), ptr(adj.slot), ptr(x),
                                            x.stride(0), ptr(H), flags, ptr(long_rows), 0 if long_rows is None else long_rows.numel(),
                                            adj.LONG_ROW, split, ptr(hub_ws), hub_bytes, _stream()), "ctgcn_core_aggregate_f32")
@@ -214,8 +246,8 @@
 
 class _CoreAggregate(torch.autograd.Function):
     @staticmethod
-    def forward(ctx, x, adj, relu):
-        H = _aggregate_fwd(adj, x, relu)
+    def forward(ctx, x, adj, relu, gather_bias):
+        H = _aggregate_fwd(adj, x, relu, None if gather_bias is None else gather_bias.detach())
         ctx.adj, ctx.relu = adj, relu
         ctx.save_for_backward(H)
         return H
@@ -224,10 +256,11 @@
     def backward(ctx, dH):
         (H,) = ctx.saved_tensors
         dH = dH.contiguous()
-        return _aggregate_bwd(ctx.adj, H, dH, ctx.relu), None, None
-
-
-def core_aggregate(x, adj, relu=True):
+        dX = _aggregate_bwd(ctx.adj, H, dH, ctx.relu)
+        return dX, None, None, (dX.sum(0) if ctx.needs_input_grad[3] else None)
+
+
+def core_aggregate(x, adj, relu=True, gather_bias=None):
     _need_cuda(x, adj.col)
     if adj.K < 1:
         raise ValueError("empty k-core adjacency list")
@@ -238,7 +271,7 @@
     if x.device != adj.device:
         raise ValueError("features on %s but adjacency on %s" % (x.device, adj.device))
     x = x if x.stride(1) == 1 else x.contiguous()
-    return _CoreAggregate.apply(x, adj, relu)
+    return _CoreAggregate.apply(x, adj, relu, gather_bias)
 
 
 import os as _os
@@ -702,7 +735,7 @@
     return os.environ.get("CTGCN_DEDUP", "1") != "0"
 
 
-def aggregate_split_planes(x, adj, n_out, plan=None, ws=None):
+def aggregate_split_planes(x, adj, n_out, plan=None, ws=None, gather_bias=None):
     lib = _lib.load()
     n, d = x.shape
     flags = adj.flags | _lib.F_RELU
@@ -717,6 +750,15 @@
     hub_dest = adj.plan_row_dest(plan, long_rows, compact) if (plan is not None and n_long) else None
     split, hub_ws, hub_bytes = _hub_pieces(lib, adj, long_rows, adj.K, d, x.device)
     with _timed("agg_fwd", n=n, d=d, K=adj.K, nnz=adj.nnz, split=True, rows_written=(plan["new_rows"] if plan is not None else n * adj.K)):
+        if gather_bias is not None:
+            _check_gather_bias(x, gather_bias)
+            check(lib.ctgcn_core_aggregate_split_bias_f32(n, d, adj.K, ptr(adj.row_ptr), ptr(adj.col), ptr(adj.val), ptr(adj.slot), ptr(x), ptr(gather_bias),
+                                                          flags, ptr(long_rows), n_long, adj.LONG_ROW, n_out,
+                                                          ptr(plan["order"]) if plan is not None else None, ptr(plan["tile_mask"]) if plan is not None else None,
+                                                          ptr(plan["tile_base"]) if compact else None, plan["operand_rows"] if compact else 0,
+                                                          ptr(hub_dest), split, ptr(hub_ws), hub_bytes, ptr(ws), ws_bytes, _stream()),
+                  "ctgcn_core_aggregate_split_bias_f32")
+            return ws, ws_bytes
         check(lib.ctgcn_core_aggregate_split_f32(n, d, adj.K, ptr(adj.row_ptr), ptr(adj.col), ptr(adj.val), ptr(adj.slot), ptr(x), x.stride(0),
                                                  flags, ptr(long_rows), n_long, adj.LONG_ROW, n_out,
                                                  ptr(plan["order"]) if plan is not None else None, ptr(plan["tile_mask"]) if plan is not None else None,
@@ -740,7 +782,7 @@
     return out
 
 
-def core_diffusion_split(x, adj, rnn, norm, out=None):
+def core_diffusion_split(x, adj, rnn, norm, out=None, gather_bias=None):
     lib = _lib.load()
     n, d = x.shape
     K, hid = adj.K, rnn.hidden_size
@@ -753,7 +795,7 @@
     with torch.cuda.device(x.device):
         if d == hid:
             plan = adj.row_plan() if row_plan_enabled() else None
-            ws, _ = aggregate_split_planes(x, adj, 1, plan)
+            ws, _ = aggregate_split_planes(x, adj, 1, plan, gather_bias=gather_bias)
             return gru_layer_presplit(ws, n, K, rnn, norm, out, plan)
         bias, b_hn = _gru_bias(rnn, hid)
         w_ih, w_hh = rnn.weight_ih_l0.detach(), rnn.weight_hh_l0.detach().contiguous()
@@ -762,7 +804,7 @@
         eps = 0.0 if norm is None else float(norm.eps)
         plan = adj.row_plan(adj.PLAN_TILE_GEMM) if (row_plan_enabled() and forward_split_mode() == 2) else None
         rows = plan["operand_rows"] if plan is not None else n * K
-        ws, ws_bytes = aggregate_split_planes(x, adj, n_out, plan)
+        ws, ws_bytes = aggregate_split_planes(x, adj, n_out, plan, gather_bias=gather_bias)
         gi_buf = torch.empty(rows * n_out, dtype=torch.float32, device=x.device) if plan is not None else _gi_buffer(n, K, hid, x.device)
         with _timed("linear_split", rows=rows, k=d, n_out=n_out, presplit=True):
             if plane_cache_enabled():
@@ -812,13 +854,15 @@
 class _CoreDiffusionFused(torch.autograd.Function):
 
     @staticmethod
-    def forward(ctx, x, adj, w_ih, w_hh, b_ih, b_hh, ln_w, ln_b, eps):
+    def forward(ctx, x, adj, w_ih, w_hh, b_ih, b_hh, ln_w, ln_b, eps, gather_bias):
         lib = _lib.load()
         n, K, hid = adj.n, adj.K, w_hh.shape[1]
         plan = adj.row_plan() if row_plan_enabled() else None
         x_d = x.detach()
+        gb = None if gather_bias is None else gather_bias.detach()
+        ctx.gather_bias = gb
         with torch.cuda.device(x.device):
-            ws, _ = aggregate_split_planes(x_d, adj, 1, plan)
+            ws, _ = aggregate_split_planes(x_d, adj, 1, plan, gather_bias=gb)
             bias, b_hn = _fold_gru_bias(b_ih, b_hh, hid)
             out = torch.empty(n, hid, dtype=torch.float32, device=x.device)
             with _timed("gru_layer", rows=n, steps=K, reduce_sum=True, presplit=True, new_rows=(plan["new_rows"] if plan is not None else n * K)):
@@ -843,7 +887,7 @@
         ws, w_ih, w_hh, b_ih, b_hh, ln_w, ln_b = ctx.saved_tensors
         if not ctx.kept:
             with torch.cuda.device(ws.device):
-                ws, _ = aggregate_split_planes(ws, ctx.adj, 1, ctx.plan)
+                ws, _ = aggregate_split_planes(ws, ctx.adj, 1, ctx.plan, gather_bias=ctx.gather_bias)
         adj, plan, eps = ctx.adj, ctx.plan, ctx.eps
         n, K, hid = adj.n, adj.K, w_hh.shape[1]
         dev = ws.device
@@ -889,14 +933,16 @@
                                                    ptr(Z) if order is not None else ptr(Z[lo:]),
                                                    ptr(S0) if (S0 is None or order is not None) else ptr(S0[lo:]), od, 1 if adj.nested else 0,
                                                    ptr(dw_ih_part), ptr(dbi_part), nb, 1, _stream()), "ctgcn_gru_bwd_in_f32")
-            dX = _aggregate_gather(adj, Z, S0, True) if ctx.needs_input_grad[0] else None
+            need_gb = ctx.gather_bias is not None and ctx.needs_input_grad[9]
+            dX = _aggregate_gather(adj, Z, S0, True) if (ctx.needs_input_grad[0] or need_gb) else None
         dw_ih = dw_ih_part.sum(0)
         dw_hh = dw_hh_part.sum(0)
         db_ih = db_hh = None
         if b_ih is not None:
             db_ih = dbi_part.sum(0)
             db_hh = torch.cat([db_ih[: 2 * hid], dbn_part.sum(0)])
-        return dX, None, dw_ih, dw_hh, db_ih, db_hh, ln_sum[:hid].clone(), ln_sum[hid:].clone(), None
+        d_gb = dX.sum(0) if (ctx.gather_bias is not None and ctx.needs_input_grad[9]) else None
+        return dX, None, dw_ih, dw_hh, db_ih, db_hh, ln_sum[:hid].clone(), ln_sum[hid:].clone(), None, d_gb
 
 
 def _fold_gru_bias(b_ih, b_hh, hid):
@@ -907,10 +953,10 @@
     return bias, b_hh.detach()[2 * hid:].contiguous()
 
 
-def core_diffusion_fused(x, adj, rnn, norm):
+def core_diffusion_fused(x, adj, rnn, norm, gather_bias=None):
     b_ih = rnn.bias_ih_l0 if rnn.bias else None
     b_hh = rnn.bias_hh_l0 if rnn.bias else None
-    return _CoreDiffusionFused.apply(x, adj, rnn.weight_ih_l0, rnn.weight_hh_l0, b_ih, b_hh, norm.weight, norm.bias, float(norm.eps))
+    return _CoreDiffusionFused.apply(x, adj, rnn.weight_ih_l0, rnn.weight_hh_l0, b_ih, b_hh, norm.weight, norm.bias, float(norm.eps), gather_bias)
 
 
 _GROUP_MAX_NODES = 200_000
diff --git a/include/ctgcn_hip.h b/include/ctgcn_hip.h
--- a/include/ctgcn_hip.h
+++ b/include/ctgcn_hip.h
@@ -57,6 +57,11 @@
                              const float *X, int64_t ldx, float *H, uint32_t flags,
                              const int32_t *long_rows, int32_t n_long, int32_t long_threshold,
                              int32_t hub_split, void *hub_workspace, size_t hub_workspace_bytes, void *stream);
+int ctgcn_core_aggregate_bias_f32(int64_t n_rows, int32_t d, int32_t K, const int32_t *row_ptr,
+                                  const int32_t *col_idx, const float *val, const uint8_t *slot,
+                                  const float *Wt, const float *gather_bias, float *H, uint32_t flags,
+                                  const int32_t *long_rows, int32_t n_long, int32_t long_threshold,
+                                  int32_t hub_split, void *hub_workspace, size_t hub_workspace_bytes, void *stream);
 
 int ctgcn_core_aggregate_bwd_prep_f32(int64_t n_rows, int32_t d, int32_t K, const float *dH,
                                       const float *H, float *Z, float *S0, uint32_t flags,
@@ -193,6 +198,13 @@
                                    const int32_t *hub_row_dest,
                                    int32_t hub_split, void *hub_workspace, size_t hub_workspace_bytes,
                                    void *workspace, size_t workspace_bytes, void *stream);
+int ctgcn_core_aggregate_split_bias_f32(int64_t n_rows, int32_t d, int32_t K, const int32_t *row_ptr, const int32_t *col_idx,
+                                        const float *val, const uint8_t *slot, const float *Wt, const float *gather_bias, uint32_t flags,
+                                        const int32_t *long_rows, int32_t n_long, int32_t long_threshold, int32_t n_out,
+                                        const int32_t *row_order, const uint32_t *tile_mask, const int32_t *tile_base, int64_t operand_rows,
+                                        const int32_t *hub_row_dest,
+                                        int32_t hub_split, void *hub_workspace, size_t hub_workspace_bytes,
+                                        void *workspace, size_t workspace_bytes, void *stream);
 int ctgcn_linear_presplit_f32(int64_t rows, int32_t n_out, int32_t k, const float *w, int64_t ldw, const float *bias, float *y, int64_t ldy,
                               void *workspace, size_t workspace_bytes, void *stream);
 
```

Result: faster. 11.28 billion edges/s (median of 6 runs) (+1.9%).
